# fpthink/3D-WSIS

Hardware: AMD Instinct MI355X
Metric: scenes/sec fwd+bwd ScanNet 2cm (~150k voxels) @1/8 GPU; HBM GB/s vs roofline (higher is better)
Workload: dtype f32

## Files before the change

3d-wsis_amd/csrc/bn.hip:

```cpp
#include <cstdlib>

#include "common.h"

using namespace wsis;

namespace {

constexpr int BN_ROWS_PER_THREAD = 8;
__host__ __device__ inline int bn_rows_per_wg(int Cp) {
  const int G = Cp >> 2;
  const int R = 256 / G > 1 ? 256 / G : 1;
  return R * BN_ROWS_PER_THREAD;
}
constexpr int BN_THREADS = 256;

struct f4 {
  float v[4];
};
__device__ __forceinline__ f4 ld4(const float* p, bool vec) {
  f4 r;
  if (vec) {
    const float4 t = *reinterpret_cast<const float4*>(p);
    r.v[0] = t.x; r.v[1] = t.y; r.v[2] = t.z; r.v[3] = t.w;
  } else {
    r.v[0] = p[0]; r.v[1] = p[1]; r.v[2] = p[2]; r.v[3] = p[3];
  }
  return r;
}

__device__ __forceinline__ float bn_pivot(const float* __restrict__ x, int64_t M, int C, int c) {
  const int n = M < 8 ? (int)M : 8;
  float s = 0.0f;
  for (int r = 0; r < n; ++r) s += x[(int64_t)r * C + c];
  return s / (float)n;
}

__global__ __launch_bounds__(BN_THREADS) void bn_stats_partial_kernel(const float* __restrict__ x, int64_t M, int C,
                                                                      int Cp, float* __restrict__ partial) {
  __shared__ float s_a[BN_THREADS * 4];
  __shared__ float s_b[BN_THREADS * 4];
  const int G = Cp >> 2;
  const int R = max(BN_THREADS / G, 1);
  const bool vec = (C & 3) == 0;
  const int64_t r0 = (int64_t)blockIdx.x * bn_rows_per_wg(Cp);
  const int64_t r1 = min(M, r0 + bn_rows_per_wg(Cp));
  for (int g0 = 0; g0 < G; g0 += BN_THREADS) {
    const int g = g0 + (threadIdx.x % min(G, BN_THREADS));
    const int rl = threadIdx.x / min(G, BN_THREADS);
    float sa[4] = {0.f, 0.f, 0.f, 0.f}, sb[4] = {0.f, 0.f, 0.f, 0.f};
    if (g < G && rl < R) {
      const int c = g * 4;
      float K[4];
#pragma unroll
      for (int e = 0; e < 4; ++e) K[e] = (c + e < C) ? bn_pivot(x, M, C, c + e) : 0.0f;
#pragma unroll 8
      for (int64_t r = r0 + rl; r < r1; r += R) {
        float v[4];
        if (vec) {
          const f4 t = ld4(x + r * C + c, true);
#pragma unroll
          for (int e = 0; e < 4; ++e) v[e] = t.v[e] - K[e];
        } else {
#pragma unroll
          for (int e = 0; e < 4; ++e) v[e] = (c + e < C) ? x[r * C + c + e] - K[e] : 0.0f;
        }
#pragma unroll
        for (int e = 0; e < 4; ++e) {
          sa[e] += v[e];
          sb[e] += v[e] * v[e];
        }
      }
    }
#pragma unroll
    for (int e = 0; e < 4; ++e) {
      s_a[threadIdx.x * 4 + e] = sa[e];
      s_b[threadIdx.x * 4 + e] = sb[e];
    }
    __syncthreads();
    if (g < G && rl == 0) {
      const int gw = min(G, BN_THREADS);
      float ta[4] = {0.f, 0.f, 0.f, 0.f}, tb[4] = {0.f, 0.f, 0.f, 0.f};
      for (int j = 0; j < R; ++j)
#pragma unroll
        for (int e = 0; e < 4; ++e) {
          ta[e] += s_a[(j * gw + (threadIdx.x % gw)) * 4 + e];
          tb[e] += s_b[(j * gw + (threadIdx.x % gw)) * 4 + e];
        }
      float* p = partial + (int64_t)blockIdx.x * 2 * Cp;
#pragma unroll
      for (int e = 0; e < 4; ++e) {
        p[g * 4 + e] = ta[e];
        p[Cp + g * 4 + e] = tb[e];
      }
    }
    __syncthreads();
  }
}

__device__ __forceinline__ double wave_sum_f64(double v) {
#pragma unroll
  for (int off = 32; off >= 1; off >>= 1) v += __shfl_xor(v, off, 64);
  return v;
}

__global__ __launch_bounds__(64) void bn_stats_final_kernel(const float* __restrict__ partial, int nblk, int C,
                                                            int Cp, int64_t M, const float* __restrict__ x0,
                                                            float* __restrict__ mean,
                                                            float* __restrict__ var,
                                                            float* __restrict__ running_mean,
                                                            float* __restrict__ running_var, float momentum) {
  const int c = blockIdx.x;
  double s = 0.0, q = 0.0;
#pragma unroll 8
  for (int b = threadIdx.x; b < nblk; b += 64) {
    s += partial[(int64_t)b * 2 * Cp + c];
    q += partial[(int64_t)b * 2 * Cp + Cp + c];
  }
  const double S = wave_sum_f64(s), Q = wave_sum_f64(q);
  if (threadIdx.x == 0) {
    const double n = (double)M;
    const double ms = S / n;
    const double mu = (double)bn_pivot(x0, M, C, c) + ms;
    double v = Q / n - ms * ms;
    if (v < 0.0) v = 0.0;
    mean[c] = (float)mu;
    var[c] = (float)v;
    if (running_mean) {
      const double unb = n > 1 ? v * n / (n - 1) : v;
      running_mean[c] = (float)((1.0 - momentum) * running_mean[c] + momentum * mu);
      running_var[c] = (float)((1.0 - momentum) * running_var[c] + momentum * unb);
    }
  }
}

constexpr int BN_FIN_CHUNKS = kBnFinChunks;

__device__ __forceinline__ bool bn_chunk_centred_stage(const float* __restrict__ partial, int nblk, int C, int64_t M,
                                                       double* __restrict__ chunk, float* __restrict__ mean,
                                                       float* __restrict__ var, float* __restrict__ running_mean,
                                                       float* __restrict__ running_var, float momentum,
                                                       unsigned* __restrict__ ticket, int g0, int G, int cgi,
                                                       double (&red)[3][8][33], int& s_last) {
  const int cl = threadIdx.x & 31, pl = threadIdx.x >> 5;
  const int c = cgi * 32 + cl;
  const int per = (nblk + G - 1) / G;
  const int lo = g0 * per;
  const int hi = lo + per < nblk ? lo + per : nblk;
  double s = 0.0, q = 0.0, w = 0.0;
  if (c < C) {
#pragma unroll 4
    for (int b = lo + pl; b < hi; b += 8) {
      const float sf = partial[(int64_t)b * 2 * C + c];
      const float qf = partial[(int64_t)b * 2 * C + C + c];
      const int64_t left = M - (int64_t)b * 32;
      const double si = sf;
      s += si;
      q += qf;
      w += si * si * (left < 32 ? 1.0 / (double)left : 0.03125);
    }
  }
  red[0][pl][cl] = s;
  red[1][pl][cl] = q;
  red[2][pl][cl] = w;
  __syncthreads();
  if (pl == 0 && c < C) {
    double S = 0.0, Q = 0.0, W = 0.0;
#pragma unroll
    for (int j = 0; j < 8; ++j) {
      S += red[0][j][cl];
      Q += red[1][j][cl];
      W += red[2][j][cl];
    }
    if (G == 1) {
      bn_finish_centred(S, Q, W, M, c, mean, var, running_mean, running_var, momentum);
    } else {
      double* o = chunk + (int64_t)g0 * 3 * C;
      st_sc1(o + c, S);
      st_sc1(o + C + c, Q);
      st_sc1(o + 2 * C + c, W);
    }
  }
  if (G == 1) return true;
  if (!ticket) return false;
  wait_stores_left();
  __syncthreads();
  if (threadIdx.x == 0) {
    const unsigned t = atomicAdd(ticket + cgi, 1u);
    s_last = t == (unsigned)G - 1;
    if (s_last) ticket[cgi] = 0u;
  }
  __syncthreads();
  if (!s_last) return false;
  double s2 = 0.0, q2 = 0.0, w2 = 0.0;
  if (c < C)
    for (int g = pl; g < G; g += 8) {
      const double* o = chunk + (int64_t)g * 3 * C;
      s2 += ld_sc1(o + c);
      q2 += ld_sc1(o + C + c);
      w2 += ld_sc1(o + 2 * C + c);
    }
  __syncthreads();
  red[0][pl][cl] = s2;
  red[1][pl][cl] = q2;
  red[2][pl][cl] = w2;
  __syncthreads();
  if (pl == 0 && c < C) {
    double S = 0.0, Q = 0.0, W = 0.0;
#pragma unroll
    for (int j = 0; j < 8; ++j) {
      S += red[0][j][cl];
      Q += red[1][j][cl];
      W += red[2][j][cl];
    }
    bn_finish_centred(S, Q, W, M, c, mean, var, running_mean, running_var, momentum);
  }
  return true;
}

__global__ __launch_bounds__(256) void bn_stats_chunk_centred_kernel(const float* __restrict__ partial, int nblk, int C,
                                                                     int64_t M, double* __restrict__ chunk,
                                                                     float* __restrict__ mean, float* __restrict__ var,
                                                                     float* __restrict__ running_mean,
                                                                     float* __restrict__ running_var, float momentum,
                                                                     unsigned* __restrict__ ticket) {
  __shared__ double red[3][8][33];
  __shared__ int s_last;
  bn_chunk_centred_stage(partial, nblk, C, M, chunk, mean, var, running_mean, running_var, momentum, ticket,
                         (int)blockIdx.x, (int)gridDim.x, (int)blockIdx.y, red, s_last);
}

__global__ __launch_bounds__(256) void bn_stats_final_centred_kernel(const double* __restrict__ chunk, int G, int C,
                                                                     int64_t M, float* __restrict__ mean,
                                                                     float* __restrict__ var,
                                                                     float* __restrict__ running_mean,
                                                                     float* __restrict__ running_var, float momentum) {
  const int lane = threadIdx.x & 63;
  const int c = blockIdx.x * 4 + (threadIdx.x >> 6);
  if (c >= C) return;
  const bool in = lane < G;
  const double S = wave_sum_f64(in ? chunk[(int64_t)lane * 3 * C + c] : 0.0);
  const double Q = wave_sum_f64(in ? chunk[(int64_t)lane * 3 * C + C + c] : 0.0);
  const double W = wave_sum_f64(in ? chunk[(int64_t)lane * 3 * C + 2 * C + c] : 0.0);
  if (lane == 0) bn_finish_centred(S, Q, W, M, c, mean, var, running_mean, running_var, momentum);
}

template <bool COHERENT>
__device__ __forceinline__ float bn_ld_stat(const float* p) {
  if (COHERENT) return __hip_atomic_load(p, __ATOMIC_RELAXED, __HIP_MEMORY_SCOPE_AGENT);
  return *p;
}

template <bool COHERENT>
__device__ __forceinline__ void bn_apply_body(const float* __restrict__ x, const float* mean,
                                              const float* var, const float* __restrict__ gamma,
                                              const float* __restrict__ beta, float eps, int relu,
                                              float* __restrict__ y, int64_t M, int C) {
  const int64_t total = M * C;
  if ((C & 3) == 0) {
    const int64_t total4 = total >> 2;
    const unsigned C4 = (unsigned)(C >> 2);
    const int64_t stride = (int64_t)gridDim.x * blockDim.x;
    int64_t t = blockIdx.x * (int64_t)blockDim.x + threadIdx.x;
    const bool fixed_c = (stride % C4) == 0;
    unsigned cg = (unsigned)(t % C4);
    float sc[4], mu[4], bt[4];
    auto coef = [&](unsigned g) {
#pragma unroll
      for (int e = 0; e < 4; ++e) {
        const int c = (int)g * 4 + e;
        sc[e] = (gamma ? gamma[c] : 1.0f) * rsqrtf(bn_ld_stat<COHERENT>(var + c) + eps);
        mu[e] = bn_ld_stat<COHERENT>(mean + c);
        bt[e] = beta ? beta[c] : 0.0f;
      }
    };
    coef(cg);
    auto body = [&](const float4 v) {
      float o[4] = {v.x, v.y, v.z, v.w};
#pragma unroll
      for (int e = 0; e < 4; ++e) {
        float z = __builtin_fmaf(o[e] - mu[e], sc[e], bt[e]);
        if (relu) z = fmaxf(z, 0.0f);
        o[e] = z;
      }
      return make_float4(o[0], o[1], o[2], o[3]);
    };
    if (fixed_c) {
      for (; t + stride < total4; t += 2 * stride) {
        const float4 v0 = reinterpret_cast<const float4*>(x)[t];
        const float4 v1 = reinterpret_cast<const float4*>(x)[t + stride];
        reinterpret_cast<float4*>(y)[t] = body(v0);
        reinterpret_cast<float4*>(y)[t + stride] = body(v1);
      }
      if (t < total4) reinterpret_cast<float4*>(y)[t] = body(reinterpret_cast<const float4*>(x)[t]);
    } else {
      for (; t < total4; t += stride) {
        cg = (unsigned)(t % C4);
        coef(cg);
        reinterpret_cast<float4*>(y)[t] = body(reinterpret_cast<const float4*>(x)[t]);
      }
    }
  } else {
    for (int64_t t = blockIdx.x * (int64_t)blockDim.x + threadIdx.x; t < total;
         t += (int64_t)gridDim.x * blockDim.x) {
      const int c = (int)(t % C);
      const float sc = (gamma ? gamma[c] : 1.0f) * rsqrtf(bn_ld_stat<COHERENT>(var + c) + eps);
      float z = __builtin_fmaf(x[t] - bn_ld_stat<COHERENT>(mean + c), sc, beta ? beta[c] : 0.0f);
      if (relu) z = fmaxf(z, 0.0f);
      y[t] = z;
    }
  }
}

__global__ void bn_apply_kernel(const float* __restrict__ x, const float* __restrict__ mean,
                                const float* __restrict__ var, const float* __restrict__ gamma,
                                const float* __restrict__ beta, float eps, int relu, float* __restrict__ y,
                                int64_t M, int C) {
  bn_apply_body<false>(x, mean, var, gamma, beta, eps, relu, y, M, C);
}

constexpr int BN_POLL_SLEEP = 12;
constexpr unsigned long long BN_SPIN_LIMIT = 200000000ull;

__device__ __forceinline__ void bn_wait_published(SyncSlot* s) {
  if (threadIdx.x == 0) {
    const unsigned long long t0 = __builtin_amdgcn_s_memrealtime();
    while (__hip_atomic_load(&s->flag, __ATOMIC_RELAXED, __HIP_MEMORY_SCOPE_AGENT) == 0u) {
      __builtin_amdgcn_s_sleep(BN_POLL_SLEEP);
      if (__builtin_amdgcn_s_memrealtime() - t0 > BN_SPIN_LIMIT) {
        __hip_atomic_store(&s->err, 1u, __ATOMIC_RELAXED, __HIP_MEMORY_SCOPE_AGENT);
        break;
      }
    }
    const unsigned l = atomicAdd(&s->left, 1u);
    if (l == gridDim.x - 1) {
      __hip_atomic_store(&s->left, 0u, __ATOMIC_RELAXED, __HIP_MEMORY_SCOPE_AGENT);
      __hip_atomic_store(&s->flag, 0u, __ATOMIC_RELAXED, __HIP_MEMORY_SCOPE_AGENT);
    }
  }
  __syncthreads();
}
__device__ __forceinline__ void bn_publish(SyncSlot* s, int CG) {
  const unsigned d = atomicAdd(&s->done, 1u);
  if (d == (unsigned)CG - 1) {
    __hip_atomic_store(&s->done, 0u, __ATOMIC_RELAXED, __HIP_MEMORY_SCOPE_AGENT);
    __threadfence();
    __hip_atomic_store(&s->flag, 1u, __ATOMIC_RELEASE, __HIP_MEMORY_SCOPE_AGENT);
  }
}

__global__ __launch_bounds__(256) void bn_finalize_apply_kernel(
    const float* __restrict__ partial, int nblk, int C, int64_t M, double* __restrict__ chunk, int G,
    float* mean, float* var, float* __restrict__ running_mean,
    float* __restrict__ running_var, float momentum, SyncSlot* __restrict__ sync, const float* __restrict__ x,
    const float* __restrict__ gamma, const float* __restrict__ beta, float eps, int relu, float* __restrict__ y) {
  __shared__ double red[3][8][33];
  __shared__ int s_last;
  const int CG = (C + 31) / 32;
  if ((int)blockIdx.x < G * CG) {
    const bool fin = bn_chunk_centred_stage(partial, nblk, C, M, chunk, mean, var, running_mean, running_var, momentum,
                                            sync->ticket, (int)blockIdx.x % G, G, (int)blockIdx.x / G, red, s_last);
    if (fin) {
      __threadfence();
      __syncthreads();
      if (threadIdx.x == 0) bn_publish(sync, CG);
    }
  }
  bn_wait_published(sync);
  bn_apply_body<true>(x, mean, var, gamma, beta, eps, relu, y, M, C);
}

__global__ __launch_bounds__(BN_THREADS) void bn_bwd_partial_kernel(
    const float* __restrict__ x, const float* __restrict__ dy, const float* __restrict__ mean,
    const float* __restrict__ var, const float* __restrict__ gamma, const float* __restrict__ beta, float eps,
    int relu, int64_t M, int C, int Cp, float* __restrict__ partial) {
  __shared__ float s_a[BN_THREADS * 4];
  __shared__ float s_b[BN_THREADS * 4];
  const int G = Cp >> 2;
  const int gw = min(G, BN_THREADS);
  const int R = max(BN_THREADS / G, 1);
  const bool vec = (C & 3) == 0;
  const int64_t r0 = (int64_t)blockIdx.x * bn_rows_per_wg(Cp);
  const int64_t r1 = min(M, r0 + bn_rows_per_wg(Cp));
  for (int g0 = 0; g0 < G; g0 += BN_THREADS) {
    const int g = g0 + (threadIdx.x % gw);
    const int rl = threadIdx.x / gw;
    float sa[4] = {0.f, 0.f, 0.f, 0.f}, sb[4] = {0.f, 0.f, 0.f, 0.f};
    if (g < G && rl < R) {
      const int c = g * 4;
      float mu[4], rstd[4], gm[4], bt[4];
#pragma unroll
      for (int e = 0; e < 4; ++e) {
        const int cc = min(c + e, C - 1);
        mu[e] = mean[cc];
        rstd[e] = rsqrtf(var[cc] + eps);
        gm[e] = gamma ? gamma[cc] : 1.0f;
        bt[e] = beta ? beta[cc] : 0.0f;
      }
#pragma unroll 8
      for (int64_t r = r0 + rl; r < r1; r += R) {
        float xv[4], dv[4];
        if (vec) {
          const f4 tx = ld4(x + r * C + c, true), td = ld4(dy + r * C + c, true);
#pragma unroll
          for (int e = 0; e < 4; ++e) {
            xv[e] = tx.v[e];
            dv[e] = td.v[e];
          }
        } else {
#pragma unroll
          for (int e = 0; e < 4; ++e) {
            const bool ok = c + e < C;
            xv[e] = ok ? x[r * C + c + e] : 0.0f;
            dv[e] = ok ? dy[r * C + c + e] : 0.0f;
          }
        }
#pragma unroll
        for (int e = 0; e < 4; ++e) {
          const float xh = (xv[e] - mu[e]) * rstd[e];
          float dz = dv[e];
          if (relu && xh * gm[e] + bt[e] <= 0.0f) dz = 0.0f;
          sa[e] += dz;
          sb[e] += dz * xh;
        }
      }
    }
#pragma unroll
    for (int e = 0; e < 4; ++e) {
      s_a[threadIdx.x * 4 + e] = sa[e];
      s_b[threadIdx.x * 4 + e] = sb[e];
    }
    __syncthreads();
    if (g < G && rl == 0) {
      float ta[4] = {0.f, 0.f, 0.f, 0.f}, tb[4] = {0.f, 0.f, 0.f, 0.f};
      for (int j = 0; j < R; ++j)
#pragma unroll
        for (int e = 0; e < 4; ++e) {
          ta[e] += s_a[(j * gw + (threadIdx.x % gw)) * 4 + e];
          tb[e] += s_b[(j * gw + (threadIdx.x % gw)) * 4 + e];
        }
      float* p = partial + (int64_t)blockIdx.x * 2 * Cp;
#pragma unroll
      for (int e = 0; e < 4; ++e) {
        p[g * 4 + e] = ta[e];
        p[Cp + g * 4 + e] = tb[e];
      }
    }
    __syncthreads();
  }
}

__global__ __launch_bounds__(64) void bn_bwd_final_kernel(const float* __restrict__ partial, int nblk, int C, int Cp,
                                                          float* __restrict__ dgamma, float* __restrict__ dbeta) {
  const int c = blockIdx.x;
  double a = 0.0, b = 0.0;
#pragma unroll 8
  for (int k = threadIdx.x; k < nblk; k += 64) {
    a += partial[(int64_t)k * 2 * Cp + c];
    b += partial[(int64_t)k * 2 * Cp + Cp + c];
  }
  const double A = wave_sum_f64(a), B = wave_sum_f64(b);
  if (threadIdx.x == 0) {
    dbeta[c] = (float)A;
    dgamma[c] = (float)B;
  }
}

__device__ __forceinline__ bool bn_sum_chunk_stage(const float* __restrict__ partial, int nblk, int C,
                                                   double* __restrict__ chunk, float* dbeta, float* dgamma,
                                                   unsigned* __restrict__ ticket, int g0, int G, int cgi,
                                                   double (&red)[2][8][33], int& s_last) {
  const int cl = threadIdx.x & 31, pl = threadIdx.x >> 5;
  const int c = cgi * 32 + cl;
  const int per = (nblk + G - 1) / G;
  const int lo = g0 * per;
  const int hi = lo + per < nblk ? lo + per : nblk;
  double a = 0.0, b = 0.0;
  if (c < C) {
#pragma unroll 4
    for (int k = lo + pl; k < hi; k += 8) {
      a += partial[(int64_t)k * 2 * C + c];
      b += partial[(int64_t)k * 2 * C + C + c];
    }
  }
  red[0][pl][cl] = a;
  red[1][pl][cl] = b;
  __syncthreads();
  if (pl == 0 && c < C) {
    double A = 0.0, B = 0.0;
#pragma unroll
    for (int j = 0; j < 8; ++j) {
      A += red[0][j][cl];
      B += red[1][j][cl];
    }
    if (G == 1) {
      dbeta[c] = (float)A;
      dgamma[c] = (float)B;
    } else {
      st_sc1(chunk + (int64_t)g0 * 2 * C + c, A);
      st_sc1(chunk + (int64_t)g0 * 2 * C + C + c, B);
    }
  }
  if (G == 1) return true;
  if (!ticket) return false;
  wait_stores_left();
  __syncthreads();
  if (threadIdx.x == 0) {
    const unsigned t = atomicAdd(ticket + cgi, 1u);
    s_last = t == (unsigned)G - 1;
    if (s_last) ticket[cgi] = 0u;
  }
  __syncthreads();
  if (!s_last) return false;
  double a2 = 0.0, b2 = 0.0;
  if (c < C)
    for (int g = pl; g < G; g += 8) {
      const double* o = chunk + (int64_t)g * 2 * C;
      a2 += ld_sc1(o + c);
      b2 += ld_sc1(o + C + c);
    }
  __syncthreads();
  red[0][pl][cl] = a2;
  red[1][pl][cl] = b2;
  __syncthreads();
  if (pl == 0 && c < C) {
    double A = 0.0, B = 0.0;
#pragma unroll
    for (int j = 0; j < 8; ++j) {
      A += red[0][j][cl];
      B += red[1][j][cl];
    }
    dbeta[c] = (float)A;
    dgamma[c] = (float)B;
  }
  return true;
}

__global__ __launch_bounds__(256) void bn_sum_chunk_kernel(const float* __restrict__ partial, int nblk, int C,
                                                           double* __restrict__ chunk, float* __restrict__ dbeta,
                                                           float* __restrict__ dgamma, unsigned* __restrict__ ticket) {
  __shared__ double red[2][8][33];
  __shared__ int s_last;
  bn_sum_chunk_stage(partial, nblk, C, chunk, dbeta, dgamma, ticket, (int)blockIdx.x, (int)gridDim.x, (int)blockIdx.y, red,
                     s_last);
}

__global__ __launch_bounds__(256) void bn_sum_final_kernel(const double* __restrict__ chunk, int G, int C,
                                                           float* __restrict__ dbeta, float* __restrict__ dgamma) {
  const int lane = threadIdx.x & 63;
  const int c = blockIdx.x * 4 + (threadIdx.x >> 6);
  if (c >= C) return;
  const bool in = lane < G;
  const double A = wave_sum_f64(in ? chunk[(int64_t)lane * 2 * C + c] : 0.0);
  const double B = wave_sum_f64(in ? chunk[(int64_t)lane * 2 * C + C + c] : 0.0);
  if (lane == 0) {
    dbeta[c] = (float)A;
    dgamma[c] = (float)B;
  }
}

template <bool COHERENT>
__device__ __forceinline__ void bn_bwd_apply_body(const float* __restrict__ x, const float* __restrict__ dy,
                                                  const float* __restrict__ mean, const float* __restrict__ var,
                                                  const float* __restrict__ gamma, const float* __restrict__ beta,
                                                  const float* dgamma, const float* dbeta,
                                                  const float* __restrict__ addend, float eps, int relu, int training,
                                                  float* __restrict__ dx, int64_t M, int C) {
  const int64_t total = M * C;
  const float inv_m = 1.0f / (float)M;
  const bool vec = (C & 3) == 0;
  const int W = vec ? 4 : 1;
  const int64_t totalw = total / W;
  const unsigned Cw = (unsigned)(C / W);
  const int64_t stride = (int64_t)gridDim.x * blockDim.x;
  int64_t t = blockIdx.x * (int64_t)blockDim.x + threadIdx.x;
  const bool fixed_c = (stride % Cw) == 0;
  float mu[4], rstd[4], gm[4], bt[4], k1[4], k2[4];
  auto coef = [&](int c0) {
#pragma unroll
    for (int e = 0; e < 4; ++e) {
      if (e < W) {
        const int c = c0 + e;
        mu[e] = mean[c];
        rstd[e] = rsqrtf(var[c] + eps);
        gm[e] = gamma ? gamma[c] : 1.0f;
        bt[e] = beta ? beta[c] : 0.0f;
        k1[e] = training ? bn_ld_stat<COHERENT>(dbeta + c) * inv_m : 0.0f;
        k2[e] = training ? bn_ld_stat<COHERENT>(dgamma + c) * inv_m : 0.0f;
      }
    }
  };
  if (t < totalw) coef((int)(t % Cw) * W);
  auto one = [&](const float (&xv)[4], const float (&dv)[4], const float (&av)[4], float (&ov)[4]) {
#pragma unroll
    for (int e = 0; e < 4; ++e) {
      if (e < W) {
        const float xh = (xv[e] - mu[e]) * rstd[e];
        float dz = dv[e];
        if (relu && xh * gm[e] + bt[e] <= 0.0f) dz = 0.0f;
        float r = dz;
        if (training) r = dz - k1[e] - xh * k2[e];
        ov[e] = gm[e] * rstd[e] * r;
        if (addend) ov[e] += av[e];
      }
    }
  };
  if (vec && fixed_c) {
    for (; t + stride < totalw; t += 2 * stride) {
      const int64_t u = t + stride;
      const f4 tx0 = ld4(x + t * 4, true), td0 = ld4(dy + t * 4, true);
      const f4 tx1 = ld4(x + u * 4, true), td1 = ld4(dy + u * 4, true);
      f4 ta0, ta1;
#pragma unroll
      for (int e = 0; e < 4; ++e) ta0.v[e] = ta1.v[e] = 0.f;
      if (addend) {
        ta0 = ld4(addend + t * 4, true);
        ta1 = ld4(addend + u * 4, true);
      }
      float o0[4], o1[4];
      one(tx0.v, td0.v, ta0.v, o0);
      one(tx1.v, td1.v, ta1.v, o1);
      reinterpret_cast<float4*>(dx)[t] = make_float4(o0[0], o0[1], o0[2], o0[3]);
      reinterpret_cast<float4*>(dx)[u] = make_float4(o1[0], o1[1], o1[2], o1[3]);
    }
  }
  for (; t < totalw; t += stride) {
    if (!fixed_c) coef((int)(t % Cw) * W);
    float xv[4], dv[4], av[4] = {0.f, 0.f, 0.f, 0.f}, ov[4];
    if (vec) {
      const f4 tx = ld4(x + t * 4, true), td = ld4(dy + t * 4, true);
#pragma unroll
      for (int e = 0; e < 4; ++e) {
        xv[e] = tx.v[e];
        dv[e] = td.v[e];
      }
      if (addend) {
        const f4 ta = ld4(addend + t * 4, true);
#pragma unroll
        for (int e = 0; e < 4; ++e) av[e] = ta.v[e];
      }
    } else {
      xv[0] = x[t];
      dv[0] = dy[t];
      if (addend) av[0] = addend[t];
    }
    one(xv, dv, av, ov);
    if (vec)
      reinterpret_cast<float4*>(dx)[t] = make_float4(ov[0], ov[1], ov[2], ov[3]);
    else
      dx[t] = ov[0];
  }
}

__global__ void bn_bwd_apply_kernel(const float* __restrict__ x, const float* __restrict__ dy,
                                    const float* __restrict__ mean, const float* __restrict__ var,
                                    const float* __restrict__ gamma, const float* __restrict__ beta,
                                    const float* __restrict__ dgamma, const float* __restrict__ dbeta,
                                    const float* __restrict__ addend, float eps, int relu, int training,
                                    float* __restrict__ dx, int64_t M, int C) {
  bn_bwd_apply_body<false>(x, dy, mean, var, gamma, beta, dgamma, dbeta, addend, eps, relu, training, dx, M, C);
}

__global__ __launch_bounds__(256) void bn_bwd_finish_apply_kernel(
    const float* __restrict__ partial, int nblk, int C, double* __restrict__ chunk, int G, float* dbeta, float* dgamma,
    SyncSlot* __restrict__ sync, const float* __restrict__ x, const float* __restrict__ dy, const float* __restrict__ mean,
    const float* __restrict__ var, const float* __restrict__ gamma, const float* __restrict__ beta,
    const float* __restrict__ addend, float eps, int relu, float* __restrict__ dx, int64_t M) {
  __shared__ double red[2][8][33];
  __shared__ int s_last;
  const int CG = (C + 31) / 32;
  if ((int)blockIdx.x < G * CG) {
    const bool fin = bn_sum_chunk_stage(partial, nblk, C, chunk, dbeta, dgamma, sync->ticket, (int)blockIdx.x % G, G,
                                        (int)blockIdx.x / G, red, s_last);
    if (fin) {
      __threadfence();
      __syncthreads();
      if (threadIdx.x == 0) bn_publish(sync, CG);
    }
  }
  bn_wait_published(sync);
  bn_bwd_apply_body<true>(x, dy, mean, var, gamma, beta, dgamma, dbeta, addend, eps, relu, 1, dx, M, C);
}

constexpr int BN_SF_ROWS = 256;

__global__ __launch_bounds__(256) void bn_small_finish_apply_kernel(
    const float* __restrict__ partial, int nblk, int C, int64_t M, float* __restrict__ mean, float* __restrict__ var,
    float* __restrict__ running_mean, float* __restrict__ running_var, float momentum, const float* __restrict__ x,
    const float* __restrict__ gamma, const float* __restrict__ beta, float eps, int relu, float* __restrict__ y, int G) {
  __shared__ double red[3][8][33];
  __shared__ float s_mu[32], s_sc[32], s_bt[32];
  const int cgi = blockIdx.y;
  const int cl = threadIdx.x & 31, pl = threadIdx.x >> 5;
  const int c = cgi * 32 + cl;
  const int per = (nblk + G - 1) / G;
  double S = 0.0, Q = 0.0, W = 0.0;
  for (int g = 0; g < G; ++g) {
    const int lo = g * per;
    const int hi = lo + per < nblk ? lo + per : nblk;
    double s = 0.0, q = 0.0, w = 0.0;
    if (c < C) {
#pragma unroll 4
      for (int b = lo + pl; b < hi; b += 8) {
        const float sf = partial[(int64_t)b * 2 * C + c];
        const float qf = partial[(int64_t)b * 2 * C + C + c];
        const int64_t left = M - (int64_t)b * 32;
        const double si = sf;
        s += si;
        q += qf;
        w += si * si * (left < 32 ? 1.0 / (double)left : 0.03125);
      }
    }
    if (g) __syncthreads();
    red[0][pl][cl] = s;
    red[1][pl][cl] = q;
    red[2][pl][cl] = w;
    __syncthreads();
    if (pl == 0 && c < C) {
      double Sg = 0.0, Qg = 0.0, Wg = 0.0;
#pragma unroll
      for (int j = 0; j < 8; ++j) {
        Sg += red[0][j][cl];
        Qg += red[1][j][cl];
        Wg += red[2][j][cl];
      }
      if (G == 1) {
        S = Sg; Q = Qg; W = Wg;
      } else {
        S += Sg; Q += Qg; W += Wg;
      }
    }
  }
  if (pl == 0 && c < C) {
    const double n = (double)M;
    const double mu = S / n;
    double v = (Q + (W - n * mu * mu)) / n;
    if (v < 0.0) v = 0.0;
    const float muf = (float)mu, vf = (float)v;
    if (blockIdx.x == 0) {
      mean[c] = muf;
      var[c] = vf;
      if (running_mean) {
        const double unb = n > 1 ? v * n / (n - 1) : v;
        running_mean[c] = (float)((1.0 - momentum) * running_mean[c] + momentum * mu);
        running_var[c] = (float)((1.0 - momentum) * running_var[c] + momentum * unb);
      }
    }
    s_mu[cl] = muf;
    s_sc[cl] = (gamma ? gamma[c] : 1.0f) * rsqrtf(vf + eps);
    s_bt[cl] = beta ? beta[c] : 0.0f;
  }
  __syncthreads();
  const int q4 = threadIdx.x & 7, rl = threadIdx.x >> 3;
  const int c4 = cgi * 32 + q4 * 4;
  if (c4 >= C) return;
  float mu4[4], sc4[4], bt4[4];
#pragma unroll
  for (int e = 0; e < 4; ++e) {
    mu4[e] = s_mu[q4 * 4 + e];
    sc4[e] = s_sc[q4 * 4 + e];
    bt4[e] = s_bt[q4 * 4 + e];
  }
  const int64_t r0 = (int64_t)blockIdx.x * BN_SF_ROWS;
#pragma unroll 4
  for (int it = 0; it < BN_SF_ROWS / 32; ++it) {
    const int64_t r = r0 + it * 32 + rl;
    if (r < M) {
      const float4 vx = *reinterpret_cast<const float4*>(x + r * C + c4);
      float o[4] = {vx.x, vx.y, vx.z, vx.w};
#pragma unroll
      for (int e = 0; e < 4; ++e) {
        float z = __builtin_fmaf(o[e] - mu4[e], sc4[e], bt4[e]);
        if (relu) z = fmaxf(z, 0.0f);
        o[e] = z;
      }
      *reinterpret_cast<float4*>(y + r * C + c4) = make_float4(o[0], o[1], o[2], o[3]);
    }
  }
}

__global__ __launch_bounds__(256) void bn_small_bwd_finish_apply_kernel(
    const float* __restrict__ partial, int nblk, int C, int64_t M, const float* __restrict__ x,
    const float* __restrict__ dy, const float* __restrict__ mean, const float* __restrict__ var,
    const float* __restrict__ gamma, const float* __restrict__ beta, const float* __restrict__ addend, float eps, int relu,
    float* __restrict__ dx, float* __restrict__ dgamma, float* __restrict__ dbeta, int G) {
  __shared__ double red[2][8][33];
  __shared__ float s_k1[32], s_k2[32];
  const int cgi = blockIdx.y;
  const int cl = threadIdx.x & 31, pl = threadIdx.x >> 5;
  const int c = cgi * 32 + cl;
  const int per = (nblk + G - 1) / G;
  double A = 0.0, B = 0.0;
  for (int g = 0; g < G; ++g) {
    const int lo = g * per;
    const int hi = lo + per < nblk ? lo + per : nblk;
    double a = 0.0, b = 0.0;
    if (c < C) {
#pragma unroll 4
      for (int k = lo + pl; k < hi; k += 8) {
        a += partial[(int64_t)k * 2 * C + c];
        b += partial[(int64_t)k * 2 * C + C + c];
      }
    }
    if (g) __syncthreads();
    red[0][pl][cl] = a;
    red[1][pl][cl] = b;
    __syncthreads();
    if (pl == 0 && c < C) {
      double Ag = 0.0, Bg = 0.0;
#pragma unroll
      for (int j = 0; j < 8; ++j) {
        Ag += red[0][j][cl];
        Bg += red[1][j][cl];
      }
      if (G == 1) {
        A = Ag; B = Bg;
      } else {
        A += Ag; B += Bg;
      }
    }
  }
  if (pl == 0 && c < C) {
    const float db = (float)A, dg = (float)B;
    if (blockIdx.x == 0) {
      dbeta[c] = db;
      dgamma[c] = dg;
    }
    const float inv_m = 1.0f / (float)M;
    s_k1[cl] = db * inv_m;
    s_k2[cl] = dg * inv_m;
  }
  __syncthreads();
  const int q4 = threadIdx.x & 7, rl = threadIdx.x >> 3;
  const int c4 = cgi * 32 + q4 * 4;
  if (c4 >= C) return;
  float mu[4], rstd[4], gm[4], bt[4], k1[4], k2[4];
#pragma unroll
  for (int e = 0; e < 4; ++e) {
    const int cc = c4 + e;
    mu[e] = mean[cc];
    rstd[e] = rsqrtf(var[cc] + eps);
    gm[e] = gamma ? gamma[cc] : 1.0f;
    bt[e] = beta ? beta[cc] : 0.0f;
    k1[e] = s_k1[q4 * 4 + e];
    k2[e] = s_k2[q4 * 4 + e];
  }
  const int64_t r0 = (int64_t)blockIdx.x * BN_SF_ROWS;
#pragma unroll 2
  for (int it = 0; it < BN_SF_ROWS / 32; ++it) {
    const int64_t r = r0 + it * 32 + rl;
    if (r < M) {
      const float4 vx = *reinterpret_cast<const float4*>(x + r * C + c4);
      const float4 vd = *reinterpret_cast<const float4*>(dy + r * C + c4);
      float4 va = make_float4(0.f, 0.f, 0.f, 0.f);
      if (addend) va = *reinterpret_cast<const float4*>(addend + r * C + c4);
      const float xv[4] = {vx.x, vx.y, vx.z, vx.w}, dv[4] = {vd.x, vd.y, vd.z, vd.w}, av[4] = {va.x, va.y, va.z, va.w};
      float ov[4];
#pragma unroll
      for (int e = 0; e < 4; ++e) {
        const float xh = (xv[e] - mu[e]) * rstd[e];
        float dz = dv[e];
        if (relu && xh * gm[e] + bt[e] <= 0.0f) dz = 0.0f;
        const float rr = dz - k1[e] - xh * k2[e];
        ov[e] = gm[e] * rstd[e] * rr;
        if (addend) ov[e] += av[e];
      }
      *reinterpret_cast<float4*>(dx + r * C + c4) = make_float4(ov[0], ov[1], ov[2], ov[3]);
    }
  }
}

static int bn_small_gmax() {
  const char* e = getenv("WSIS_BN_SMALL_G");
  const int g = e ? atoi(e) : 4;
  return g < 1 ? 1 : g > 8 ? 8 : g;
}
static bool bn_small_fused_on() {
  const char* e = getenv("WSIS_BN_SMALL_FUSED");
  return !e || atoi(e) != 0;
}

int64_t bn_small_rows() {
  static const int64_t v = [] {
    const char* e = getenv("WSIS_BN_SMALL_ROWS");
    return e ? (int64_t)atoll(e) : (int64_t)4096;
  }();
  return v;
}
constexpr int BN_SMALL_THREADS = 1024;

__device__ __forceinline__ void block_sum2_f64(double (&a)[4], double (&b)[4], double* sh) {
  const int lane = threadIdx.x & 63, wave = threadIdx.x >> 6;
#pragma unroll
  for (int off = 32; off >= 1; off >>= 1) {
#pragma unroll
    for (int e = 0; e < 4; ++e) {
      a[e] += __shfl_xor(a[e], off, 64);
      b[e] += __shfl_xor(b[e], off, 64);
    }
  }
  if (lane == 0) {
#pragma unroll
    for (int e = 0; e < 4; ++e) {
      sh[wave * 8 + e] = a[e];
      sh[wave * 8 + 4 + e] = b[e];
    }
  }
  __syncthreads();
#pragma unroll
  for (int e = 0; e < 4; ++e) {
    double sa = 0.0, sb = 0.0;
    for (int w = 0; w < BN_SMALL_THREADS / 64; ++w) {
      sa += sh[w * 8 + e];
      sb += sh[w * 8 + 4 + e];
    }
    a[e] = sa;
    b[e] = sb;
  }
}

__global__ __launch_bounds__(BN_SMALL_THREADS) void bn_stats_small_kernel(const float* __restrict__ x, int64_t M, int C,
                                                                    float* __restrict__ mean, float* __restrict__ var,
                                                                    float* __restrict__ running_mean,
                                                                    float* __restrict__ running_var, float momentum) {
  __shared__ double sh[BN_SMALL_THREADS / 64 * 8];
  const int c0 = blockIdx.x * 4;
  const bool vec = (C & 3) == 0;
  float sa[4] = {0.f, 0.f, 0.f, 0.f}, sb[4] = {0.f, 0.f, 0.f, 0.f};
  float K[4];
#pragma unroll
  for (int e = 0; e < 4; ++e) K[e] = (c0 + e < C) ? bn_pivot(x, M, C, c0 + e) : 0.0f;
#pragma unroll 8
  for (int64_t r = threadIdx.x; r < M; r += BN_SMALL_THREADS) {
    float v[4];
    if (vec) {
      const f4 t = ld4(x + r * C + c0, true);
#pragma unroll
      for (int e = 0; e < 4; ++e) v[e] = t.v[e] - K[e];
    } else {
#pragma unroll
      for (int e = 0; e < 4; ++e) v[e] = (c0 + e < C) ? x[r * C + c0 + e] - K[e] : 0.0f;
    }
#pragma unroll
    for (int e = 0; e < 4; ++e) {
      sa[e] += v[e];
      sb[e] += v[e] * v[e];
    }
  }
  double a[4], b[4];
#pragma unroll
  for (int e = 0; e < 4; ++e) {
    a[e] = sa[e];
    b[e] = sb[e];
  }
  block_sum2_f64(a, b, sh);
  if (threadIdx.x < 4 && c0 + (int)threadIdx.x < C) {
    const int e = threadIdx.x, c = c0 + e;
    const double n = (double)M;
    const double ms = a[e] / n;
    const double mu = (double)K[e] + ms;
    double v = b[e] / n - ms * ms;
    if (v < 0.0) v = 0.0;
    mean[c] = (float)mu;
    var[c] = (float)v;
    if (running_mean) {
      const double unb = n > 1 ? v * n / (n - 1) : v;
      running_mean[c] = (float)((1.0 - momentum) * running_mean[c] + momentum * mu);
      running_var[c] = (float)((1.0 - momentum) * running_var[c] + momentum * unb);
    }
  }
}

__global__ __launch_bounds__(BN_SMALL_THREADS) void bn_bwd_small_kernel(
    const float* __restrict__ x, const float* __restrict__ dy, const float* __restrict__ mean,
    const float* __restrict__ var, const float* __restrict__ gamma, const float* __restrict__ beta, float eps,
    int relu, int64_t M, int C, float* __restrict__ dgamma, float* __restrict__ dbeta) {
  __shared__ double sh[BN_SMALL_THREADS / 64 * 8];
  const int c0 = blockIdx.x * 4;
  const bool vec = (C & 3) == 0;
  float mu[4], rstd[4], gm[4], bt[4];
#pragma unroll
  for (int e = 0; e < 4; ++e) {
    const int cc = min(c0 + e, C - 1);
    mu[e] = mean[cc];
    rstd[e] = rsqrtf(var[cc] + eps);
    gm[e] = gamma ? gamma[cc] : 1.0f;
    bt[e] = beta ? beta[cc] : 0.0f;
  }
  float sa[4] = {0.f, 0.f, 0.f, 0.f}, sb[4] = {0.f, 0.f, 0.f, 0.f};
#pragma unroll 8
  for (int64_t r = threadIdx.x; r < M; r += BN_SMALL_THREADS) {
    float xv[4], dv[4];
    if (vec) {
      const f4 tx = ld4(x + r * C + c0, true), td = ld4(dy + r * C + c0, true);
#pragma unroll
      for (int e = 0; e < 4; ++e) {
        xv[e] = tx.v[e];
        dv[e] = td.v[e];
      }
    } else {
#pragma unroll
      for (int e = 0; e < 4; ++e) {
        const bool ok = c0 + e < C;
        xv[e] = ok ? x[r * C + c0 + e] : 0.0f;
        dv[e] = ok ? dy[r * C + c0 + e] : 0.0f;
      }
    }
#pragma unroll
    for (int e = 0; e < 4; ++e) {
      const float xh = (xv[e] - mu[e]) * rstd[e];
      float dz = dv[e];
      if (relu && xh * gm[e] + bt[e] <= 0.0f) dz = 0.0f;
      sa[e] += dz;
      sb[e] += dz * xh;
    }
  }
  double a[4], b[4];
#pragma unroll
  for (int e = 0; e < 4; ++e) {
    a[e] = sa[e];
    b[e] = sb[e];
  }
  block_sum2_f64(a, b, sh);
  if (threadIdx.x < 4 && c0 + (int)threadIdx.x < C) {
    dbeta[c0 + threadIdx.x] = (float)a[threadIdx.x];
    dgamma[c0 + threadIdx.x] = (float)b[threadIdx.x];
  }
}

int bn_nblk(int64_t M, int Cp) { return (int)ceil_div(M > 0 ? M : 1, (int64_t)bn_rows_per_wg(Cp)); }

}

extern "C" {

int64_t wsis_bn_workspace_bytes(int64_t M, int32_t C) {
  if (M < 0 || C < 1) return -1;
  const int64_t Cp = (C + 3) / 4 * 4;
  return (int64_t)bn_nblk(M, (int)Cp) * 2 * Cp * (int64_t)sizeof(float) + 256;
}

int wsis_bn_stats(const float* d_x, int64_t M, int32_t C, float* d_mean, float* d_var, float* d_running_mean,
                  float* d_running_var, float momentum, void* d_ws, int64_t ws_bytes, void* stream) {
  WSIS_REQUIRE(M >= 1 && C >= 1 && d_x && d_mean && d_var && d_ws, "bad args");
  WSIS_REQUIRE(ws_bytes >= wsis_bn_workspace_bytes(M, C), "workspace too small");
  WSIS_REQUIRE((d_running_mean == nullptr) == (d_running_var == nullptr), "running stats come in pairs");
  const int Cp = (C + 3) / 4 * 4;
  const int nblk = bn_nblk(M, Cp);
  float* partial = static_cast<float*>(d_ws);
  hipStream_t st = as_stream(stream);
  WSIS_REQUIRE(Cp / 4 <= BN_THREADS, "C > 1024 is not supported");
  if (M <= bn_small_rows()) {
    hipLaunchKernelGGL(bn_stats_small_kernel, dim3(Cp / 4), dim3(BN_SMALL_THREADS), 0, st, d_x, M, C, d_mean, d_var,
                       d_running_mean, d_running_var, momentum);
    WSIS_LAUNCH_CHECK();
    return WSIS_OK;
  }
  hipLaunchKernelGGL(bn_stats_partial_kernel, dim3(nblk), dim3(BN_THREADS), 0, st, d_x, M, C, Cp, partial);
  WSIS_LAUNCH_CHECK();
  hipLaunchKernelGGL(bn_stats_final_kernel, dim3(C), dim3(64), 0, st, partial, nblk, C, Cp, M, d_x, d_mean,
                     d_var, d_running_mean, d_running_var, momentum);
  WSIS_LAUNCH_CHECK();
  return WSIS_OK;
}


__device__ __forceinline__ void colsum_block(const bool IN, const bool OUT, const float* __restrict__ x, int64_t lo,
                                             int64_t hi, int C4, float4* red, float* __restrict__ out) {
  const int RL = 256 / C4;
  const int cl = threadIdx.x % C4, rl = threadIdx.x / C4;
  float4 a = {0.f, 0.f, 0.f, 0.f};
  if (rl < RL) {
    const float4* x4 = reinterpret_cast<const float4*>(x);
#pragma unroll 8
    for (int64_t r = lo + rl; r < hi; r += RL) {
      float4 v;
      if (IN) {
        const float* p = x + (r * C4 + cl) * 4;
        v = make_float4(ld_sc1(p), ld_sc1(p + 1), ld_sc1(p + 2), ld_sc1(p + 3));
      } else {
        v = x4[r * C4 + cl];
      }
      a.x += v.x;
      a.y += v.y;
      a.z += v.z;
      a.w += v.w;
    }
    red[rl * C4 + cl] = a;
  }
  __syncthreads();
  if (threadIdx.x < C4) {
    float4 s = red[threadIdx.x];
    for (int j = 1; j < RL; ++j) {
      const float4 v = red[j * C4 + threadIdx.x];
      s.x += v.x;
      s.y += v.y;
      s.z += v.z;
      s.w += v.w;
    }
    if (OUT) {
      float* p = out + threadIdx.x * 4;
      st_sc1(p, s.x);
      st_sc1(p + 1, s.y);
      st_sc1(p + 2, s.z);
      st_sc1(p + 3, s.w);
    } else {
      reinterpret_cast<float4*>(out)[threadIdx.x] = s;
    }
  }
}

__global__ __launch_bounds__(256) void colsum_kernel(const float* __restrict__ x, int64_t M, int C, int64_t per,
                                                     float* __restrict__ chunk, float* __restrict__ out,
                                                     unsigned* __restrict__ ticket) {
  __shared__ float4 red[256];
  __shared__ int s_last;
  const int C4 = C >> 2;
  const int64_t lo = (int64_t)blockIdx.x * per;
  const int64_t hi = lo + per < M ? lo + per : M;
  if (gridDim.x == 1) {
    colsum_block(false, false, x, lo, hi, C4, red, out);
    return;
  }
  colsum_block(false, true, x, lo, hi, C4, red, chunk + (int64_t)blockIdx.x * C);
  wait_stores_left();
  __syncthreads();
  if (threadIdx.x == 0) {
    const unsigned t = atomicAdd(ticket, 1u);
    s_last = t == gridDim.x - 1;
    if (s_last) *ticket = 0u;
  }
  __syncthreads();
  if (!s_last) return;
  __syncthreads();
  colsum_block(true, false, chunk, 0, gridDim.x, C4, red, out);
}

static unsigned* bn_tickets(void* d_sync) {
  static int on = -1;
  if (on < 0) {
    const char* e = tune_env("WSIS_BN_TICKET");
    on = e ? atoi(e) : 1;
  }
  if (!on || !d_sync) return nullptr;
  return static_cast<SyncSlot*>(d_sync)->ticket;
}


int64_t wsis_bn_stats_finalize_workspace_bytes(int64_t n_part, int32_t C) {
  return (int64_t)bn_fin_chunks(n_part) * 3 * C * (int64_t)sizeof(double) + 256;
}

int wsis_bn_stats_finalize(const float* d_partials, int64_t n_part, int64_t M, int32_t C, float* d_mean, float* d_var,
                           float* d_running_mean, float* d_running_var, float momentum, void* d_ws, int64_t ws_bytes,
                           void* d_sync, void* stream) {
  WSIS_REQUIRE(n_part >= 1 && M >= 1 && C >= 1 && d_partials && d_mean && d_var, "bad args");
  WSIS_REQUIRE(n_part < ((int64_t)1 << 31), "too many partials");
  WSIS_REQUIRE((d_running_mean == nullptr) == (d_running_var == nullptr), "running stats come in pairs");
  WSIS_REQUIRE(n_part == (M + 31) / 32, "one partial per 32-row slice");
  const int G = bn_fin_chunks(n_part);
  WSIS_REQUIRE(G == 1 || (d_ws && ws_bytes >= wsis_bn_stats_finalize_workspace_bytes(n_part, C)), "workspace too small");
  double* chunk = reinterpret_cast<double*>((reinterpret_cast<uintptr_t>(d_ws) + 255) & ~(uintptr_t)255);
  WSIS_REQUIRE(C <= 512, "more than 512 channels");
  unsigned* tickets = bn_tickets(d_sync);
  hipLaunchKernelGGL(bn_stats_chunk_centred_kernel, dim3(G, (C + 31) / 32), dim3(256), 0, as_stream(stream), d_partials,
                     (int)n_part, C, M, chunk, d_mean, d_var, d_running_mean, d_running_var, momentum, tickets);
  WSIS_LAUNCH_CHECK();
  if (G > 1 && !tickets) {
    hipLaunchKernelGGL(bn_stats_final_centred_kernel, dim3((C + 3) / 4), dim3(256), 0, as_stream(stream), chunk, G, C, M,
                       d_mean, d_var, d_running_mean, d_running_var, momentum);
    WSIS_LAUNCH_CHECK();
  }
  return WSIS_OK;
}

static int bn_fused_grid(int64_t M, int C, int need_chunk_wgs, int which = 0) {
#if !WSIS_EXPERIMENTAL
  return 0;
#endif
  const char* e = getenv("WSIS_BN_FUSED_APPLY");
  const int on = e ? atoi(e) : 0;
  const char* ed = getenv(which ? "WSIS_BN_FUSED_BWD" : "WSIS_BN_FUSED_FWD");
  const int on_dir = ed ? atoi(ed) : on;
  const char* g = tune_env("WSIS_BN_FUSED_GRID");
  int gmax = g ? atoi(g) : 256;
  if (gmax < 64 || gmax > 512) gmax = 256;
  int n_cu = 0;
  {
    int dev = 0, v = 0;
    n_cu = (hipGetDevice(&dev) == hipSuccess &&
            hipDeviceGetAttribute(&v, hipDeviceAttributeMultiprocessorCount, dev) == hipSuccess) ? v : 0;
  }
  if (!on_dir || (C & 3) != 0) return 0;
  const int cw = C >> 2;
  const int64_t work = (M * C) >> 2;
  int gcap = (work > 600000 && gmax == 256) ? 512 : gmax;
  if (gcap > 2 * n_cu) gcap = 2 * n_cu;
  if (gcap < 1) return 0;
  int grid = gcap - (gcap % cw);
  const int need = grid_for(work, 256);
  if (need < grid) {
    grid = need;
    if (grid > cw) grid -= grid % cw;
  }
  return (grid >= need_chunk_wgs && grid >= 1) ? grid : 0;
}

int wsis_bn_stats_finalize_apply(const float* d_partials, int64_t n_part, int64_t M, int32_t C, float* d_mean,
                                 float* d_var, float* d_running_mean, float* d_running_var, float momentum,
                                 const float* d_x, const float* d_gamma, const float* d_beta, float eps, int32_t relu,
                                 float* d_y, void* d_ws, int64_t ws_bytes, void* d_sync, void* stream) {
  WSIS_REQUIRE(n_part >= 1 && M >= 1 && C >= 1 && d_partials && d_mean && d_var && d_x && d_y, "bad args");
  WSIS_REQUIRE(n_part == (M + 31) / 32 && n_part < ((int64_t)1 << 31), "one partial per 32-row slice");
  WSIS_REQUIRE(C <= 512, "more than 512 channels");
  hipStream_t st = as_stream(stream);
  const int G = bn_fin_chunks(n_part);
  const int CG = (C + 31) / 32;
  WSIS_REQUIRE(G == 1 || (d_ws && ws_bytes >= wsis_bn_stats_finalize_workspace_bytes(n_part, C)), "workspace too small");
  double* chunk = reinterpret_cast<double*>((reinterpret_cast<uintptr_t>(d_ws) + 255) & ~(uintptr_t)255);
  unsigned* tickets = bn_tickets(d_sync);
  const int grid = tickets ? bn_fused_grid(M, C, G * CG) : 0;
  const bool fused = grid > 0;
  if (G <= bn_small_gmax() && (G == 1 || tickets) && (C & 3) == 0 && bn_small_fused_on() &&
      (reinterpret_cast<uintptr_t>(d_x) & 15) == 0 &&
      (reinterpret_cast<uintptr_t>(d_y) & 15) == 0) {
    hipLaunchKernelGGL(bn_small_finish_apply_kernel, dim3((unsigned)ceil_div(M, BN_SF_ROWS), (unsigned)CG), dim3(256), 0,
                       st, d_partials, (int)n_part, (int)C, M, d_mean, d_var, d_running_mean, d_running_var, momentum, d_x,
                       d_gamma, d_beta, eps, (int)relu, d_y, G);
    WSIS_LAUNCH_CHECK();
    return WSIS_OK;
  }
  if (!fused) {
    const int rc = wsis_bn_stats_finalize(d_partials, n_part, M, C, d_mean, d_var, d_running_mean, d_running_var, momentum,
                                          d_ws, ws_bytes, d_sync, stream);
    if (rc != WSIS_OK) return rc;
    return wsis_bn_apply(d_x, d_mean, d_var, d_gamma, d_beta, eps, relu, d_y, M, C, stream);
  }
  hipLaunchKernelGGL(bn_finalize_apply_kernel, dim3(grid), dim3(256), 0, st, d_partials, (int)n_part, (int)C, M, chunk, G,
                     d_mean, d_var, d_running_mean, d_running_var, momentum, static_cast<SyncSlot*>(d_sync), d_x, d_gamma,
                     d_beta, eps, (int)relu, d_y);
  WSIS_LAUNCH_CHECK();
  return WSIS_OK;
}

static int bn_apply_grid(int64_t work, int cw, int pt_unused) {
  (void)pt_unused;
  const int pt = tune_int("WSIS_BN_APPLY_PT", 8);
  int64_t g;
  if (pt < 0) {
    g = grid_for(work, 256);
  } else {
    g = ceil_div(work, (int64_t)256 * pt);
    if (g < 512) {
      g = ceil_div(work, 256);
      if (g > 512) g = 512;
    }
    if (g > 16384) g = 16384;
  }
  if (g < 1) g = 1;
  if (g > cw) g -= g % cw;
  return (int)g;
}

int wsis_bn_apply(const float* d_x, const float* d_mean, const float* d_var, const float* d_gamma,
                  const float* d_beta, float eps, int32_t relu, float* d_y, int64_t M, int32_t C, void* stream) {
  WSIS_REQUIRE(M >= 0 && C >= 1, "bad sizes");
  if (M == 0) return WSIS_OK;
  WSIS_REQUIRE(d_x && d_mean && d_var && d_y, "null pointer");
  const int64_t work = (C & 3) == 0 ? (M * C) >> 2 : M * C;
  const int cw = (C & 3) == 0 ? C >> 2 : C;
  const int grid = bn_apply_grid(work, cw, 2);
  hipLaunchKernelGGL(bn_apply_kernel, dim3(grid), dim3(256), 0, as_stream(stream), d_x, d_mean, d_var,
                     d_gamma, d_beta, eps, relu, d_y, M, C);
  WSIS_LAUNCH_CHECK();
  return WSIS_OK;
}

int wsis_bn_bwd_from_partials(const float* d_partials, int64_t n_part, const float* d_x, const float* d_dy,
                              const float* d_mean, const float* d_var, const float* d_gamma, const float* d_beta,
                              float eps, int32_t relu, float* d_dx, float* d_dgamma, float* d_dbeta,
                              const float* d_addend, int64_t M, int32_t C, void* d_ws, int64_t ws_bytes, void* d_sync,
                              void* stream) {
  WSIS_REQUIRE(M >= 1 && C >= 1 && d_partials && d_x && d_dy && d_mean && d_var && d_dgamma && d_dbeta, "bad args");
  WSIS_REQUIRE(n_part == (M + 31) / 32 && n_part < ((int64_t)1 << 31), "one partial per 32-row slice");
  const int G = bn_fin_chunks(n_part);
  WSIS_REQUIRE(G == 1 || (d_ws && ws_bytes >= wsis_bn_stats_finalize_workspace_bytes(n_part, C)), "workspace too small");
  double* chunk = reinterpret_cast<double*>((reinterpret_cast<uintptr_t>(d_ws) + 255) & ~(uintptr_t)255);
  hipStream_t st = as_stream(stream);
  WSIS_REQUIRE(C <= 512, "more than 512 channels");
  unsigned* tickets = bn_tickets(d_sync);
  if (d_dx && G <= bn_small_gmax() && (G == 1 || tickets) && (C & 3) == 0 && bn_small_fused_on() &&
      (reinterpret_cast<uintptr_t>(d_x) & 15) == 0 &&
      (reinterpret_cast<uintptr_t>(d_dy) & 15) == 0 && (reinterpret_cast<uintptr_t>(d_dx) & 15) == 0 &&
      (reinterpret_cast<uintptr_t>(d_addend) & 15) == 0) {
    hipLaunchKernelGGL(bn_small_bwd_finish_apply_kernel, dim3((unsigned)ceil_div(M, BN_SF_ROWS), (unsigned)((C + 31) / 32)),
                       dim3(256), 0, st, d_partials, (int)n_part, (int)C, M, d_x, d_dy, d_mean, d_var, d_gamma, d_beta,
                       d_addend, eps, (int)relu, d_dx, d_dgamma, d_dbeta, G);
    WSIS_LAUNCH_CHECK();
    return WSIS_OK;
  }
  if (d_dx) {
    const int CG = (C + 31) / 32;
    const int fgrid = tickets ? bn_fused_grid(M, C, G * CG, 1) : 0;
    if (fgrid > 0) {
      hipLaunchKernelGGL(bn_bwd_finish_apply_kernel, dim3(fgrid), dim3(256), 0, st, d_partials, (int)n_part, (int)C, chunk, G,
                         d_dbeta, d_dgamma, static_cast<SyncSlot*>(d_sync), d_x, d_dy, d_mean,
                         d_var, d_gamma, d_beta, d_addend, eps, (int)relu, d_dx, M);
      WSIS_LAUNCH_CHECK();
      return WSIS_OK;
    }
  }
  hipLaunchKernelGGL(bn_sum_chunk_kernel, dim3(G, (C + 31) / 32), dim3(256), 0, st, d_partials, (int)n_part, C, chunk,
                     d_dbeta, d_dgamma, tickets);
  WSIS_LAUNCH_CHECK();
  if (G > 1 && !tickets) {
    hipLaunchKernelGGL(bn_sum_final_kernel, dim3((C + 3) / 4), dim3(256), 0, st, chunk, G, C, d_dbeta, d_dgamma);
    WSIS_LAUNCH_CHECK();
  }
  if (d_dx) {
    const int64_t work = (C & 3) == 0 ? (M * C) >> 2 : M * C;
    const int cw = (C & 3) == 0 ? C >> 2 : C;
    const int grid = bn_apply_grid(work, cw, 2);
    hipLaunchKernelGGL(bn_bwd_apply_kernel, dim3(grid), dim3(256), 0, st, d_x, d_dy, d_mean, d_var, d_gamma, d_beta,
                       d_dgamma, d_dbeta, d_addend, eps, relu, 1, d_dx, M, C);
    WSIS_LAUNCH_CHECK();
  }
  return WSIS_OK;
}

int wsis_bn_bwd_apply(const float* d_x, const float* d_dy, const float* d_mean, const float* d_var,
                      const float* d_gamma, const float* d_beta, const float* d_sum_dz_xhat, const float* d_sum_dz,
                      float eps, int32_t relu, float* d_dx, const float* d_addend, int64_t M, int32_t C, void* stream) {
  WSIS_REQUIRE(M >= 1 && C >= 1 && d_x && d_dy && d_mean && d_var && d_sum_dz_xhat && d_sum_dz && d_dx, "bad args");
  const int64_t work = (C & 3) == 0 ? (M * C) >> 2 : M * C;
  const int cw = (C & 3) == 0 ? C >> 2 : C;
  const int grid = bn_apply_grid(work, cw, 2);
  hipLaunchKernelGGL(bn_bwd_apply_kernel, dim3(grid), dim3(256), 0, as_stream(stream), d_x, d_dy, d_mean, d_var, d_gamma,
                     d_beta, d_sum_dz_xhat, d_sum_dz, d_addend, eps, relu, 1, d_dx, M, C);
  WSIS_LAUNCH_CHECK();
  return WSIS_OK;
}

int wsis_bn_bwd(const float* d_x, const float* d_dy, const float* d_mean, const float* d_var,
                const float* d_gamma, const float* d_beta, float eps, int32_t relu, int32_t training,
                float* d_dx, float* d_dgamma, float* d_dbeta, const float* d_addend, int64_t M, int32_t C, void* d_ws,
                int64_t ws_bytes, void* stream) {
  WSIS_REQUIRE(M >= 1 && C >= 1 && d_x && d_dy && d_mean && d_var && d_dgamma && d_dbeta && d_ws, "bad args");
  WSIS_REQUIRE(ws_bytes >= wsis_bn_workspace_bytes(M, C), "workspace too small");
  const int Cp = (C + 3) / 4 * 4;
  const int nblk = bn_nblk(M, Cp);
  float* partial = static_cast<float*>(d_ws);
  hipStream_t st = as_stream(stream);
  WSIS_REQUIRE(Cp / 4 <= BN_THREADS, "C > 1024 is not supported");
  if (M <= bn_small_rows()) {
    hipLaunchKernelGGL(bn_bwd_small_kernel, dim3(Cp / 4), dim3(BN_SMALL_THREADS), 0, st, d_x, d_dy, d_mean, d_var, d_gamma,
                       d_beta, eps, relu, M, C, d_dgamma, d_dbeta);
    WSIS_LAUNCH_CHECK();
  } else {
    hipLaunchKernelGGL(bn_bwd_partial_kernel, dim3(nblk), dim3(BN_THREADS), 0, st, d_x, d_dy, d_mean, d_var, d_gamma,
                       d_beta, eps, relu, M, C, Cp, partial);
    WSIS_LAUNCH_CHECK();
    hipLaunchKernelGGL(bn_bwd_final_kernel, dim3(C), dim3(64), 0, st, partial, nblk, C, Cp, d_dgamma, d_dbeta);
    WSIS_LAUNCH_CHECK();
  }
  if (d_dx) {
    const int64_t work = (C & 3) == 0 ? (M * C) >> 2 : M * C;
    const int cw = (C & 3) == 0 ? C >> 2 : C;
    const int grid = bn_apply_grid(work, cw, 2);
    hipLaunchKernelGGL(bn_bwd_apply_kernel, dim3(grid), dim3(256), 0, st, d_x, d_dy, d_mean, d_var, d_gamma, d_beta,
                       d_dgamma, d_dbeta, d_addend, eps, relu, training, d_dx, M, C);
    WSIS_LAUNCH_CHECK();
  }
  return WSIS_OK;
}

int64_t wsis_sync_bytes(void) { return (int64_t)kSyncSlotsTotal * (int64_t)sizeof(SyncSlot); }

int64_t wsis_colsum_workspace_bytes(int64_t M, int32_t C) {
  if (M < 0 || C < 4) return -1;
  int64_t per = (M + 127) / 128;
  if (per < 256) per = 256;
  const int64_t G = (M + per - 1) / per;
  return (G > 1 ? G : 1) * (int64_t)C * (int64_t)sizeof(float) + 256;
}

int wsis_colsum(const float* d_x, int64_t M, int32_t C, float* d_out, void* d_ws, int64_t ws_bytes, void* d_sync,
                void* stream) {
  WSIS_REQUIRE(M >= 0 && C >= 4 && C % 4 == 0 && C <= 1024 && d_out, "colsum: C must be a multiple of 4, <= 1024");
  hipStream_t st = as_stream(stream);
  if (M == 0) {
    WSIS_HIP_CHECK(hipMemsetAsync(d_out, 0, sizeof(float) * (size_t)C, st));
    return WSIS_OK;
  }
  WSIS_REQUIRE(d_x && (reinterpret_cast<uintptr_t>(d_x) & 15) == 0 && (reinterpret_cast<uintptr_t>(d_out) & 15) == 0,
               "colsum: 16-byte alignment");
  int64_t per = (M + 127) / 128;
  if (per < 256) per = 256;
  const int64_t G = (M + per - 1) / per;
  float* chunk = nullptr;
  unsigned* ticket = nullptr;
  if (G > 1) {
    WSIS_REQUIRE(d_ws && ws_bytes >= wsis_colsum_workspace_bytes(M, C), "workspace too small");
    chunk = reinterpret_cast<float*>((reinterpret_cast<uintptr_t>(d_ws) + 255) & ~(uintptr_t)255);
    WSIS_REQUIRE(d_sync, "colsum over more than one chunk needs a sync slot");
    ticket = static_cast<SyncSlot*>(d_sync)->ticket;
  }
  hipLaunchKernelGGL(colsum_kernel, dim3((unsigned)G), dim3(256), 0, st, d_x, M, (int)C, per, chunk, d_out, ticket);
  WSIS_LAUNCH_CHECK();
  return WSIS_OK;
}

}
```

3d-wsis_amd/csrc/common.h:

```cpp
#pragma once
#include <hip/hip_runtime.h>
#include <hip/hip_ext.h>
#include <cstdlib>

#include <cstdint>
#include <cstdio>
#include <string>
#include <vector>

#include "../../include/wsis_hip.h"

namespace wsis {
inline const char* tune_env(const char* name) {
#if WSIS_EXPERIMENTAL
  return getenv(name);
#else
  (void)name;
  return nullptr;
#endif
}
inline int tune_int(const char* name, int dflt) {
  const char* e = tune_env(name);
  return e ? atoi(e) : dflt;
}

std::string& err_slot();
int fail(int code, const char* fmt, ...);

#define WSIS_HIP_CHECK(expr)                                                          \
  do {                                                                                \
    hipError_t e_ = (expr);                                                           \
    if (e_ != hipSuccess)                                                             \
      return ::wsis::fail(WSIS_ERR_HIP, "%s failed: %s (%s:%d)", #expr, hipGetErrorString(e_), \
                          __FILE__, __LINE__);                                        \
  } while (0)

#define WSIS_LAUNCH_CHECK() WSIS_HIP_CHECK(hipGetLastError())

#define WSIS_REQUIRE(cond, msg)                                     \
  do {                                                              \
    if (!(cond)) return ::wsis::fail(WSIS_ERR_ARG, "%s: %s", __func__, msg); \
  } while (0)

inline hipStream_t as_stream(void* s) { return reinterpret_cast<hipStream_t>(s); }

inline int64_t ceil_div(int64_t a, int64_t b) { return (a + b - 1) / b; }

inline int grid_for(int64_t work_items, int block) {
  int64_t g = ceil_div(work_items, block);
  if (g < 1) g = 1;
  if (g > 256 * 8) g = 256 * 8;
  return (int)g;
}

struct ProfRec {
  hipEvent_t a, b, c;
  const unsigned long long* d_stamps = nullptr;
  int s0 = 0, sm = 0, s1 = 0;
};
inline bool g_prof_on = false;
inline std::vector<ProfRec> g_prof[3];
inline std::vector<void*> g_prof_bufs;

struct ProfScope {
  int which;
  hipStream_t st;
  ProfRec r{};
  int stage = 0;
  bool exact = false;
  ProfScope(int w, hipStream_t s, bool exact_events = false) : which(w), st(s) {
    if (g_prof_on && hipEventCreate(&r.a) == hipSuccess && hipEventCreate(&r.b) == hipSuccess) {
      exact = exact_events && prof_exact();
      stage = exact ? 1 : (hipEventRecord(r.a, st) == hipSuccess ? 1 : 0);
    }
  }
  static bool prof_exact() {
    static int on = -1;
    if (on < 0) {
      const char* e = getenv("WSIS_PROF_EXACT");
      on = e ? atoi(e) : 1;
    }
    return on != 0;
  }
  void bracket() {
    if (exact && stage == 1) {
      exact = false;
      stage = hipEventRecord(r.a, st) == hipSuccess ? 1 : 0;
    }
  }
  hipEvent_t ka() const { return (exact && stage == 1) ? r.a : nullptr; }
  hipEvent_t kb() const { return (exact && stage == 1) ? r.b : nullptr; }
  void stop() {
    if (stage == 1) {
      if (!exact) (void)hipEventRecord(r.b, st);
      stage = 2;
    }
  }
  void tail() {
    if (stage == 2 && hipEventCreate(&r.c) == hipSuccess) (void)hipEventRecord(r.c, st);
  }
  ~ProfScope() {
    if (stage == 2) g_prof[which].push_back(r);
  }
};


#ifdef __HIPCC__
__device__ __forceinline__ void st_sc1(float* p, float v) { __hip_atomic_store(p, v, __ATOMIC_RELAXED, __HIP_MEMORY_SCOPE_AGENT); }
__device__ __forceinline__ void st_sc1(double* p, double v) { __hip_atomic_store(p, v, __ATOMIC_RELAXED, __HIP_MEMORY_SCOPE_AGENT); }
__device__ __forceinline__ float ld_sc1(const float* p) {
  return __hip_atomic_load(const_cast<float*>(p), __ATOMIC_RELAXED, __HIP_MEMORY_SCOPE_AGENT);
}
__device__ __forceinline__ double ld_sc1(const double* p) {
  return __hip_atomic_load(const_cast<double*>(p), __ATOMIC_RELAXED, __HIP_MEMORY_SCOPE_AGENT);
}
__device__ __forceinline__ void wait_stores_left() { asm volatile("s_waitcnt vmcnt(0)" ::: "memory"); }
#endif

struct SyncSlot {
  unsigned ticket[16];
  unsigned done, flag, left, err;
  unsigned ctr[44];
  unsigned fin[960];
};
static_assert(sizeof(SyncSlot) == 4096, "sync slot layout");
constexpr int kSyncSlots = 64;
constexpr int kSyncSlotsTotal = kSyncSlots + 1;
inline SyncSlot* sync_slot(void* d_sync, int i) {
  return d_sync ? static_cast<SyncSlot*>(d_sync) + (i % kSyncSlots) : nullptr;
}
inline void* deep_sync_slot(void* d_sync) { return d_sync ? static_cast<SyncSlot*>(d_sync) + kSyncSlots : nullptr; }

__device__ __forceinline__ void bn_finish_centred(double S, double Q, double W, int64_t M, int c, float* mean, float* var,
                                                  float* running_mean, float* running_var, float momentum) {
  const double n = (double)M;
  const double mu = S / n;
  double v = (Q + (W - n * mu * mu)) / n;
  if (v < 0.0) v = 0.0;
  mean[c] = (float)mu;
  var[c] = (float)v;
  if (running_mean) {
    const double unb = n > 1 ? v * n / (n - 1) : v;
    running_mean[c] = (float)((1.0 - momentum) * running_mean[c] + momentum * mu);
    running_var[c] = (float)((1.0 - momentum) * running_var[c] + momentum * unb);
  }
}

constexpr int kBnFinChunks = 64;
inline int bn_fin_chunks(int64_t n_part) {
  int64_t g = n_part / 64;
  if (g < 1) g = 1;
  if (g > kBnFinChunks) g = kBnFinChunks;
  return (int)g;
}

bool spconv_in_supported(int K, int Cin, int Cout);
int spconv_in_launch(const float* d_X, const int32_t* d_nbr, const int32_t* d_order, const float* d_W, const float* d_bias,
                     const float* d_residual, float* d_out, int64_t M_out, hipEvent_t ka, hipEvent_t kb, hipStream_t st);

int64_t spconv_in_dw_workspace_bytes(int64_t M_out);
int spconv_in_dw_launch(const float* d_X, const int32_t* d_nbr, const int32_t* d_order, const float* d_dY, float* d_dW,
                        int64_t M_out, void* d_ws, hipEvent_t ka, hipEvent_t kb, hipStream_t st);

int spconv_ring_plan(int64_t M_out, int K, int Cin, int Cout);
int spconv_ring_launch(int nt, const float* d_X, const int32_t* d_nbr, const int32_t* d_order, const float* d_WT, int flip,
                       const float* d_bias, const float* d_residual, float* d_out, float* d_stats, const void* epi,
                       unsigned* d_err, int64_t M_in, int64_t M_out, int K, int Cin, int Cout, hipEvent_t ka, hipEvent_t kb, hipStream_t st,
                       unsigned long long* d_dbg = nullptr);

bool dw2_supported(int K, int Cin, int Cout);
bool dw2_fits(int64_t M_in, int64_t M_out, int K, int Cin, int Cout);
int64_t dw2_workspace_bytes(int64_t M_out, int K, int Cin, int Cout);
void dw2_set_batch_rows(int64_t rows);
int64_t dw2_batch_rows();
struct DwRedRec {
  const float* partial = nullptr;
  float* dW = nullptr;
  int64_t total4 = 0;
  int32_t P = 0;
};
void dw2_set_defer(DwRedRec* slot);
int dw2_reduce_batch(const DwRedRec* recs, int n, hipStream_t st);
int dw2_launch(const float* d_X, const int32_t* d_nbr, const int32_t* d_order, const float* d_dY, float* d_dW,
               int64_t M_in, int64_t M_out, int K, int Cin, int Cout, void* d_ws, hipStream_t st);
int dw2_launch_swapped(const float* d_X, const float* d_mean, const float* d_var, const float* d_gamma, const float* d_beta,
                       float eps, int relu, const int32_t* d_nbr_b, const int32_t* d_order_b, int flip, const float* d_dY,
                       float* d_dW, int64_t M_in, int64_t M_out, int K, int Cin, int Cout, void* d_ws, hipStream_t st);

#ifdef __HIPCC__
struct RowCol {
  int64_t row;
  int col;
};
__device__ __forceinline__ RowCol row_col(int64_t t, int C, int64_t total) {
  RowCol rc;
  if ((C & (C - 1)) == 0) {
    const int sh = __ffs(C) - 1;
    rc.row = t >> sh;
    rc.col = (int)(t & (C - 1));
  } else if (total < ((int64_t)1 << 32)) {
    const uint32_t q = (uint32_t)t / (uint32_t)C;
    rc.row = q;
    rc.col = (int)((uint32_t)t - q * (uint32_t)C);
  } else {
    rc.row = t / C;
    rc.col = (int)(t - rc.row * C);
  }
  return rc;
}
#endif

constexpr int64_t kEmptyKey = -1;

__device__ __forceinline__ uint64_t mix64(uint64_t x) {
  x ^= x >> 33;
  x *= 0xff51afd7ed558ccdULL;
  x ^= x >> 33;
  x *= 0xc4ceb9fe1a85ec53ULL;
  x ^= x >> 33;
  return x;
}

__device__ __forceinline__ int32_t hash_lookup(const int64_t* __restrict__ keys,
                                               const int32_t* __restrict__ vals, uint64_t mask,
                                               int64_t key) {
  uint64_t h = mix64((uint64_t)key) & mask;
  for (;;) {
    int64_t k = keys[h];
    if (k == key) return vals[h];
    if (k == kEmptyKey) return -1;
    h = (h + 1) & mask;
  }
}

}
```

3d-wsis_amd/csrc/executor.hip:

```cpp
#include <optional>
#include <condition_variable>
#include <cstdlib>
#include <deque>
#include <map>
#include <mutex>
#include <string>
#include <thread>
#include <utility>
#include <vector>

#include <unistd.h>

#include <algorithm>

#include "common.h"
#if WSIS_EXPERIMENTAL
#include "deep.h"
#endif

using namespace wsis;

namespace {

constexpr int64_t ALIGN = 256;
inline int64_t up(int64_t v) { return (v + ALIGN - 1) / ALIGN * ALIGN; }

template <int W>
__global__ void cat_rows_kernel(const float* __restrict__ a, const float* __restrict__ b, float* __restrict__ out,
                                int64_t M, int Ca, int Cb) {
  const int Ca_w = Ca / W, C_w = (Ca + Cb) / W;
  const int64_t total = M * C_w;
  for (int64_t t = blockIdx.x * (int64_t)blockDim.x + threadIdx.x; t < total; t += (int64_t)gridDim.x * blockDim.x) {
    const RowCol rc = row_col(t, C_w, total);
    const int64_t r = rc.row;
    const int c = rc.col;
    const float* src = c < Ca_w ? a + (r * Ca_w + c) * W : b + (r * (C_w - Ca_w) + (c - Ca_w)) * W;
    if (W == 4)
      reinterpret_cast<float4*>(out)[t] = *reinterpret_cast<const float4*>(src);
    else
      out[t] = *src;
  }
}

template <int W>
__global__ void split_rows_kernel(const float* __restrict__ in, float* __restrict__ a, float* __restrict__ b, int64_t M,
                                  int Ca, int Cb) {
  const int Ca_w = Ca / W, C_w = (Ca + Cb) / W;
  const int64_t total = M * C_w;
  for (int64_t t = blockIdx.x * (int64_t)blockDim.x + threadIdx.x; t < total; t += (int64_t)gridDim.x * blockDim.x) {
    const RowCol rc = row_col(t, C_w, total);
    const int64_t r = rc.row;
    const int c = rc.col;
    float* dst = c < Ca_w ? a + (r * Ca_w + c) * W : b + (r * (C_w - Ca_w) + (c - Ca_w)) * W;
    if (W == 4)
      *reinterpret_cast<float4*>(dst) = reinterpret_cast<const float4*>(in)[t];
    else
      *dst = in[t];
  }
}

__global__ void add_inplace_kernel(float* __restrict__ dst, const float* __restrict__ src, int64_t n) {
  for (int64_t t = blockIdx.x * (int64_t)blockDim.x + threadIdx.x; t < n; t += (int64_t)gridDim.x * blockDim.x)
    dst[t] += src[t];
}

inline bool vec4_ok(const wsis_op& op, const void* p0, const void* p1, const void* p2) {
  return (op.Cin % 4 == 0) && (op.Cout % 4 == 0) &&
         ((reinterpret_cast<uintptr_t>(p0) | reinterpret_cast<uintptr_t>(p1) | reinterpret_cast<uintptr_t>(p2)) & 15) == 0;
}

constexpr int WT_MAX = 64;
constexpr int WT_TILE = 32;
struct WtBatch {
  const float* src[WT_MAX];
  float* dst[WT_MAX];
  int K[WT_MAX], Cin[WT_MAX], Cout[WT_MAX], flip[WT_MAX];
  int start[WT_MAX + 1];
  int n;
};

__global__ __launch_bounds__(256) void weight_transpose_batch_kernel(WtBatch b) {
  __shared__ float tile[WT_TILE][WT_TILE + 1];
  const int t = blockIdx.x;
  int lo = 0, hi = b.n - 1;
  while (lo < hi) {
    const int mid = (lo + hi + 1) >> 1;
    if (b.start[mid] <= t)
      lo = mid;
    else
      hi = mid - 1;
  }
  const int Cin = b.Cin[lo], Cout = b.Cout[lo], K = b.K[lo];
  const int ti = (Cin + WT_TILE - 1) / WT_TILE, to = (Cout + WT_TILE - 1) / WT_TILE;
  int u = t - b.start[lo];
  const int bo = u % to;
  u /= to;
  const int bi = u % ti;
  const int kt = u / ti;
  const int ks = b.flip[lo] ? (K - 1 - kt) : kt;
  const float* __restrict__ src = b.src[lo] + (int64_t)ks * Cin * Cout;
  float* __restrict__ dst = b.dst[lo] + (int64_t)kt * Cin * Cout;
  const int x = threadIdx.x & 31, y0 = threadIdx.x >> 5;
#pragma unroll
  for (int y = y0; y < WT_TILE; y += 8) {
    const int ci = bi * WT_TILE + y, co = bo * WT_TILE + x;
    if (ci < Cin && co < Cout) tile[y][x] = src[(int64_t)ci * Cout + co];
  }
  __syncthreads();
#pragma unroll
  for (int y = y0; y < WT_TILE; y += 8) {
    const int co = bo * WT_TILE + y, ci = bi * WT_TILE + x;
    if (ci < Cin && co < Cout) dst[(int64_t)co * Cin + ci] = tile[x][y];
  }
}

struct SideStream {
  bool pending_join = false;
  hipStream_t stream = nullptr;
  hipEvent_t join = nullptr;
  hipEvent_t mark_main = nullptr, mark_side = nullptr;
  hipEvent_t wt_fork = nullptr, wt_done = nullptr;
  std::vector<hipEvent_t> fork;
  size_t next = 0;
};

SideStream* side_stream_for(hipStream_t main) {
  static std::mutex mu;
  static std::map<std::pair<int, hipStream_t>, SideStream> pool;
  int dev = 0;
  if (hipGetDevice(&dev) != hipSuccess) return nullptr;
  std::lock_guard<std::mutex> lock(mu);
  SideStream& s = pool[std::make_pair(dev, main)];
  if (!s.stream) {
    if (hipStreamCreateWithFlags(&s.stream, hipStreamNonBlocking) != hipSuccess) return nullptr;
    if (hipEventCreateWithFlags(&s.join, hipEventDisableTiming) != hipSuccess) return nullptr;
    if (hipEventCreateWithFlags(&s.mark_main, hipEventDisableTiming) != hipSuccess) return nullptr;
    if (hipEventCreateWithFlags(&s.mark_side, hipEventDisableTiming) != hipSuccess) return nullptr;
    if (hipEventCreateWithFlags(&s.wt_fork, hipEventDisableTiming) != hipSuccess) return nullptr;
    if (hipEventCreateWithFlags(&s.wt_done, hipEventDisableTiming) != hipSuccess) return nullptr;
  }
  return &s;
}

hipEvent_t next_fork_event(SideStream* s) {
  if (s->next == s->fork.size()) {
    hipEvent_t e = nullptr;
    if (hipEventCreateWithFlags(&e, hipEventDisableTiming) != hipSuccess) return nullptr;
    s->fork.push_back(e);
  }
  return s->fork[s->next++];
}

struct DwTask {
  std::thread::id owner;
  wsis_op op;
  hipEvent_t ev;
  int dev;
  hipStream_t side;
  char* ws;
  int64_t ws_bytes;
  DwRedRec* rec = nullptr;
  const DwRedRec* flush = nullptr;
  int flush_n = 0;
};
static int issue_dw_raw(const wsis_op& op, char* dw_ws, int64_t dw_bytes, void* dw_stream) {
  if (op.flags & WSIS_OPF_BN_IN)
    return wsis_spconv_dw_bn((const float*)op.in[0], (const float*)op.in[7], (const float*)op.in[8], (const float*)op.in[9],
                             (const float*)op.in[10], op.eps, (op.flags & WSIS_OPF_RELU) ? 1 : 0, (const int32_t*)op.in[5],
                             (const int32_t*)op.in[6], (op.flags & WSIS_OPF_FLIP) ? 1 : 0, (const float*)op.in[2],
                             (float*)op.out[1], op.M_in, op.M_out, op.K, op.Cin, op.Cout, dw_ws, dw_bytes, dw_stream);
  return wsis_spconv_dw((const float*)op.in[0], (const int32_t*)op.in[3], (const int32_t*)op.in[4], (const float*)op.in[2],
                        (float*)op.out[1], op.M_in, op.M_out, op.K, op.Cin, op.Cout, dw_ws, dw_bytes, dw_stream);
}
int issue_dw(const wsis_op& op, char* dw_ws, int64_t dw_bytes, void* dw_stream, DwRedRec* rec = nullptr) {
  if (rec) *rec = DwRedRec{};
  dw2_set_defer(rec);
  const int rc = issue_dw_raw(op, dw_ws, dw_bytes, dw_stream);
  dw2_set_defer(nullptr);
  return rc;
}
class DwWorker {
 public:
  void push(DwTask t) {
    std::lock_guard<std::mutex> lock(mu_);
    const long pid = (long)getpid();
    if (started_ && pid_ != pid) {
      started_ = false;
      q_.clear();
      st_.clear();
    }
    if (!started_) {
      started_ = true;
      pid_ = pid;
      std::thread(&DwWorker::run, this).detach();
    }
    t.owner = std::this_thread::get_id();
    q_.push_back(t);
    ++st_[t.owner].pending;
    cv_.notify_one();
  }
  int drain(std::string* msg) {
    const std::thread::id me = std::this_thread::get_id();
    std::unique_lock<std::mutex> lock(mu_);
    done_.wait(lock, [&] { return st_[me].pending == 0; });
    State& s = st_[me];
    const int rc = s.err;
    if (rc != WSIS_OK && msg) *msg = s.msg;
    s.err = WSIS_OK;
    s.msg.clear();
    return rc;
  }

 private:
  struct State {
    int pending = 0, err = WSIS_OK;
    std::string msg;
  };
  void run() {
    for (;;) {
      DwTask t;
      {
        std::unique_lock<std::mutex> lock(mu_);
        cv_.wait(lock, [this] { return !q_.empty(); });
        t = q_.front();
        q_.pop_front();
      }
      int rc = WSIS_OK;
      std::string msg;
      hipError_t he = hipSetDevice(t.dev);
      if (he == hipSuccess && t.ev) he = hipStreamWaitEvent(t.side, t.ev, 0);
      if (he != hipSuccess) {
        rc = WSIS_ERR_HIP;
        msg = std::string("dW worker: ") + hipGetErrorString(he);
      } else {
        rc = t.flush ? dw2_reduce_batch(t.flush, t.flush_n, t.side) : issue_dw(t.op, t.ws, t.ws_bytes, t.side, t.rec);
        if (rc != WSIS_OK) msg = wsis_last_error();
      }
      std::lock_guard<std::mutex> lock(mu_);
      State& s = st_[t.owner];
      if (rc != WSIS_OK && s.err == WSIS_OK) {
        s.err = rc;
        s.msg = msg;
      }
      if (--s.pending == 0) done_.notify_all();
    }
  }
  std::mutex mu_;
  std::condition_variable cv_, done_;
  std::deque<DwTask> q_;
  std::map<std::thread::id, State> st_;
  bool started_ = false;
  long pid_ = 0;
};
DwWorker& dw_worker() {
  static DwWorker* w = new DwWorker();
  return *w;
}
bool dw_thread_enabled() {
  const char* e = tune_env("WSIS_DW_THREAD");
  return e ? atoi(e) != 0 : true;
}

bool dw_batch_reduce_enabled() {
  const char* e = getenv("WSIS_DW_BATCH_REDUCE");
  return (e ? atoi(e) != 0 : false) && !g_prof_on;
}

bool dw_tail_main_enabled() {
  const char* e = getenv("WSIS_DW_TAIL_MAIN");
  return e ? atoi(e) != 0 : true;
}
inline bool dw_tail_on_main(const wsis_op* ops, int n, int i) {
  return i == n - 1 && ops[i].kind == WSIS_OP_CONV_BWD && ops[i].out[1] && !ops[i].out[0];
}

bool dw_stream_enabled() {
  const char* e = getenv("WSIS_DW_STREAM");
  return e ? atoi(e) != 0 : true;
}

inline int64_t wt_bytes_of(const wsis_op& op) {
  return up((int64_t)op.K * op.Cin * op.Cout * (int64_t)sizeof(float));
}

bool fwd2_enabled() {
  const char* e = getenv("WSIS_FWD2");
  return e ? atoi(e) != 0 : true;
}
inline bool use_fwd2(const wsis_op& op, bool on) {
  const int64_t gathered = op.kind == WSIS_OP_CONV ? op.M_in * op.Cin : op.M_out * op.Cout;
  return on && wsis_spconv_fwd_t_supported(op.K, op.Cin, op.Cout) != 0 && gathered * 4 < ((int64_t)1 << 31);
}
inline bool needs_wt(const wsis_op& op, bool on) {
  if (op.kind == WSIS_OP_CONV) return use_fwd2(op, on);
  if (op.kind == WSIS_OP_CONV_BWD) return op.out[0] != nullptr && !use_fwd2(op, on);
  return false;
}

inline int64_t dw_ws_of(const wsis_op& op) {
  if (op.flags & WSIS_OPF_BN_IN) return up(wsis_spconv_dw_bn_workspace_bytes(op.M_in, op.K, op.Cin, op.Cout));
  return up(wsis_spconv_dw_workspace_bytes(op.M_out, op.K, op.Cin, op.Cout));
}

int64_t op_ws_bytes(const wsis_op& op, bool on) {
  switch (op.kind) {
    case WSIS_OP_CONV:
#if WSIS_EXPERIMENTAL
      if (op.flags & (WSIS_OPF_BN_IN | WSIS_OPF_STAT_FIN))
        return up(std::max(wsis_spconv_fwd_f_workspace_bytes(op.M_out, op.K, op.Cin, op.Cout),
                           wsis_spconv_fwd_t_workspace_bytes(op.M_out, op.K, op.Cin, op.Cout)));
#else
      if (op.flags & (WSIS_OPF_BN_IN | WSIS_OPF_STAT_FIN)) return -1;
#endif
      if (use_fwd2(op, on)) return up(wsis_spconv_fwd_t_workspace_bytes(op.M_out, op.K, op.Cin, op.Cout));
      return up(wsis_spconv_fwd_workspace_bytes(op.M_out, op.K, op.Cin, op.Cout));
    case WSIS_OP_BN_RELU:
      if (!(op.flags & WSIS_OPF_TRAINING)) return 0;
      return up(std::max(wsis_bn_workspace_bytes(op.M_in, op.Cin),
                         wsis_bn_stats_finalize_workspace_bytes((op.M_in + 31) / 32, op.Cin)));
    case WSIS_OP_BN_RELU_BWD:
      return up(std::max(wsis_bn_workspace_bytes(op.M_in, op.Cin),
                         wsis_bn_stats_finalize_workspace_bytes((op.M_in + 31) / 32, op.Cin)));
    case WSIS_OP_CONV_BWD:
      if (!op.out[0]) return 0;
      if (use_fwd2(op, on)) return up(wsis_spconv_fwd_t_workspace_bytes(op.M_in, op.K, op.Cout, op.Cin));
      return up(wsis_spconv_fwd_workspace_bytes(op.M_in, op.K, op.Cout, op.Cin));
    default:
      return 0;
  }
}


#if WSIS_EXPERIMENTAL
inline int64_t deep_rows(const wsis_op& op) {
  switch (op.kind) {
    case WSIS_OP_CONV: return op.M_out;
    case WSIS_OP_CONV_BWD: return op.out[0] ? op.M_in : 0;
    default: return op.M_in;
  }
}
inline bool aligned16(const void* p) { return (reinterpret_cast<uintptr_t>(p) & 15) == 0; }

inline int paired_bn(const wsis_op* ops, int n, int i) {
  const wsis_op& op = ops[i];
  for (int j = i + 1; j < n && j <= i + 4; ++j)
    if (ops[j].kind == WSIS_OP_BN_RELU_BWD && ops[j].in[1] == op.out[0] && (ops[j].flags & WSIS_OPF_STATS)) return j;
  return -1;
}

bool deep_op_ok(const wsis_op* ops, int n, int i, bool fwd2_on) {
  const wsis_op& op = ops[i];
  const int64_t R = deep_max_rows();
  int nw = 0, zs = 0;
  switch (op.kind) {
    case WSIS_OP_CONV:
      if (op.flags & (WSIS_OPF_BN_IN | WSIS_OPF_STAT_FIN)) return false;
      if (!use_fwd2(op, fwd2_on) || op.M_out < 1 || op.M_out > R) return false;
      if ((int64_t)op.K * op.M_out * 4 >= ((int64_t)1 << 31)) return false;
      return deep_conv_plan(op.M_out, op.K, op.Cin, op.Cout, &nw, &zs) && aligned16(op.in[0]) && aligned16(op.out[0]);
    case WSIS_OP_CONV_BWD: {
      if (op.flags & WSIS_OPF_BN_IN) return false;
      if (!op.out[0]) return op.M_in <= R;
      if (!use_fwd2(op, fwd2_on) || op.M_in < 1 || op.M_in > R) return false;
      if (!deep_conv_plan(op.M_in, op.K, op.Cout, op.Cin, &nw, &zs)) return false;
      if (op.flags & WSIS_OPF_STATS) {
        const int j = paired_bn(ops, n, i);
        if (j < 0 || !ops[j].in[7] || ops[j].M_in != op.M_in || ops[j].Cin != op.Cin) return false;
      }
      return aligned16(op.in[2]) && aligned16(op.out[0]);
    }
    case WSIS_OP_BN_RELU:
      if (op.M_in < 1 || op.M_in > R || op.Cin % 32 || !deep_bn_rows_ok(op.M_in)) return false;
      if (op.flags & WSIS_OPF_TRAINING) {
        if (!(op.flags & WSIS_OPF_STATS) || !op.in[5]) return false;
        if (op.in[6] && (op.K % 32 || op.K <= 0 || op.K >= op.Cin)) return false;
      } else if (!op.out[0]) {
        return false;
      }
      return aligned16(op.in[0]) && (!op.out[0] || aligned16(op.out[0]));
    case WSIS_OP_BN_RELU_BWD:
      if (op.M_in < 1 || op.M_in > R || op.Cin % 32 || !deep_bn_rows_ok(op.M_in)) return false;
      if (!(op.flags & WSIS_OPF_TRAINING) || !(op.flags & WSIS_OPF_STATS) || !op.in[7]) return false;
      return aligned16(op.in[0]) && aligned16(op.in[1]) && aligned16(op.out[0]) && (!op.in[6] || aligned16(op.in[6]));
    case WSIS_OP_CAT:
      return op.M_in >= 1 && op.M_in <= R && vec4_ok(op, op.in[0], op.in[1], op.out[0]);
    case WSIS_OP_SPLIT:
      return op.M_in >= 1 && op.M_in <= R && vec4_ok(op, op.in[0], op.out[0], op.out[1]);
    default:
      return false;
  }
}

int deep_run_end(const wsis_op* ops, int n, int i0, int stop, bool fwd2_on) {
  int i1 = i0;
  while (i1 < n && (stop < 0 || i1 <= stop) && deep_op_ok(ops, n, i1, fwd2_on)) ++i1;
  for (int i = i0; i < i1; ++i)
    if (ops[i].kind == WSIS_OP_CONV_BWD && ops[i].out[0] && (ops[i].flags & WSIS_OPF_STATS)) {
      const int j = paired_bn(ops, n, i);
      if (j >= i1) {
        i1 = i;
        break;
      }
    }
  for (int j = i0; j < i1; ++j)
    if (ops[j].kind == WSIS_OP_BN_RELU_BWD) {
      bool found = false;
      for (int i = j - 1; i >= i0 && i >= j - 4 && !found; --i)
        found = ops[i].kind == WSIS_OP_CONV_BWD && ops[i].out[0] == ops[j].in[1] && (ops[i].flags & WSIS_OPF_STATS);
      if (!found) {
        i1 = j;
        break;
      }
    }
  return i1;
}

constexpr int kDeepMinOps = 4;
std::vector<std::pair<std::vector<DeepOp>, const unsigned long long*>> g_deep_log;
inline int64_t deep_table_bytes(int n_ops) { return up((int64_t)(2 * n_ops + 2) * (int64_t)sizeof(DeepOp)); }

int64_t deep_slab_bytes(const wsis_op* ops, int i0, int i1) {
  int64_t b = 0;
  for (int i = i0; i < i1; ++i) {
    const wsis_op& op = ops[i];
    int nw = 0, zs = 1;
    if (op.kind == WSIS_OP_CONV && deep_conv_plan(op.M_out, op.K, op.Cin, op.Cout, &nw, &zs) && zs > 1)
      b += up((int64_t)zs * op.M_out * op.Cout * 4);
    if (op.kind == WSIS_OP_CONV_BWD && op.out[0] && deep_conv_plan(op.M_in, op.K, op.Cout, op.Cin, &nw, &zs) && zs > 1)
      b += up((int64_t)zs * op.M_in * op.Cin * 4);
  }
  return b;
}

int64_t deep_ws_bytes(const wsis_op* ops, int n, bool fwd2_on) {
  if (!deep_enabled()) return 0;
  int64_t best = 0;
  for (int i = 0; i < n;) {
    if (!deep_op_ok(ops, n, i, fwd2_on)) {
      ++i;
      continue;
    }
    const int i1 = deep_run_end(ops, n, i, -1, fwd2_on);
    if (i1 - i >= kDeepMinOps) best = std::max(best, deep_table_bytes(i1 - i) + deep_slab_bytes(ops, i, i1));
    i = i1 > i ? i1 : i + 1;
  }
  return best;
}

int deep_build(const wsis_op* ops, int n, int i0, int i1, const char* wt_base, const std::vector<int64_t>& wt_off, char* slab,
               bool stamps, std::vector<DeepOp>& tab, std::vector<std::pair<int, std::pair<int, int>>>& conv_stamps) {
  tab.clear();
  conv_stamps.clear();
  auto push = [&](DeepOp& d) {
    d.stamp = stamps ? (int)tab.size() + 1 : -1;
    tab.push_back(d);
  };
  for (int i = i0; i < i1; ++i) {
    const wsis_op& op = ops[i];
    DeepOp d{};
    d.NW = 1;
    d.ZS = 1;
    switch (op.kind) {
      case WSIS_OP_CONV:
      case WSIS_OP_CONV_BWD: {
        const bool fwd = op.kind == WSIS_OP_CONV;
        if (!fwd && !op.out[0]) break;
        const int64_t Mo = fwd ? op.M_out : op.M_in, Mg = fwd ? op.M_in : op.M_out;
        const int Ci = fwd ? op.Cin : op.Cout, Co = fwd ? op.Cout : op.Cin;
        int nw = 1, zs = 1;
        if (!deep_conv_plan(Mo, op.K, Ci, Co, &nw, &zs)) return fail(WSIS_ERR_ARG, "deep: op %d has no plan", i);
        d.kind = DK_CONV;
        d.NW = nw;
        d.ZS = zs;
        d.K = op.K;
        d.Cin = Ci;
        d.Cout = Co;
        d.M_in = Mg;
        d.M_out = Mo;
        d.x_bytes = (uint32_t)(Mg * Ci * 4);
        const void* stats = nullptr;
        DeepOp epi{};
        if (fwd) {
          d.p[0] = op.in[0];
          d.p[1] = op.in[1];
          d.p[2] = op.in[2];
          d.p[3] = wt_base + wt_off[i];
          d.p[4] = op.in[4];
          d.p[5] = op.in[5];
          d.p[6] = op.out[0];
          d.flip = 0;
          if (op.flags & WSIS_OPF_STATS) stats = op.out[1];
        } else {
          d.p[0] = op.in[2];
          d.p[1] = op.in[5];
          d.p[2] = op.in[6];
          d.p[3] = op.in[1];
          d.p[6] = op.out[0];
          d.flip = (op.flags & WSIS_OPF_FLIP) ? 1 : 0;
          if (op.flags & WSIS_OPF_STATS) {
            const wsis_op& bn = ops[paired_bn(ops, n, i)];
            stats = bn.in[7];
            epi.p[9] = bn.in[0];
            epi.p[10] = bn.in[2];
            epi.p[11] = bn.in[3];
            epi.p[12] = bn.in[4];
            epi.p[13] = bn.in[5];
            epi.eps = bn.eps;
            epi.relu = (bn.flags & WSIS_OPF_RELU) ? 1 : 0;
          }
        }
        WSIS_REQUIRE(d.p[1] || (op.K == 1 && Mg == Mo), "nbr may be null only for the dense 1x1 case");
        const int s0 = (int)tab.size();
        if (zs > 1) {
          DeepOp r = d;
          d.p[7] = slab;
          d.p[4] = d.p[5] = nullptr;
          push(d);
          r.kind = DK_REDUCE;
          r.p[7] = slab;
          r.p[8] = stats;
          for (int k = 9; k <= 13; ++k) r.p[k] = epi.p[k];
          r.eps = epi.eps;
          r.relu = epi.relu;
          push(r);
          slab += up((int64_t)zs * Mo * Co * 4);
        } else {
          d.p[8] = stats;
          for (int k = 9; k <= 13; ++k) d.p[k] = epi.p[k];
          d.eps = epi.eps;
          d.relu = epi.relu;
          push(d);
        }
        conv_stamps.push_back({i, {s0, (int)tab.size()}});
        break;
      }
      case WSIS_OP_BN_RELU: {
        const bool training = (op.flags & WSIS_OPF_TRAINING) != 0;
        const bool upd = (op.flags & WSIS_OPF_UPDATE_RUNNING) != 0;
        d.kind = DK_BN_FWD;
        d.training = training ? 1 : 0;
        d.relu = (op.flags & WSIS_OPF_RELU) ? 1 : 0;
        d.Cin = op.Cin;
        d.M_in = op.M_in;
        d.eps = op.eps;
        d.momentum = op.momentum;
        d.C0 = op.in[6] ? op.K : op.Cin;
        d.p[0] = op.in[0];
        d.p[1] = op.in[1];
        d.p[2] = op.in[2];
        d.p[3] = (training && !upd) ? nullptr : op.in[3];
        d.p[4] = (training && !upd) ? nullptr : op.in[4];
        d.p[5] = op.in[5];
        d.p[6] = op.in[6];
        d.p[7] = op.out[0];
        d.p[8] = op.out[1];
        d.p[9] = op.out[2];
        push(d);
        break;
      }
      case WSIS_OP_BN_RELU_BWD:
        d.kind = DK_BN_BWD;
        d.relu = (op.flags & WSIS_OPF_RELU) ? 1 : 0;
        d.Cin = op.Cin;
        d.M_in = op.M_in;
        d.eps = op.eps;
        d.p[0] = op.in[0];
        d.p[1] = op.in[1];
        d.p[2] = op.in[2];
        d.p[3] = op.in[3];
        d.p[4] = op.in[4];
        d.p[5] = op.in[5];
        d.p[6] = op.in[6];
        d.p[7] = op.in[7];
        d.p[8] = op.out[0];
        d.p[9] = op.out[1];
        d.p[10] = op.out[2];
        push(d);
        break;
      case WSIS_OP_CAT:
        d.kind = DK_CAT;
        d.Cin = op.Cin;
        d.Cout = op.Cout;
        d.M_in = op.M_in;
        d.p[0] = op.in[0];
        d.p[1] = op.in[1];
        d.p[2] = op.out[0];
        push(d);
        break;
      case WSIS_OP_SPLIT:
        d.kind = DK_SPLIT;
        d.Cin = op.Cin;
        d.Cout = op.Cout;
        d.M_in = op.M_in;
        d.p[0] = op.in[0];
        d.p[1] = op.out[0];
        d.p[2] = op.out[1];
        push(d);
        break;
      default:
        return fail(WSIS_ERR_ARG, "deep: op %d of kind %d is not a phase", i, op.kind);
    }
  }
  return WSIS_OK;
}

#else
inline int64_t deep_ws_bytes(const wsis_op*, int, bool) { return 0; }
#endif

}

__global__ void warm_stream_kernel(int* p) {
  if (p && threadIdx.x == 0xffff) p[0] = 0;
}

extern "C" {

int wsis_warm_streams(void* stream) {
  hipStream_t st = as_stream(stream);
  SideStream* side = side_stream_for(st);
  WSIS_REQUIRE(side != nullptr, "side stream creation failed");
  hipLaunchKernelGGL(warm_stream_kernel, dim3(1), dim3(64), 0, st, (int*)nullptr);
  hipLaunchKernelGGL(warm_stream_kernel, dim3(1), dim3(64), 0, side->stream, (int*)nullptr);
  WSIS_LAUNCH_CHECK();
  WSIS_HIP_CHECK(hipStreamSynchronize(side->stream));
  return WSIS_OK;
}

int64_t wsis_run_ops_workspace_bytes(const wsis_op* ops, int32_t n) {
  if (!ops || n < 0) return -1;
  int64_t need = ALIGN, wt = 0, dw = 0, dw_sum = 0;
  const bool on = fwd2_enabled();
  for (int i = 0; i < n; ++i) {
    int64_t b = op_ws_bytes(ops[i], on);
    if (b < 0) return -1;
    if (dw_tail_on_main(ops, n, i)) b = std::max(b, dw_ws_of(ops[i]));
    if (b > need) need = b;
    if (needs_wt(ops[i], on)) wt += wt_bytes_of(ops[i]);
    if (ops[i].kind == WSIS_OP_CONV_BWD && ops[i].out[1]) {
      const int64_t d = dw_ws_of(ops[i]);
      if (d < 0) return -1;
      if (d > dw) dw = d;
      dw_sum += d;
    }
  }
  const char* be = getenv("WSIS_DW_BATCH_REDUCE");
  const bool batch = be && atoi(be) != 0;
  return wt + (batch ? std::max(dw, dw_sum) : dw) + need + deep_ws_bytes(ops, n, on) + ALIGN;
}

int wsis_run_ops(const wsis_op* ops, int32_t n, void* d_ws, int64_t ws_bytes, void* d_sync, void* stream) {
  return wsis_run_ops_marked(ops, n, d_ws, ws_bytes, d_sync, stream, -1, nullptr);
}

static int run_ops_impl(const wsis_op* ops, int32_t n, void* d_ws, int64_t ws_bytes, void* d_sync, void* stream,
                        int32_t mark_op, void* waiter_stream, bool defer_join = false);

int wsis_run_ops_part(const wsis_op* ops, int32_t n, void* d_ws, int64_t ws_bytes, void* d_sync, void* stream, int32_t last) {
  return run_ops_impl(ops, n, d_ws, ws_bytes, d_sync, stream, -1, nullptr, last == 0);
}

int wsis_run_ops_marked(const wsis_op* ops, int32_t n, void* d_ws, int64_t ws_bytes, void* d_sync, void* stream,
                        int32_t mark_op, void* waiter_stream) {
#if !WSIS_EXPERIMENTAL
  return run_ops_impl(ops, n, d_ws, ws_bytes, d_sync, stream, mark_op, waiter_stream);
#else
  const char* ge = getenv("WSIS_GRAPH");
  const int graph_mode = ge ? atoi(ge) : 0;
  if (!graph_mode || mark_op >= 0 || g_prof_on || n == 0)
    return run_ops_impl(ops, n, d_ws, ws_bytes, d_sync, stream, mark_op, waiter_stream);
  hipStream_t st = as_stream(stream);
  static std::map<std::pair<hipStream_t, int64_t>, hipGraphExec_t> cache;
  static hipStream_t cap = nullptr;
  if (!cap) WSIS_HIP_CHECK(hipStreamCreateWithFlags(&cap, hipStreamNonBlocking));
  const int target = graph_mode >= 4 ? graph_mode : 1 << 30;
  int chunk_no = 0;
  for (int i0 = 0; i0 < n; ++chunk_no) {
    int i1 = i0, pending = 0;
    while (i1 < n) {
      const wsis_op& op = ops[i1];
      if (op.kind == WSIS_OP_CONV_BWD && (op.flags & WSIS_OPF_STATS) && op.out[0]) ++pending;
      if (op.kind == WSIS_OP_BN_RELU_BWD && (op.flags & WSIS_OPF_STATS) && pending > 0) --pending;
      ++i1;
      if (i1 - i0 >= target && pending == 0) break;
    }
    WSIS_HIP_CHECK(hipStreamBeginCapture(cap, hipStreamCaptureModeRelaxed));
    const int rc = run_ops_impl(ops + i0, i1 - i0, d_ws, ws_bytes, d_sync, cap, -1, nullptr);
    hipGraph_t g = nullptr;
    const hipError_t ec = hipStreamEndCapture(cap, &g);
    if (ec != hipSuccess || !g) return fail(WSIS_ERR_HIP, "graph capture failed: %s", hipGetErrorString(ec));
    if (rc != WSIS_OK) {
      (void)hipGraphDestroy(g);
      return rc;
    }
    const auto key = std::make_pair(st, ((int64_t)ops[0].kind * 4096 + n) * 64 + chunk_no);
    hipGraphExec_t& ex = cache[key];
    bool ready = false;
    if (ex) {
      hipGraphNode_t bad = nullptr;
      hipGraphExecUpdateResult res;
      if (hipGraphExecUpdate(ex, g, &bad, &res) == hipSuccess && res == hipGraphExecUpdateSuccess) {
        ready = true;
      } else {
        (void)hipGetLastError();
        (void)hipGraphExecDestroy(ex);
        ex = nullptr;
      }
    }
    if (!ready) {
      const hipError_t ei = hipGraphInstantiate(&ex, g, nullptr, nullptr, 0);
      if (ei != hipSuccess) {
        (void)hipGraphDestroy(g);
        ex = nullptr;
        return fail(WSIS_ERR_HIP, "graph instantiate failed: %s", hipGetErrorString(ei));
      }
    }
    const hipError_t el = hipGraphLaunch(ex, st);
    (void)hipGraphDestroy(g);
    if (el != hipSuccess) return fail(WSIS_ERR_HIP, "graph launch failed: %s", hipGetErrorString(el));
    i0 = i1;
  }
  return WSIS_OK;
#endif
}

static int run_ops_impl(const wsis_op* ops, int32_t n, void* d_ws, int64_t ws_bytes, void* d_sync, void* stream,
                        int32_t mark_op, void* waiter_stream, bool defer_join) {
  WSIS_REQUIRE((ops || n == 0) && n >= 0, "bad op list");
  WSIS_REQUIRE(mark_op < n && (mark_op < 0 || waiter_stream), "bad milestone");
  WSIS_REQUIRE((n == 0 || ws_bytes >= wsis_run_ops_workspace_bytes(ops, n)) && (d_ws || n == 0), "workspace too small");
  hipStream_t st = as_stream(stream);
  char* ws = static_cast<char*>(d_ws);
  const bool on = fwd2_enabled();
  std::vector<int64_t> wt_off(n, -1);
  int64_t wt_total = 0;
  SideStream* wt_side = nullptr;
  bool wt_pending = false;
  {
    const char* we = getenv("WSIS_WT_SIDE");
    hipStreamCaptureStatus cs = hipStreamCaptureStatusNone;
    const bool cap = hipStreamIsCapturing(st, &cs) != hipSuccess || cs != hipStreamCaptureStatusNone;
    bool any_wt = false, first_needs = n > 0 && needs_wt(ops[0], on);
    for (int i = 0; i < n && !any_wt; ++i) any_wt = needs_wt(ops[i], on);
    if ((we ? atoi(we) != 0 : true) && dw_stream_enabled() && !cap && any_wt && !first_needs && !g_prof_on &&
        deep_ws_bytes(ops, n, on) == 0)
      wt_side = side_stream_for(st);
    if (wt_side) {
      hipError_t e = hipEventRecord(wt_side->wt_fork, st);
      if (e == hipSuccess) e = hipStreamWaitEvent(wt_side->stream, wt_side->wt_fork, 0);
      if (e != hipSuccess) return fail(WSIS_ERR_HIP, "weight-transpose fork failed: %s", hipGetErrorString(e));
    }
  }
  hipStream_t wt_st = wt_side ? wt_side->stream : st;
  {
    WtBatch b;
    b.n = 0;
    b.start[0] = 0;
    auto flush = [&]() -> int {
      if (b.n == 0) return WSIS_OK;
      hipLaunchKernelGGL(weight_transpose_batch_kernel, dim3(b.start[b.n]), dim3(256), 0, wt_st, b);
      WSIS_LAUNCH_CHECK();
      b.n = 0;
      return WSIS_OK;
    };
    for (int i = 0; i < n; ++i) {
      const wsis_op& op = ops[i];
      if (!needs_wt(op, on)) continue;
      const bool fwd = op.kind == WSIS_OP_CONV;
      const void* wsrc = fwd ? op.in[3] : op.in[1];
      WSIS_REQUIRE(wsrc, "convolution without weights");
      wt_off[i] = wt_total;
      b.src[b.n] = (const float*)wsrc;
      b.dst[b.n] = reinterpret_cast<float*>(ws + wt_total);
      b.K[b.n] = op.K;
      b.Cin[b.n] = op.Cin;
      b.Cout[b.n] = op.Cout;
      b.flip[b.n] = (!fwd && (op.flags & WSIS_OPF_FLIP)) ? 1 : 0;
      b.start[b.n + 1] = b.start[b.n] + op.K * ((op.Cin + WT_TILE - 1) / WT_TILE) * ((op.Cout + WT_TILE - 1) / WT_TILE);
      ++b.n;
      wt_total += wt_bytes_of(op);
      if (b.n == WT_MAX) {
        const int rc = flush();
        if (rc != WSIS_OK) return rc;
      }
    }
    const int rc = flush();
    if (rc != WSIS_OK) return rc;
    if (wt_side) {
      const hipError_t e = hipEventRecord(wt_side->wt_done, wt_side->stream);
      if (e != hipSuccess) return fail(WSIS_ERR_HIP, "weight-transpose event failed: %s", hipGetErrorString(e));
      wt_pending = true;
    }
  }
  ws += wt_total;
  ws_bytes -= wt_total;
  char* const wt_base = static_cast<char*>(d_ws);
  const bool dw_defer = dw_batch_reduce_enabled();
  const bool tail_main = dw_tail_main_enabled();
  const char* early_env = getenv("WSIS_DW_EARLY");
  const char* early_rows_env = getenv("WSIS_DW_EARLY_ROWS");
  const int64_t early_rows = early_rows_env ? atoll(early_rows_env) : 500000;
  const bool dw_early = early_env ? atoi(early_env) != 0 : dw2_batch_rows() < early_rows;
  int64_t dw_bytes = 0, dw_sum = 0;
  int n_dw = 0;
  for (int i = 0; i < n; ++i)
    if (ops[i].kind == WSIS_OP_CONV_BWD && ops[i].out[1]) {
      const int64_t d = dw_ws_of(ops[i]);
      if (d > dw_bytes) dw_bytes = d;
      dw_sum += d;
      ++n_dw;
    }
  char* const dw_ws = ws;
  ws += dw_defer ? dw_sum : dw_bytes;
  ws_bytes -= dw_defer ? dw_sum : dw_bytes;
  if (ws_bytes < 0) return fail(WSIS_ERR_ARG, "wsis_run_ops: workspace too small for the weight-gradient slabs");
  std::vector<DwRedRec> dw_recs((size_t)(dw_defer ? n_dw : 0));
  int dw_next = 0, dw_flushed = 0;
  int64_t dw_off = 0;
  const int64_t deep_bytes = deep_ws_bytes(ops, n, on);
  char* const deep_ws = ws;
  (void)deep_ws;
  ws += deep_bytes;
  ws_bytes -= deep_bytes;
  SideStream* side = (dw_bytes > 0 && dw_stream_enabled()) ? side_stream_for(st) : nullptr;
  if (side) side->next = 0;
  hipStreamCaptureStatus cap_state = hipStreamCaptureStatusNone;
  const bool capturing = hipStreamIsCapturing(st, &cap_state) != hipSuccess || cap_state != hipStreamCaptureStatusNone;
  const bool use_worker = side != nullptr && dw_thread_enabled() && !g_prof_on && !capturing;
  int cur_dev = 0;
  if (use_worker && hipGetDevice(&cur_dev) != hipSuccess) return fail(WSIS_ERR_HIP, "hipGetDevice failed");
  bool worker_busy = false;
  auto drain_worker = [&]() -> int {
    if (!worker_busy) return WSIS_OK;
    worker_busy = false;
    std::string msg;
    const int wrc = dw_worker().drain(&msg);
    return wrc == WSIS_OK ? WSIS_OK : fail(wrc, "%s", msg.c_str());
  };
#define RUN_LAUNCH_CHECK()                                                                              \
  do {                                                                                                  \
    const hipError_t le_ = hipGetLastError();                                                           \
    if (le_ != hipSuccess) rc = fail(WSIS_ERR_HIP, "wsis_run_ops: launch failed: %s", hipGetErrorString(le_)); \
  } while (0)
  bool forked = false;
  int first_err = WSIS_OK;
  auto dw_issue = [&](const wsis_op& op) -> int {
    void* dw_stream = stream;
    char* my_ws = dw_ws;
    int64_t my_bytes = dw_bytes;
    DwRedRec* rec = nullptr;
    if (dw_defer && dw_next < n_dw) {
      my_bytes = dw_ws_of(op);
      my_ws = dw_ws + dw_off;
      dw_off += my_bytes;
      rec = &dw_recs[(size_t)dw_next++];
    }
    if (side) {
      hipEvent_t e = next_fork_event(side);
      hipError_t he = e ? hipEventRecord(e, st) : hipErrorOutOfMemory;
      if (he == hipSuccess && !use_worker) he = hipStreamWaitEvent(side->stream, e, 0);
      if (he != hipSuccess) return fail(WSIS_ERR_HIP, "dW side-stream fork failed: %s", hipGetErrorString(he));
      dw_stream = side->stream;
      forked = true;
      if (use_worker) {
        DwTask t;
        t.op = op;
        t.ev = e;
        t.dev = cur_dev;
        t.side = side->stream;
        t.ws = my_ws;
        t.ws_bytes = my_bytes;
        t.rec = rec;
        dw_worker().push(t);
        worker_busy = true;
        return WSIS_OK;
      }
    }
    return issue_dw(op, my_ws, my_bytes, dw_stream, rec);
  };
  auto dw_flush = [&]() -> int {
    if (!dw_defer || dw_flushed == dw_next) return WSIS_OK;
    const DwRedRec* recs = dw_recs.data() + dw_flushed;
    const int cnt = dw_next - dw_flushed;
    dw_flushed = dw_next;
    if (side && use_worker) {
      DwTask t;
      t.ev = nullptr;
      t.dev = cur_dev;
      t.side = side->stream;
      t.ws = nullptr;
      t.ws_bytes = 0;
      t.flush = recs;
      t.flush_n = cnt;
      dw_worker().push(t);
      worker_busy = true;
      return WSIS_OK;
    }
    return dw2_reduce_batch(recs, cnt, side ? side->stream : st);
  };
#if WSIS_EXPERIMENTAL
  const bool deep_on = deep_bytes > 0 && d_sync != nullptr && !capturing;
  std::vector<DeepOp> deep_tab;
  std::vector<std::pair<int, std::pair<int, int>>> deep_convs;
#endif
  const char* slab_bn_env = getenv("WSIS_SLAB_BN_PARTIALS");
  const bool slab_bn_partials = slab_bn_env && atoi(slab_bn_env) != 0;
  std::vector<char> bn_unfused(n, 0);
  for (int i = 0; i < n; ++i) {
    int rc = WSIS_OK;
    if (wt_pending && wt_off[i] >= 0) {
      wt_pending = false;
      const hipError_t e = hipStreamWaitEvent(st, wt_side->wt_done, 0);
      if (e != hipSuccess) {
        first_err = fail(WSIS_ERR_HIP, "weight-transpose join failed: %s", hipGetErrorString(e));
        break;
      }
    }
#if WSIS_EXPERIMENTAL
    if (deep_on && deep_op_ok(ops, n, i, on)) {
      const int i1 = deep_run_end(ops, n, i, mark_op >= i ? mark_op : -1, on);
      if (i1 - i >= kDeepMinOps) {
        char* slab = deep_ws + deep_table_bytes(i1 - i);
        rc = deep_build(ops, n, i, i1, wt_base, wt_off, slab, g_prof_on, deep_tab, deep_convs);
        unsigned long long* d_stamps = nullptr;
        if (rc == WSIS_OK && g_prof_on && !deep_tab.empty()) {
          if (hipMalloc((void**)&d_stamps, (deep_tab.size() + 1) * sizeof(unsigned long long)) != hipSuccess)
            rc = fail(WSIS_ERR_HIP, "deep: stamp buffer allocation failed");
          else
            g_prof_bufs.push_back(d_stamps);
        }
        if (rc == WSIS_OK)
          rc = deep_launch(deep_tab.data(), (int)deep_tab.size(), deep_ws, deep_sync_slot(d_sync), d_stamps, st);
        if (rc == WSIS_OK && d_stamps) {
          if (g_deep_log.size() > 64) g_deep_log.clear();
          g_deep_log.push_back({deep_tab, d_stamps});
        }
        if (rc == WSIS_OK && d_stamps)
          for (const auto& cs : deep_convs) {
            ProfRec r{};
            r.d_stamps = d_stamps;
            r.s0 = cs.second.first;
            r.sm = cs.second.first + 1;
            r.s1 = cs.second.second;
            g_prof[0].push_back(r);
          }
        for (int k = i; k < i1 && rc == WSIS_OK; ++k)
          if (ops[k].kind == WSIS_OP_CONV_BWD && ops[k].out[1]) rc = dw_issue(ops[k]);
        if (rc != WSIS_OK) {
          first_err = rc;
          break;
        }
        i = i1 - 1;
        goto op_done;
      }
    }
#endif
    {
    const wsis_op& op = ops[i];
    const bool is_bn = op.kind == WSIS_OP_BN_RELU || op.kind == WSIS_OP_BN_RELU_BWD;
    std::optional<ProfScope> bn_prof;
    if (is_bn && g_prof_on) bn_prof.emplace(2, st);
    switch (op.kind) {
      case WSIS_OP_CONV:
        if (op.flags & (WSIS_OPF_BN_IN | WSIS_OPF_STAT_FIN)) {
#if !WSIS_EXPERIMENTAL
          rc = fail(WSIS_ERR_ARG, "op %d: the fused BatchNorm forms of the convolution are in the EXPERIMENTAL build only", i);
          break;
#else
          if (wt_off[i] < 0) {
            rc = fail(WSIS_ERR_ARG, "op %d: fused BatchNorm requested from a convolution that is not on wsis_spconv_fwd_t", i);
            break;
          }
          wsis_bn_in bi;
          bi.mean = (const float*)op.in[6];
          bi.var = (const float*)op.in[7];
          bi.gamma = (const float*)op.in[8];
          bi.beta = (const float*)op.in[9];
          bi.eps = op.eps;
          bi.relu = (op.flags & WSIS_OPF_RELU) ? 1 : 0;
          wsis_stat_target tg[2];
          int nt = 0;
          if (op.flags & WSIS_OPF_STAT_FIN) {
            tg[0].mean = (float*)op.out[2];
            tg[0].var = (float*)op.out[3];
            tg[0].running_mean = (float*)const_cast<void*>(op.in[10]);
            tg[0].running_var = (float*)const_cast<void*>(op.in[11]);
            tg[0].momentum = op.momentum;
            tg[0].reserved = 0;
            nt = 1;
            if (op.out[4]) {
              tg[1].mean = (float*)op.out[4];
              tg[1].var = (float*)op.out[5];
              tg[1].running_mean = (float*)op.out[6];
              tg[1].running_var = (float*)op.out[7];
              tg[1].momentum = op.momentum2;
              tg[1].reserved = 0;
              nt = 2;
            }
          }
          rc = wsis_spconv_fwd_f((const float*)op.in[0], (op.flags & WSIS_OPF_BN_IN) ? &bi : nullptr, (const int32_t*)op.in[1],
                                 (const int32_t*)op.in[2], reinterpret_cast<const float*>(wt_base + wt_off[i]), 0,
                                 (const float*)op.in[4], (const float*)op.in[5], (float*)op.out[0],
                                 (op.flags & WSIS_OPF_STATS) ? (float*)op.out[1] : nullptr, tg, nt, op.M_in, op.M_out, op.K,
                                 op.Cin, op.Cout, ws, ws_bytes, sync_slot(d_sync, i), stream);
          break;
#endif
        }
        if (wt_off[i] >= 0)
          rc = wsis_spconv_fwd_t((const float*)op.in[0], (const int32_t*)op.in[1], (const int32_t*)op.in[2],
                                 reinterpret_cast<const float*>(wt_base + wt_off[i]), 0, (const float*)op.in[4],
                                 (const float*)op.in[5], (float*)op.out[0],
                                 (op.flags & WSIS_OPF_STATS) ? (float*)op.out[1] : nullptr, op.M_in, op.M_out, op.K,
                                 op.Cin, op.Cout, ws, ws_bytes, sync_slot(d_sync, i), stream);
        else if (op.flags & WSIS_OPF_STATS)
          rc = fail(WSIS_ERR_ARG, "op %d: statistics requested from a convolution that is not on wsis_spconv_fwd_t", i);
        else
          rc = wsis_spconv_fwd((const float*)op.in[0], (const int32_t*)op.in[1], (const int32_t*)op.in[2],
                               (const float*)op.in[3], (const float*)op.in[4], (const float*)op.in[5],
                               (float*)op.out[0], op.M_in, op.M_out, op.K, op.Cin, op.Cout, ws, ws_bytes, stream);
        break;
      case WSIS_OP_BN_RELU: {
        const float* mean = (const float*)op.out[1];
        const float* var = (const float*)op.out[2];
        if (op.flags & WSIS_OPF_TRAINING) {
          const bool upd = (op.flags & WSIS_OPF_UPDATE_RUNNING) != 0;
          float* rm = upd ? (float*)op.in[3] : nullptr;
          float* rv = upd ? (float*)op.in[4] : nullptr;
          if ((op.flags & WSIS_OPF_STATS) && op.M_in > 0) {
            const int64_t n_part = (op.M_in + 31) / 32;
            const int C0 = op.in[6] ? op.K : op.Cin;
            if (!op.in[6] && op.out[0]) {
              rc = wsis_bn_stats_finalize_apply((const float*)op.in[5], n_part, op.M_in, op.Cin, (float*)op.out[1],
                                                (float*)op.out[2], rm, rv, op.momentum, (const float*)op.in[0],
                                                (const float*)op.in[1], (const float*)op.in[2], op.eps,
                                                (op.flags & WSIS_OPF_RELU) ? 1 : 0, (float*)op.out[0], ws, ws_bytes,
                                                sync_slot(d_sync, i), stream);
              break;
            }
            rc = wsis_bn_stats_finalize((const float*)op.in[5], n_part, op.M_in, C0, (float*)op.out[1],
                                        (float*)op.out[2], rm, rv, op.momentum, ws, ws_bytes, sync_slot(d_sync, i), stream);
            if (rc == WSIS_OK && op.in[6])
              rc = wsis_bn_stats_finalize((const float*)op.in[6], n_part, op.M_in, op.Cin - C0, (float*)op.out[1] + C0,
                                          (float*)op.out[2] + C0, rm ? rm + C0 : nullptr, rv ? rv + C0 : nullptr,
                                          op.momentum, ws, ws_bytes, sync_slot(d_sync, i), stream);
          } else {
            rc = wsis_bn_stats((const float*)op.in[0], op.M_in, op.Cin, (float*)op.out[1], (float*)op.out[2], rm, rv,
                               op.momentum, ws, ws_bytes, stream);
          }
          if (rc != WSIS_OK) break;
        } else {
          mean = (const float*)op.in[3];
          var = (const float*)op.in[4];
        }
        if (!op.out[0]) break;
        rc = wsis_bn_apply((const float*)op.in[0], mean, var, (const float*)op.in[1], (const float*)op.in[2], op.eps,
                           (op.flags & WSIS_OPF_RELU) ? 1 : 0, (float*)op.out[0], op.M_in, op.Cin, stream);
        break;
      }
      case WSIS_OP_CAT:
        if (op.M_in > 0) {
          if (vec4_ok(op, op.in[0], op.in[1], op.out[0]))
            hipLaunchKernelGGL(cat_rows_kernel<4>, dim3(grid_for(op.M_in * (op.Cin + op.Cout) / 4, 256)), dim3(256), 0,
                               st, (const float*)op.in[0], (const float*)op.in[1], (float*)op.out[0], op.M_in, op.Cin,
                               op.Cout);
          else
            hipLaunchKernelGGL(cat_rows_kernel<1>, dim3(grid_for(op.M_in * (op.Cin + op.Cout), 256)), dim3(256), 0, st,
                               (const float*)op.in[0], (const float*)op.in[1], (float*)op.out[0], op.M_in, op.Cin,
                               op.Cout);
          RUN_LAUNCH_CHECK();
        }
        break;
      case WSIS_OP_SPLIT:
        if (op.M_in > 0) {
          if (vec4_ok(op, op.in[0], op.out[0], op.out[1]))
            hipLaunchKernelGGL(split_rows_kernel<4>, dim3(grid_for(op.M_in * (op.Cin + op.Cout) / 4, 256)), dim3(256),
                               0, st, (const float*)op.in[0], (float*)op.out[0], (float*)op.out[1], op.M_in, op.Cin,
                               op.Cout);
          else
            hipLaunchKernelGGL(split_rows_kernel<1>, dim3(grid_for(op.M_in * (op.Cin + op.Cout), 256)), dim3(256), 0, st,
                               (const float*)op.in[0], (float*)op.out[0], (float*)op.out[1], op.M_in, op.Cin, op.Cout);
          RUN_LAUNCH_CHECK();
        }
        break;
      case WSIS_OP_ADD:
        if (op.M_in * op.Cin > 0) {
          hipLaunchKernelGGL(add_inplace_kernel, dim3(grid_for(op.M_in * op.Cin, 256)), dim3(256), 0, st,
                             (float*)op.out[0], (const float*)op.in[0], op.M_in * op.Cin);
          RUN_LAUNCH_CHECK();
        }
        break;
      case WSIS_OP_CONV_BWD: {
        char* rest = ws;
        const int64_t rest_bytes = ws_bytes;
        bool dw_forked = false;
        if (dw_early && op.out[1] && op.out[0] && side) {
          rc = dw_issue(op);
          dw_forked = true;
          if (rc != WSIS_OK) break;
        }
        if (op.out[0]) {
          if (wt_off[i] >= 0 && (op.flags & WSIS_OPF_STATS)) {
            rc = fail(WSIS_ERR_ARG, "op %d: BatchNorm partials requested from a dIn pass that is not on wsis_spconv_fwd_t", i);
            break;
          }
          if (wt_off[i] >= 0) {
            const float* WT = reinterpret_cast<const float*>(wt_base + wt_off[i]);
            rc = wsis_spconv_fwd((const float*)op.in[2], (const int32_t*)op.in[5], (const int32_t*)op.in[6], WT, nullptr,
                                 nullptr, (float*)op.out[0], op.M_out, op.M_in, op.K, op.Cout, op.Cin, rest, rest_bytes,
                                 stream);
          } else if (op.flags & WSIS_OPF_STATS) {
            const wsis_op* bn = nullptr;
            for (int j = i + 1; j < n && j <= i + 4 && !bn; ++j)
              if (ops[j].kind == WSIS_OP_BN_RELU_BWD && ops[j].in[1] == op.out[0] && (ops[j].flags & WSIS_OPF_STATS))
                bn = &ops[j];
            if (!bn || !bn->in[7] || bn->M_in != op.M_in || bn->Cin != op.Cin) {
              rc = fail(WSIS_ERR_ARG, "op %d: no BatchNorm backward takes the partials of this dIn pass", i);
              break;
            }
            if (!slab_bn_partials && wsis_spconv_fwd_t_slabs(op.M_in, op.K, op.Cout, op.Cin) > 1) {
              bn_unfused[bn - ops] = 1;
              rc = wsis_spconv_fwd_t((const float*)op.in[2], (const int32_t*)op.in[5], (const int32_t*)op.in[6],
                                     (const float*)op.in[1], (op.flags & WSIS_OPF_FLIP) ? 1 : 0, nullptr, nullptr,
                                     (float*)op.out[0], nullptr, op.M_out, op.M_in, op.K, op.Cout, op.Cin, rest,
                                     rest_bytes, sync_slot(d_sync, i), stream);
              if (rc != WSIS_OK) break;
              goto din_done;
            }
            rc = wsis_spconv_fwd_t_bn((const float*)op.in[2], (const int32_t*)op.in[5], (const int32_t*)op.in[6],
                                      (const float*)op.in[1], (op.flags & WSIS_OPF_FLIP) ? 1 : 0, (float*)op.out[0],
                                      (float*)const_cast<void*>(bn->in[7]), (const float*)bn->in[0],
                                      (const float*)bn->in[2], (const float*)bn->in[3], (const float*)bn->in[4],
                                      (const float*)bn->in[5], bn->eps, (bn->flags & WSIS_OPF_RELU) ? 1 : 0, op.M_out,
                                      op.M_in, op.K, op.Cout, op.Cin, rest, rest_bytes, sync_slot(d_sync, i), stream);
          } else {
            rc = wsis_spconv_fwd_t((const float*)op.in[2], (const int32_t*)op.in[5], (const int32_t*)op.in[6],
                                   (const float*)op.in[1], (op.flags & WSIS_OPF_FLIP) ? 1 : 0, nullptr, nullptr,
                                   (float*)op.out[0], nullptr, op.M_out, op.M_in, op.K, op.Cout, op.Cin, rest, rest_bytes,
                                   sync_slot(d_sync, i), stream);
          }
          if (rc != WSIS_OK) break;
        }
      din_done:
        if (op.out[1] && !dw_forked) {
          if (tail_main && side && dw_tail_on_main(ops, n, i)) {
            rc = issue_dw(op, ws, ws_bytes, stream, nullptr);
          } else {
            rc = dw_issue(op);
          }
        }
        break;
      }
      case WSIS_OP_BN_RELU_BWD:
        if ((op.flags & WSIS_OPF_STATS) && !bn_unfused[i]) {
          if (!op.in[7] || !(op.flags & WSIS_OPF_TRAINING)) {
            rc = fail(WSIS_ERR_ARG, "op %d: BatchNorm backward from partials needs in[7] and training mode", i);
            break;
          }
          rc = wsis_bn_bwd_from_partials((const float*)op.in[7], (op.M_in + 31) / 32, (const float*)op.in[0],
                                         (const float*)op.in[1], (const float*)op.in[2], (const float*)op.in[3],
                                         (const float*)op.in[4], (const float*)op.in[5], op.eps,
                                         (op.flags & WSIS_OPF_RELU) ? 1 : 0, (float*)op.out[0], (float*)op.out[1],
                                         (float*)op.out[2], (const float*)op.in[6], op.M_in, op.Cin, ws, ws_bytes,
                                         sync_slot(d_sync, i), stream);
          break;
        }
        rc = wsis_bn_bwd((const float*)op.in[0], (const float*)op.in[1], (const float*)op.in[2], (const float*)op.in[3],
                         (const float*)op.in[4], (const float*)op.in[5], op.eps, (op.flags & WSIS_OPF_RELU) ? 1 : 0,
                         (op.flags & WSIS_OPF_TRAINING) ? 1 : 0, (float*)op.out[0], (float*)op.out[1], (float*)op.out[2],
                         (const float*)op.in[6], op.M_in, op.Cin, ws, ws_bytes, stream);
        break;
      default:
        rc = fail(WSIS_ERR_ARG, "wsis_run_ops: unknown op kind");
    }
    if (bn_prof) bn_prof->stop();
    }
    if (rc != WSIS_OK) {
      first_err = rc;
      break;
    }
#if WSIS_EXPERIMENTAL
  op_done:
#endif
    if (i == mark_op) {
      SideStream* ms = side ? side : side_stream_for(st);
      {
        int wrc = dw_flush();
        if (wrc == WSIS_OK) wrc = drain_worker();
        if (wrc != WSIS_OK) {
          first_err = wrc;
          break;
        }
      }
      hipError_t e = ms ? hipEventRecord(ms->mark_main, st) : hipErrorOutOfMemory;
      if (e == hipSuccess) e = hipStreamWaitEvent(as_stream(waiter_stream), ms->mark_main, 0);
      if (e == hipSuccess && forked) {
        e = hipEventRecord(ms->mark_side, side->stream);
        if (e == hipSuccess) e = hipStreamWaitEvent(as_stream(waiter_stream), ms->mark_side, 0);
      }
      if (e != hipSuccess) {
        first_err = fail(WSIS_ERR_HIP, "wsis_run_ops: milestone failed: %s", hipGetErrorString(e));
        break;
      }
    }
  }
#undef RUN_LAUNCH_CHECK
  {
    int wrc = first_err == WSIS_OK ? dw_flush() : WSIS_OK;
    if (wrc != WSIS_OK && first_err == WSIS_OK) first_err = wrc;
    wrc = drain_worker();
    if (wrc != WSIS_OK && first_err == WSIS_OK) first_err = wrc;
  }
  if (defer_join && first_err == WSIS_OK) {
    if (forked) side->pending_join = true;
    return WSIS_OK;
  }
  if (!forked && !side && dw_stream_enabled()) {
    SideStream* s2 = side_stream_for(st);
    if (s2 && s2->pending_join) {
      side = s2;
      forked = true;
    }
  } else if (side && side->pending_join) {
    forked = true;
  }
  if (forked) {
    side->pending_join = false;
    const hipError_t e1 = hipEventRecord(side->join, side->stream);
    const hipError_t e2 = e1 == hipSuccess ? hipStreamWaitEvent(st, side->join, 0) : e1;
    if (e2 != hipSuccess && first_err == WSIS_OK)
      return fail(WSIS_ERR_HIP, "side-stream join failed: %s", hipGetErrorString(e2));
  }
  return first_err;
}

#if WSIS_EXPERIMENTAL
int wsis_debug_deep_phases(int32_t which, int32_t* info, double* us, int32_t cap) {
  if (which < 0 || which >= (int)g_deep_log.size()) return -1;
  const auto& rec = g_deep_log[which];
  const int n = (int)rec.first.size();
  if (n > cap) return -1;
  std::vector<unsigned long long> t(n + 1);
  if (hipDeviceSynchronize() != hipSuccess) return -1;
  if (hipMemcpy(t.data(), rec.second, (n + 1) * sizeof(unsigned long long), hipMemcpyDeviceToHost) != hipSuccess) return -1;
  for (int i = 0; i < n; ++i) {
    const DeepOp& d = rec.first[i];
    info[i * 8 + 0] = d.kind;
    info[i * 8 + 1] = d.NW;
    info[i * 8 + 2] = d.ZS;
    info[i * 8 + 3] = (int32_t)(d.kind == DK_CONV || d.kind == DK_REDUCE ? d.M_out : d.M_in);
    info[i * 8 + 4] = d.Cin;
    info[i * 8 + 5] = d.Cout;
    info[i * 8 + 6] = d.K;
    info[i * 8 + 7] = (int32_t)d.M_in;
    us[i] = (double)(t[i + 1] - t[i]) * 0.01;
  }
  return n;
}

#endif

}
```

3d-wsis_amd/model/unet_native.py:

```python
import os

import numpy as np
import torch
from torch import nn
from torch.autograd import Function

import wsis_native as _n
import wsis_ops
from spconv import ops as sp_ops

OP_CONV, OP_BN_RELU, OP_CAT, OP_SPLIT, OP_ADD, OP_CONV_BWD, OP_BN_RELU_BWD = 1, 2, 3, 4, 5, 6, 7
F_RELU, F_TRAINING, F_UPDATE, F_FLIP, F_STATS, F_BN_IN, F_STAT_FIN = 1, 2, 4, 8, 16, 32, 64
N_IN, N_OUT = 12, 8

OP_DTYPE = np.dtype([("kind", "<i4"), ("flags", "<i4"), ("M_in", "<i8"), ("M_out", "<i8"), ("K", "<i4"),
                     ("Cin", "<i4"), ("Cout", "<i4"), ("reserved", "<i4"), ("eps", "<f4"), ("momentum", "<f4"),
                     ("momentum2", "<f4"), ("reserved2", "<f4"), ("inp", "<u8", (N_IN,)), ("out", "<u8", (N_OUT,))])
assert OP_DTYPE.itemsize == 216

_FWD = 1 << 62
_BWD = 1 << 61
_PAR = 1 << 60
_TBL = 1 << 59
_EXT = 1 << 58
_TAGS = (_FWD, _BWD, _PAR, _TBL, _EXT)
_ID_MASK = (1 << 32) - 1
_OFF_SHIFT = 32
_OFF_MASK = (1 << 26) - 1


def _at(handle, floats):
    if floats == 0 or handle == 0:
        return handle
    if any(handle & t for t in _TAGS):
        return handle + (int(floats) << _OFF_SHIFT)
    return handle + 4 * int(floats)


def _fuse_fin_enabled():
    on = os.environ.get("WSIS_FUSE_BN_FIN", "0") != "0"
    if on:
        _n.require_experimental("WSIS_FUSE_BN_FIN (statistics finished inside the convolution)")
    return on


def _fuse_apply_level():
    v = os.environ.get("WSIS_FUSE_BN_APPLY", "")
    lvl = int(v) if v.lstrip("-").isdigit() else 99
    if lvl < 99:
        _n.require_experimental("WSIS_FUSE_BN_APPLY (BatchNorm applied by the consuming convolution)")
    return lvl


def _fuse_stats_enabled():
    return os.environ.get("WSIS_FUSE_BN_STATS", "1") != "0"


def _lvl(level):
    return -(level + 1)


class _Recorder(object):

    def __init__(self, tag, align=256):
        self.tag, self.align = tag, align
        self.rows = []
        self.alloc_level, self.alloc_mult, self.alloc_slices = [], [], []

    def alloc(self, level, mult, per_slice=False):
        self.alloc_level.append(level)
        self.alloc_mult.append(int(mult))
        self.alloc_slices.append(bool(per_slice))
        return self.tag | (len(self.alloc_level) - 1)

    def op(self, kind, flags=0, M_in=0, M_out=0, K=0, Cin=0, Cout=0, eps=0.0, momentum=0.0, inp=(), out=()):
        inp = list(inp) + [0] * (N_IN - len(inp))
        out = list(out) + [0] * (N_OUT - len(out))
        self.rows.append([kind, flags, M_in, M_out, K, Cin, Cout, eps, momentum, inp, out, 0.0])
        return len(self.rows) - 1


class _Arena(object):

    def __init__(self, rec):
        self.level = np.asarray(rec.alloc_level, dtype=np.int64)
        self.mult = np.asarray(rec.alloc_mult, dtype=np.int64)
        self.slices = np.asarray(rec.alloc_slices, dtype=bool)
        self.align = rec.align

    def layout(self, Mvec):
        if len(self.level) == 0:
            return np.zeros(0, dtype=np.int64), 0
        rows = np.where(self.level >= 0, Mvec[np.maximum(self.level, 0)], 1)
        rows = np.where(self.slices, (rows + 31) // 32, rows)
        size = (rows * self.mult * 4 + self.align - 1) // self.align * self.align
        end = np.cumsum(size)
        return end - size, int(end[-1])


class _Template(object):

    def __init__(self, rec):
        n = len(rec.rows)
        self.arr = np.zeros(n, dtype=OP_DTYPE)
        ptr = np.zeros((n, N_IN + N_OUT), dtype=np.uint64)
        m_in = np.zeros(n, dtype=np.int64)
        m_out = np.zeros(n, dtype=np.int64)
        for i, r in enumerate(rec.rows):
            self.arr[i] = (r[0], r[1], 0, 0, r[4], r[5], r[6], 0, r[7], r[8], r[11], 0, 0, 0)
            m_in[i], m_out[i] = r[2], r[3]
            ptr[i, :N_IN] = r[9]
            ptr[i, N_IN:] = r[10]
        self.m_in_lit, self.m_out_lit = np.maximum(m_in, 0), np.maximum(m_out, 0)
        self.m_in_lvl, self.m_out_lvl = np.maximum(-m_in - 1, 0), np.maximum(-m_out - 1, 0)
        self.m_in_sym, self.m_out_sym = m_in < 0, m_out < 0
        flat = ptr.reshape(-1)
        self.static = flat.copy()
        self.patch = {}
        for tag in _TAGS:
            pos = np.nonzero((flat & np.uint64(tag)) != 0)[0]
            off = ((flat[pos] >> np.uint64(_OFF_SHIFT)) & np.uint64(_OFF_MASK)) * np.uint64(4)
            self.patch[tag] = (pos, (flat[pos] & np.uint64(_ID_MASK)).astype(np.int64), off)
            self.static[pos] = 0

    def instantiate(self, Mvec, luts):
        arr = self.arr.copy()
        arr["M_in"] = np.where(self.m_in_sym, Mvec[self.m_in_lvl], self.m_in_lit)
        arr["M_out"] = np.where(self.m_out_sym, Mvec[self.m_out_lvl], self.m_out_lit)
        flat = self.static.copy()
        for tag, (pos, idx, off) in self.patch.items():
            if len(pos):
                flat[pos] = luts[tag][idx] + off
        ptr = flat.reshape(-1, N_IN + N_OUT)
        arr["inp"] = ptr[:, :N_IN]
        arr["out"] = ptr[:, N_IN:]
        return arr


def _ptr(t):
    return 0 if t is None else t.data_ptr()


class _Table(object):

    def __init__(self, nbr_f=0, order_f=0, nbr_b=0, order_b=0, flip=0):
        self.nbr_f, self.order_f, self.nbr_b, self.order_b, self.flip = nbr_f, order_f, nbr_b, order_b, flip


def _subm(l):
    return _Table(_TBL | (l * 6), _TBL | (l * 6 + 1), _TBL | (l * 6), _TBL | (l * 6 + 1), 1)


def _down(l):
    return _Table(_TBL | (l * 6 + 2), _TBL | (l * 6 + 3), _TBL | (l * 6 + 4), _TBL | (l * 6 + 5), 0)


def _up(l):
    return _Table(_TBL | (l * 6 + 4), _TBL | (l * 6 + 5), _TBL | (l * 6 + 2), _TBL | (l * 6 + 3), 0)


class _Compiled(object):
    pass


class UNetProgram(object):

    def __init__(self, net):
        self.net = net
        self.params = [p for m in (net.input_conv, net.unet, net.output_layer) for p in m.parameters()]
        self.bns = [m for mod in (net.unet, net.output_layer) for m in mod.modules() if isinstance(m, nn.BatchNorm1d)]
        self.flat_grad, self.flat_params = None, []
        self.flat_tail = None
        self.tail_floats = 0
        self.overlap = None
        self._garena = None
        self.persistent_grads = os.environ.get("WSIS_PERSISTENT_GRADS", "1") != "0"
        self.bn_sync = None
        self._cache = {}

    def _conv(self, rec, x, conv, table, lvl_in, lvl_out, residual=0, stats=True):
        K = int(np.prod(conv.kernel_size))
        Cin, Cout = conv.in_channels, conv.out_channels
        W = conv.weight
        assert conv.bias is None, "the UNet convolutions carry no bias (sparse_unet3d.py)"
        y = rec.alloc(lvl_out, Cout)
        t = table if table is not None else _Table()
        part = 0
        if stats and self._fuse_stats and sp_ops._use_fwd2(K, Cin, Cout):
            part = rec.alloc(lvl_out, 2 * Cout, per_slice=True)
        v = self._virt.get(x)
        flags, eps, bn_in = (F_STATS if part else 0), 0.0, (0, 0, 0, 0)
        if v is not None:
            assert sp_ops._use_fwd2(K, Cin, Cout) and v["C"] == Cin
            x = v["x"]
            flags |= F_BN_IN | (F_RELU if v["relu"] else 0)
            eps, bn_in = v["eps"], (v["mean"], v["var"], v["gamma"], v["beta"])
        row = rec.op(OP_CONV, flags, _lvl(lvl_in), _lvl(lvl_out), K, Cin, Cout, eps=eps,
                     inp=(x, t.nbr_f, t.order_f, W.data_ptr(), 0, residual) + bn_in, out=(y, part))
        if part:
            self._stats_src[y] = [(part, Cout, row)]
        self._acc_f.append(("spconv_fwd_kernel", t.nbr_f, lvl_out, Cin, Cout))

        def bwd(recb, dy, need_dx=True):
            dx = recb.alloc(lvl_in, Cin) if need_dx else 0
            dW = self._grad_handle(W)
            bflags = (F_FLIP if t.flip else 0) | ((F_BN_IN | (F_RELU if v["relu"] else 0)) if v is not None else 0)
            recb.op(OP_CONV_BWD, bflags, _lvl(lvl_in), _lvl(lvl_out), K, Cin, Cout, eps=eps,
                    inp=(x, W.data_ptr(), dy, t.nbr_f, t.order_f, t.nbr_b, t.order_b) + bn_in, out=(dx, dW))
            if need_dx:
                self._acc_b.append(("spconv_fwd_kernel", t.nbr_b, lvl_in, Cout, Cin))
            self._acc_b.append(("spconv_dw_kernel", t.nbr_f, lvl_out, Cin, Cout))
            return dx
        return y, bwd

    def _bn_relu(self, rec, x, bn, lvl, relu=True, fuse=False):
        C = bn.num_features
        training = bn.training or not bn.track_running_stats
        update = bn.training and bn.track_running_stats
        flags = (F_RELU if relu else 0) | (F_TRAINING if training else 0) | (F_UPDATE if update else 0)
        if update and bn.num_batches_tracked is not None:
            assert bn.momentum is not None, "cumulative-average BatchNorm is not used by 3D-WSIS"
            self._count.append(bn)
        fuse = fuse and lvl >= self._fuse_apply_lvl and self._fuse_stats and C % 32 == 0
        momentum = bn.momentum if bn.momentum is not None else 0.1
        mean = rec.alloc(-1, C) if training else bn.running_mean.data_ptr()
        var = rec.alloc(-1, C) if training else bn.running_var.data_ptr()
        src = self._stats_src.get(x) if training else None
        have_parts = src is not None and sum(c for _, c, _ in src) == C and len(src) <= 2
        stats_done = False
        if have_parts and self._fuse_fin and lvl >= self._fuse_fin_lvl and all(rec.rows[r][10][4] == 0 for _, _, r in src):
            c0 = 0
            rm = _ptr(bn.running_mean) if update else 0
            rv = _ptr(bn.running_var) if update else 0
            for _, c, r in src:
                row = rec.rows[r]
                tgt = (_at(mean, c0), _at(var, c0), _at(rm, c0), _at(rv, c0))
                if not (row[1] & F_STAT_FIN):
                    row[1] |= F_STAT_FIN
                    row[10][2], row[10][3], row[9][10], row[9][11] = tgt
                    row[8] = momentum
                else:
                    row[10][4:8] = tgt
                    row[11] = momentum
                c0 += c
            stats_done = True
        y = rec.alloc(lvl, 0 if fuse else C)
        if fuse:
            self._virt[y] = dict(x=x, C=C, mean=mean, var=var, gamma=_ptr(bn.weight), beta=_ptr(bn.bias), eps=bn.eps,
                                 relu=relu)
        if training and not stats_done:
            K0, parts, sflags = 0, (0, 0), flags
            if have_parts:
                sflags |= F_STATS
                K0 = src[0][1]
                parts = (src[0][0], src[1][0] if len(src) == 2 else 0)
            rec.op(OP_BN_RELU, sflags, _lvl(lvl), _lvl(lvl), K0, C, C, bn.eps, momentum,
                   inp=(x, _ptr(bn.weight), _ptr(bn.bias), _ptr(bn.running_mean), _ptr(bn.running_var), parts[0], parts[1]),
                   out=(0 if fuse else y, mean, var))
            self._acc_f.append(("bn_op", 0, lvl, C, (0 if fuse else 2) + (0 if have_parts else 1)))
        elif not fuse:
            rec.op(OP_BN_RELU, flags & ~(F_TRAINING | F_UPDATE), _lvl(lvl), _lvl(lvl), 0, C, C, bn.eps, momentum,
                   inp=(x, _ptr(bn.weight), _ptr(bn.bias), mean, var), out=(y,))
            self._acc_f.append(("bn_op", 0, lvl, C, 2))

        def bwd(recb, dy, addend=0):
            dx = recb.alloc(lvl, C)
            dg = self._grad_handle(bn.weight) if bn.weight is not None else recb.alloc(-1, C)
            db = self._grad_handle(bn.bias) if bn.bias is not None else recb.alloc(-1, C)
            recb.op(OP_BN_RELU_BWD, flags & ~F_STATS, _lvl(lvl), _lvl(lvl), 0, C, C, bn.eps, 0.0,
                    inp=(x, dy, mean, var, _ptr(bn.weight), _ptr(bn.bias), addend), out=(dx, dg, db))
            self._acc_b.append(("bn_op", 0, lvl, C, 3 + (1 if addend else 0)))
            return dx
        return y, bwd

    def _fuse_bn_bwd(self, recb):
        if os.environ.get("WSIS_FUSE_BN_BWD", "1") == "0" or not self._fuse_stats:
            return
        rows = recb.rows
        for i, r in enumerate(rows):
            if r[0] != OP_CONV_BWD or not r[10][0]:
                continue
            K, Cin, Cout = r[4], r[5], r[6]
            if not sp_ops._use_fwd2(K, Cout, Cin):
                continue
            dx = r[10][0]
            for j in range(i + 1, min(i + 5, len(rows))):
                b = rows[j]
                if b[0] == OP_BN_RELU_BWD and b[9][1] == dx and (b[1] & F_TRAINING) and b[5] == Cin and b[2] == r[2]:
                    lvl = -b[2] - 1
                    b[9][7] = recb.alloc(lvl, 2 * Cin, per_slice=True)
                    b[1] |= F_STATS
                    r[1] |= F_STATS
                    break

    def _residual_block(self, rec, x, blk, lvl):
        seq = blk.conv_branch
        bn1, conv1, bn2, conv2 = seq[0], seq[2], seq[3], seq[5]
        table = _subm(lvl)
        a1, b_bn1 = self._bn_relu(rec, x, bn1, lvl, fuse=True)
        z1, b_c1 = self._conv(rec, a1, conv1, table, lvl, lvl)
        a2, b_bn2 = self._bn_relu(rec, z1, bn2, lvl, fuse=True)
        first = blk.i_branch[0]
        if isinstance(first, nn.Identity):
            res, b_i = x, None
        else:
            res, b_i = self._conv(rec, x, first, None, lvl, lvl, stats=False)
        out, b_c2 = self._conv(rec, a2, conv2, table, lvl, lvl, residual=res)

        def bwd(recb, d_out):
            d_a2 = b_c2(recb, d_out)
            d_z1 = b_bn2(recb, d_a2)
            d_a1 = b_c1(recb, d_z1)
            d_skip = d_out if b_i is None else b_i(recb, d_out)
            return b_bn1(recb, d_a1, addend=d_skip)
        return out, bwd

    def _ublock(self, rec, x, ub, lvl):
        bwds = []
        for blk in ub.blocks:
            x, b = self._residual_block(rec, x, blk, lvl)
            bwds.append(b)
        if len(ub.nPlanes) == 1:
            def bwd_leaf(recb, d):
                for b in reversed(bwds):
                    d = b(recb, d)
                return d
            return x, bwd_leaf
        C0 = ub.nPlanes[0]
        identity = x
        a, b_bn = self._bn_relu(rec, x, ub.conv[0], lvl, fuse=True)
        d, b_down = self._conv(rec, a, ub.conv[2], _down(lvl), lvl, lvl + 1)
        u, b_u = self._ublock(rec, d, ub.u, lvl + 1)
        a2, b_bn2 = self._bn_relu(rec, u, ub.deconv[0], lvl + 1, fuse=True)
        up, b_up = self._conv(rec, a2, ub.deconv[2], _up(lvl), lvl + 1, lvl)
        cat = rec.alloc(lvl, 2 * C0)
        rec.op(OP_CAT, 0, _lvl(lvl), _lvl(lvl), 0, C0, C0, inp=(identity, up), out=(cat,))
        if identity in self._stats_src and up in self._stats_src:
            self._stats_src[cat] = self._stats_src[identity] + self._stats_src[up]
        x = cat
        tails = []
        for blk in ub.blocks_tail:
            x, b = self._residual_block(rec, x, blk, lvl)
            tails.append(b)

        def bwd(recb, dcur):
            for b in reversed(tails):
                dcur = b(recb, dcur)
            d_id = recb.alloc(lvl, C0)
            d_up = recb.alloc(lvl, C0)
            recb.op(OP_SPLIT, 0, _lvl(lvl), _lvl(lvl), 0, C0, C0, inp=(dcur,), out=(d_id, d_up))
            d_a2 = b_up(recb, d_up)
            d_u = b_bn2(recb, d_a2)
            d_d = b_u(recb, d_u)
            d_a = b_down(recb, d_d)
            d_x = b_bn(recb, d_a, addend=d_id)
            for b in reversed(bwds):
                d_x = b(recb, d_x)
            return d_x
        return x, bwd

    def _grad_handle(self, p):
        h = self._grad.get(id(p))
        if h is None:
            h = self._prec.alloc(-1, p.numel())
            self._grad[id(p)] = h
        return h

    def _mode_key(self, need_dx):
        return (need_dx, self.bn_sync is not None, _fuse_stats_enabled(), _fuse_fin_enabled(), _fuse_apply_level(),
                os.environ.get("WSIS_FUSE_BN_FIN_LVL", "0"),
                os.environ.get("WSIS_FWD2", "1"), tuple(bn.training for bn in self.bns), tuple(p.data_ptr() for p in self.params),
                tuple(bn.running_mean.data_ptr() if bn.running_mean is not None else 0 for bn in self.bns))

    def compiled(self, need_dx):
        key = self._mode_key(need_dx)
        c = self._cache.get(key)
        if c is not None:
            return c
        if len(self._cache) > 8:
            self._cache.clear()
        net = self.net
        c = _Compiled()
        rec, recb = _Recorder(_FWD), _Recorder(_BWD)
        self._prec, self._grad = _Recorder(_PAR, align=16), {}
        self._acc_f, self._acc_b, self._count = [], [], []
        self._stats_src, self._fuse_stats = {}, _fuse_stats_enabled()
        self._virt, self._fuse_apply_lvl = {}, _fuse_apply_level()
        self._fuse_fin = _fuse_fin_enabled() and self._fuse_stats
        self._fuse_fin_lvl = int(os.environ.get("WSIS_FUSE_BN_FIN_LVL", "0"))
        if self.bn_sync is not None:
            self._fuse_fin, self._fuse_apply_lvl = False, 99
        y, b_in = self._conv(rec, _EXT | 0, net.input_conv[0], _subm(0), 0, 0)
        y, b_u = self._ublock(rec, y, net.unet, 0)
        out, b_out = self._bn_relu(rec, y, net.output_layer[0], 0)
        d = b_out(recb, _EXT | 1)
        d = b_u(recb, d)
        dx = b_in(recb, d, need_dx)
        self._fuse_bn_bwd(recb)
        c.fwd, c.bwd = _Template(rec), _Template(recb)
        c.fwd_arena, c.bwd_arena, c.par_arena = _Arena(rec), _Arena(recb), _Arena(self._prec)
        c.out_id, c.dx_id = out & _ID_MASK, (dx & _ID_MASK) if need_dx else -1
        c.grad_ids = [(self._grad[id(p)] & _ID_MASK) if id(p) in self._grad else -1 for p in self.params]
        c.acc_f, c.acc_b, c.count = self._acc_f, self._acc_b, self._count
        done = np.zeros(len(recb.rows), dtype=np.int64)
        hw = 0
        for i, r in enumerate(recb.rows):
            for h in r[10]:
                if h & _PAR:
                    hw = max(hw, (h & _ID_MASK) + 1)
            done[i] = hw
        c.bwd_grads_done = done
        c.out_channels = net.output_layer[0].num_features
        self._cache[key] = c
        return c

    def bind(self, tensor):
        net = self.net
        sp_ops.prebuild_unet_rulebooks(tensor, net.blocks)
        L = net.blocks
        self.Mvec = np.zeros(L, dtype=np.int64)
        self.table_lut = np.zeros(L * 6, dtype=np.uint64)
        self.table_tensors = [None] * (L * 6)
        pyr = getattr(tensor.indice_dict, "pyramid", None)
        if pyr is not None and pyr.n_levels == L:
            lay, base = pyr.layout, np.uint64(pyr.base)
            self.Mvec[:] = lay[:, sp_ops.PYR_ROWS]
            fields = (sp_ops.PYR_SUBM_NBR_P, sp_ops.PYR_SUBM_ORDER, sp_ops.PYR_DOWN_NBR_P, sp_ops.PYR_DOWN_ORDER,
                      sp_ops.PYR_UP_NBR_P, sp_ops.PYR_UP_ORDER)
            off = lay[:, fields]
            self.table_lut[:] = np.where(off >= 0, off.astype(np.uint64) + base, np.uint64(0)).reshape(-1)
            self.table_tensors = _LazyTables(tensor.indice_dict, L)
            self.keep = [tensor.indice_dict]
            return
        for lvl in range(L):
            rb = tensor.indice_dict["subm%d" % (lvl + 1)]
            self.Mvec[lvl] = rb.in_indices.shape[0]
            ts = [rb.nbr_p, rb.order, None, None, None, None]
            if lvl + 1 < L:
                rd = tensor.indice_dict["spconv%d" % (lvl + 1)]
                ts[2:] = [rd.nbr_p, rd.order, rd.nbr_up_p, rd.order_up]
            for j, t in enumerate(ts):
                self.table_lut[lvl * 6 + j] = _ptr(t)
                self.table_tensors[lvl * 6 + j] = t
        self.keep = [tensor.indice_dict]

    def account(self, entries, Mvec, tensors):
        prof = sp_ops.PROFILER
        if prof is None:
            return
        for name, nbr, lvl, Cin, Cout in entries:
            if name == "bn_op":
                M = int(Mvec[lvl])
                prof.end(name, None, M * Cin * Cout * 4, 0, (M, Cin, Cout, M))
                continue
            t = tensors[nbr & _ID_MASK] if nbr else None
            P = prof.pairs(t, int(Mvec[lvl]))
            prof.end(name, None, P * (Cin + Cout) * 4 + P * 8, 2 * P * Cin * Cout, (int(Mvec[lvl]), Cin, Cout, P))


class _LazyTables(object):

    def __init__(self, indice_dict, L):
        self.d, self.L = indice_dict, L

    def __getitem__(self, i):
        lvl, slot = divmod(int(i), 6)
        if slot < 2:
            rb = self.d["subm%d" % (lvl + 1)]
            return (rb.nbr_p, rb.order)[slot]
        rd = self.d["spconv%d" % (lvl + 1)]
        return (rd.nbr_p, rd.order, rd.nbr_up_p, rd.order_up)[slot - 2]


def _arena_tensor(nbytes, device, zero=False):
    make = torch.zeros if zero else torch.empty
    t = make(nbytes + 256, dtype=torch.uint8, device=device)
    return t, (t.data_ptr() + 255) // 256 * 256


def _view(arena, base, offset, shape):
    numel = int(np.prod(shape))
    off = base + int(offset) - arena.data_ptr()
    return arena[off:off + numel * 4].view(torch.float32).view(shape)


class _GradArena(object):

    @staticmethod
    def key_of(prog, c, ptotal, tail, dev):
        return (id(c), int(ptotal), int(tail), dev, tuple(p.requires_grad for p in prog.params))

    def __init__(self, prog, c, poffs, ptotal, tail, dev):
        self.key = self.key_of(prog, c, ptotal, tail, dev)
        self.c = c
        self.arena, self.base = _arena_tensor(ptotal + tail, dev, zero=True)
        self.flat = self.arena.view(torch.float32)
        self.first = (self.base - self.arena.data_ptr()) // 4
        self.lut = poffs.astype(np.uint64) + np.uint64(self.base)
        self.params, self.views = [], []
        for i, p in enumerate(prog.params):
            gid = c.grad_ids[i]
            if gid >= 0 and p.requires_grad:
                off = self.first + int(poffs[gid]) // 4
                self.params.append(p)
                self.views.append(self.flat[off:off + p.numel()].view(p.shape))
        t0 = self.first + (ptotal + 3) // 4
        self.tail = self.flat[t0:t0 + prog.tail_floats] if prog.tail_floats else None


class UNetFunction(Function):

    @staticmethod
    def forward(ctx, x, prog, anchor=None):
        _n.require_cuda(x)
        x = x if (x.dtype == torch.float32 and x.is_contiguous()) else x.contiguous().float()
        need_dx = bool(x.requires_grad)
        c = prog.compiled(need_dx)
        for bn in c.count:
            wsis_ops._defer_batch_count(bn)
        Mvec, table_lut, tensors = prog.Mvec, prog.table_lut, prog.table_tensors
        offs, total = c.fwd_arena.layout(Mvec)
        arena, base = _arena_tensor(total, x.device)
        fwd_lut = offs.astype(np.uint64) + np.uint64(base)
        none = fwd_lut[:0]
        luts = {_FWD: fwd_lut, _TBL: table_lut, _EXT: np.array([x.data_ptr(), 0], dtype=np.uint64), _BWD: none,
                _PAR: none}
        sy = prog.bn_sync.new_pass() if prog.bn_sync is not None else None
        if sy is not None:
            sy.arenas = [arena]
            _run_synced(_n.hip(), c.fwd.instantiate(Mvec, luts), x.device, sy)
        else:
            _run(_n.hip(), c.fwd.instantiate(Mvec, luts), x.device)
        ctx.sy = sy
        if not (torch.is_grad_enabled() and (need_dx or anchor is not None)):
            sp_ops.verify_pending_counts()
        prog.account(c.acc_f, Mvec, tensors)
        out = _view(arena, base, offs[c.out_id], (int(Mvec[0]), c.out_channels))
        ctx.prog, ctx.c, ctx.arena, ctx.fwd_lut, ctx.x = prog, c, arena, fwd_lut, x
        ctx.Mvec, ctx.table_lut, ctx.tensors, ctx.keep = Mvec, table_lut, tensors, prog.keep
        return out

    @staticmethod
    def backward(ctx, d_out):
        prog, c, Mvec = ctx.prog, ctx.c, ctx.Mvec
        d_out = d_out if (d_out.dtype == torch.float32 and d_out.is_contiguous()) else d_out.contiguous().float()
        dev = d_out.device
        boffs, btotal = c.bwd_arena.layout(Mvec)
        poffs, ptotal = c.par_arena.layout(Mvec)
        garena, gbase = _arena_tensor(btotal, dev)
        tail = int(prog.tail_floats) * 4
        ga = prog._garena
        if ga is None or ga.key != _GradArena.key_of(prog, c, ptotal, tail, dev):
            ga = prog._garena = _GradArena(prog, c, poffs, ptotal, tail, dev)
        if not prog.persistent_grads or any(p.grad is not None for p in ga.params):
            ga = _GradArena(prog, c, poffs, ptotal, tail, dev)
        parena, pflat, first = ga.arena, ga.flat, ga.first
        luts = {_FWD: ctx.fwd_lut, _BWD: boffs.astype(np.uint64) + np.uint64(gbase), _PAR: ga.lut, _TBL: ctx.table_lut,
                _EXT: np.array([ctx.x.data_ptr(), d_out.data_ptr()], dtype=np.uint64)}
        hook = prog.overlap
        if ctx.sy is not None:
            ctx.sy.arenas = [ctx.arena, garena, parena]
            _run_synced(_n.hip(), c.bwd.instantiate(Mvec, luts), dev, ctx.sy)
        elif hook is not None and hook.ready() and len(poffs) > 1:
            starts = np.append(poffs, ptotal)
            want = ptotal // 2
            op_i = int(np.searchsorted(starts[c.bwd_grads_done], want))
            op_i = min(op_i, len(c.bwd_grads_done) - 2)
            split = int(starts[c.bwd_grads_done[op_i]]) // 4
            _run(_n.hip(), c.bwd.instantiate(Mvec, luts), dev, mark_op=op_i, waiter=hook.comm_stream_ptr())
            hook.early(pflat[first:first + split], first + split)
        else:
            _run(_n.hip(), c.bwd.instantiate(Mvec, luts), dev)
        prog.account(c.acc_b, Mvec, ctx.tensors)
        for p, v in zip(ga.params, ga.views):
            p.grad = v if p.grad is None else p.grad + v
        prog.flat_grad, prog.flat_params, prog.flat_tail = pflat, ga.params, ga.tail
        dx = _view(garena, gbase, boffs[c.dx_id], tuple(ctx.x.shape)) if c.dx_id >= 0 else None
        sp_ops.verify_pending_counts()
        return dx, None, None



class _BnSync(object):

    def __init__(self, prog, group):
        self.group = group
        self.by_ptr = {}
        for bn in prog.bns:
            for t in (bn.running_mean, bn.running_var):
                if t is not None:
                    self.by_ptr[t.data_ptr()] = t
        self.counts = {}
        self.arenas = []

    def new_pass(self):
        p = _BnSync.__new__(_BnSync)
        p.group, p.by_ptr, p.counts, p.arenas = self.group, self.by_ptr, {}, []
        return p

    def view(self, ptr, numel):
        ptr = int(ptr)
        for a in self.arenas:
            base = a.data_ptr()
            if base <= ptr < base + a.numel():
                return a[ptr - base:ptr - base + 4 * numel].view(torch.float32)
        raise _n.WsisError("synced BatchNorm: pointer outside the pass's arenas")


def _bn_fwd_synced(lib, op, sy, dev, st, slot):
    import torch.distributed as dist
    M, C, flags = int(op["M_in"]), int(op["Cin"]), int(op["flags"])
    inp, out = [int(v) for v in op["inp"]], [int(v) for v in op["out"]]
    mom, eps = float(op["momentum"]), float(op["eps"])
    mean, var = sy.view(out[1], C), sy.view(out[2], C)
    if M > 0 and (flags & F_STATS):
        n_part = (M + 31) // 32
        C0 = int(op["K"]) if inp[6] else C
        wsb = lib.wsis_bn_stats_finalize_workspace_bytes(n_part, C)
        ws = torch.empty(wsb, dtype=torch.uint8, device=dev)
        _n.check(lib.wsis_bn_stats_finalize(inp[5], n_part, M, C0, out[1], out[2], None, None, mom, _n.ptr(ws), wsb, slot, st),
                 "bn_stats_finalize")
        if inp[6]:
            _n.check(lib.wsis_bn_stats_finalize(inp[6], n_part, M, C - C0, out[1] + 4 * C0, out[2] + 4 * C0, None, None, mom,
                                                _n.ptr(ws), wsb, slot, st), "bn_stats_finalize")
    elif M > 0:
        wsb = lib.wsis_bn_workspace_bytes(M, C)
        ws = torch.empty(wsb, dtype=torch.uint8, device=dev)
        _n.check(lib.wsis_bn_stats(inp[0], M, C, out[1], out[2], None, None, mom, _n.ptr(ws), wsb, st), "bn_stats")
    else:
        mean.zero_()
        var.zero_()
    t = torch.cat((mean.double(), var.double(), torch.full((1,), float(M), dtype=torch.float64, device=dev)))
    parts = [torch.empty_like(t) for _ in range(dist.get_world_size(sy.group))]
    dist.all_gather(parts, t, group=sy.group)
    g = torch.stack(parts)
    n_i = g[:, 2 * C:2 * C + 1]
    N = n_i.sum()
    mean64 = (g[:, :C] * n_i).sum(0) / N
    dm = g[:, :C] - mean64
    var64 = ((g[:, C:2 * C] + dm * dm) * n_i).sum(0) / N
    mean.copy_(mean64.float())
    var.copy_(var64.float())
    if flags & F_UPDATE:
        rm, rv = sy.by_ptr[inp[3]], sy.by_ptr[inp[4]]
        unb = var64 * (N / (N - 1.0).clamp_min(1.0))
        rm.mul_(1.0 - mom).add_(mean, alpha=mom)
        rv.mul_(1.0 - mom).add_(unb.float(), alpha=mom)
    sy.counts[out[1]] = N
    if out[0] and M > 0:
        _n.check(lib.wsis_bn_apply(inp[0], out[1], out[2], inp[1] or None, inp[2] or None, eps, 1 if flags & F_RELU else 0,
                                   out[0], M, C, st), "bn_apply")


def _bn_bwd_synced(lib, op, sy, dev, st):
    import torch.distributed as dist
    M, C, flags = int(op["M_in"]), int(op["Cin"]), int(op["flags"])
    inp, out = [int(v) for v in op["inp"]], [int(v) for v in op["out"]]
    eps, relu = float(op["eps"]), 1 if flags & F_RELU else 0
    dg, db = sy.view(out[1], C), sy.view(out[2], C)
    if M > 0:
        wsb = lib.wsis_bn_workspace_bytes(M, C)
        ws = torch.empty(wsb, dtype=torch.uint8, device=dev)
        _n.check(lib.wsis_bn_bwd(inp[0], inp[1], inp[2], inp[3], inp[4] or None, inp[5] or None, eps, relu, 1, None, out[1],
                                 out[2], None, M, C, _n.ptr(ws), wsb, st), "bn_bwd")
    else:
        dg.zero_()
        db.zero_()
    g = torch.cat((dg, db)).double()
    dist.all_reduce(g, group=sy.group)
    N = sy.counts[inp[2]]
    if M > 0:
        sc = (g * (float(M) / N)).float()
        _n.check(lib.wsis_bn_bwd_apply(inp[0], inp[1], inp[2], inp[3], inp[4] or None, inp[5] or None, _n.ptr(sc[:C]),
                                       _n.ptr(sc[C:]), eps, relu, out[0], inp[6] or None, M, C, st), "bn_bwd_apply")


def _run_synced(lib, ops, device, sy):
    n = len(ops)
    base, item = ops.ctypes.data, ops.dtype.itemsize
    kinds = ops["kind"]
    bwd_pair = (kinds == OP_CONV_BWD) | (kinds == OP_BN_RELU_BWD)
    ops["flags"] = np.where(bwd_pair, ops["flags"] & ~F_STATS, ops["flags"])
    flags = ops["flags"]
    is_bn = ((kinds == OP_BN_RELU) | (kinds == OP_BN_RELU_BWD)) & ((flags & F_TRAINING) != 0)
    sync = _n.ptr(_n.sync_block(device))
    st = _n.stream_ptr()
    keep = []
    try:
        i = 0
        while i < n:
            j = i
            while j < n and not is_bn[j]:
                j += 1
            if j > i:
                p = base + i * item
                wsb = lib.wsis_run_ops_workspace_bytes(p, j - i)
                if wsb < 0:
                    raise _n.WsisError("run_ops workspace query failed")
                ws = torch.empty(wsb, dtype=torch.uint8, device=device)
                keep.append(ws)
                _n.check(lib.wsis_run_ops_part(p, j - i, _n.ptr(ws), wsb, sync, st, 0), "run_ops_part")
            if j < n:
                if int(kinds[j]) == OP_BN_RELU:
                    _bn_fwd_synced(lib, ops[j], sy, device, st, sync)
                else:
                    _bn_bwd_synced(lib, ops[j], sy, device, st)
                j += 1
            i = j
    finally:
        _n.check(lib.wsis_run_ops_part(None, 0, None, 0, sync, st, 1), "run_ops_part")
    return keep


def _run(lib, ops, device, mark_op=-1, waiter=None):
    n = len(ops)
    p = ops.ctypes.data
    ws_bytes = lib.wsis_run_ops_workspace_bytes(p, n)
    if ws_bytes < 0:
        raise _n.WsisError("run_ops workspace query failed")
    ws = torch.empty(ws_bytes, dtype=torch.uint8, device=device)
    sync = _n.ptr(_n.sync_block(device))
    if mark_op >= 0:
        _n.check(lib.wsis_run_ops_marked(p, n, _n.ptr(ws), ws_bytes, sync, _n.stream_ptr(), int(mark_op), waiter),
                 "run_ops")
    else:
        _n.check(lib.wsis_run_ops(p, n, _n.ptr(ws), ws_bytes, sync, _n.stream_ptr()), "run_ops")


_EXPERIMENTAL_SWITCHES = ("WSIS_DEEP", "WSIS_FWD2P", "WSIS_RING", "WSIS_GRAPH", "WSIS_BN_FUSED_APPLY", "WSIS_BN_FUSED_FWD", "WSIS_BN_FUSED_BWD")


TUNE_KNOBS = (
    "WSIS_BN_APPLY_PT", "WSIS_BN_FUSED_GRID", "WSIS_BN_TICKET", "WSIS_DW2", "WSIS_DW2_HI", "WSIS_DW2_LO",
    "WSIS_DW2_WAVES", "WSIS_DW2_XCD", "WSIS_DW2_XSH", "WSIS_DW2_DENSE_WG", "WSIS_DW2_RED", "WSIS_DW2_PFLOOR", "WSIS_DW_BAL", "WSIS_DW_H16", "WSIS_DW_DIV", "WSIS_DW_THREAD", "WSIS_FWD2P_MIN",
    "WSIS_FWD2_BD", "WSIS_FWD2_DA_NW4", "WSIS_FWD2_DEAL", "WSIS_FWD2_NOSLAB", "WSIS_FWD2_NW", "WSIS_FWD2_NW_MAX",
    "WSIS_FWD2_NW_MAX_NOSLAB", "WSIS_FWD2_RG", "WSIS_FWD2_RGH", "WSIS_FWD2_RGH_LATE", "WSIS_FWD2_SNAKE",
    "WSIS_FWD2_TR", "WSIS_FWD2_TR_DA", "WSIS_FWD2_WAVES", "WSIS_FWD2_XCD", "WSIS_FWD2_ZS", "WSIS_FWD_NB_SMALL",
    "WSIS_FWD_SMALL_TILES", "WSIS_KSPLIT_TARGET", "WSIS_SL_BLOCKS", "WSIS_TILE_BAND", "WSIS_TILE_SCHED",
    "WSIS_TILE_SCHED_MIN", "WSIS_XCD_AWARE")
_WARNED_KNOBS = set()
_KNOB_SCAN = [0]


def _check_experimental_switches():
    for k in _EXPERIMENTAL_SWITCHES:
        if os.environ.get(k, "0") not in ("", "0"):
            _n.require_experimental(k + "=" + os.environ[k])
    _KNOB_SCAN[0] += 1
    if _KNOB_SCAN[0] > 4 and _KNOB_SCAN[0] % 64:
        return
    ignored = [k for k in TUNE_KNOBS if k in os.environ and k not in _WARNED_KNOBS]
    if ignored and not _n.experimental():
        import warnings
        _WARNED_KNOBS.update(ignored)
        warnings.warn("tuning knob(s) %s are set but the DEFAULT libwsis_hip.so is loaded: they are live in the "
                      "EXPERIMENTAL build only (make -C 3d-wsis_amd/csrc EXPERIMENTAL=1) and have no effect here"
                      % ", ".join(ignored), RuntimeWarning, stacklevel=2)


def run_unet(net, input_tensor, sync_group=None):
    _check_experimental_switches()
    prog = getattr(net, "_native_prog", None)
    if prog is None:
        prog = UNetProgram(net)
        net._native_prog = prog
    if sync_group is None:
        prog.bn_sync = None
    elif prog.bn_sync is None or prog.bn_sync.group is not sync_group:
        prog.bn_sync = _BnSync(prog, sync_group)
    prog.bind(input_tensor)
    anchor = next((p for p in prog.params if p.requires_grad), None) if torch.is_grad_enabled() else None
    return UNetFunction.apply(input_tensor.features, prog, anchor)
```

Measured before the change: 134.2.

## Fuse U-block skip-gradient split into the first tail BatchNorm backward

In the U-block backward pass, the first tail BatchNorm backward can now write its dx directly into two separate buffers, the identity half and the upsample half, using a column cut. This removes the separate OP_SPLIT pass that read and rewrote the full gradient tensor. The apply kernels gain a SPLIT template variant that computes per-element destination addresses. The deep fused conv/BN paths are disabled for split ops, which could lose some fusion for those layers.

```diff
diff --git a/3d-wsis_amd/csrc/bn.hip b/3d-wsis_amd/csrc/bn.hip
--- a/3d-wsis_amd/csrc/bn.hip
+++ b/3d-wsis_amd/csrc/bn.hip
@@ -558,13 +558,14 @@
   }
 }
 
-template <bool COHERENT>
+template <bool COHERENT, bool SPLIT = false>
 __device__ __forceinline__ void bn_bwd_apply_body(const float* __restrict__ x, const float* __restrict__ dy,
                                                   const float* __restrict__ mean, const float* __restrict__ var,
                                                   const float* __restrict__ gamma, const float* __restrict__ beta,
                                                   const float* dgamma, const float* dbeta,
                                                   const float* __restrict__ addend, float eps, int relu, int training,
-                                                  float* __restrict__ dx, int64_t M, int C) {
+                                                  float* __restrict__ dx, int64_t M, int C,
+                                                  float* __restrict__ dx2 = nullptr, int cs = 0) {
   const int64_t total = M * C;
   const float inv_m = 1.0f / (float)M;
   const bool vec = (C & 3) == 0;
@@ -590,6 +591,16 @@
     }
   };
   if (t < totalw) coef((int)(t % Cw) * W);
+  auto split_dst = [&](int64_t r, int c) -> float* {
+    return c < cs ? dx + r * cs + c : dx2 + r * (C - cs) + (c - cs);
+  };
+  const int64_t rstep = SPLIT ? stride / Cw : 0;
+  int64_t srow = 0;
+  int scol = 0;
+  if (SPLIT && t < totalw) {
+    srow = t / Cw;
+    scol = (int)(t - srow * Cw) * W;
+  }
   auto one = [&](const float (&xv)[4], const float (&dv)[4], const float (&av)[4], float (&ov)[4]) {
 #pragma unroll
     for (int e = 0; e < 4; ++e) {
@@ -619,12 +630,22 @@
       float o0[4], o1[4];
       one(tx0.v, td0.v, ta0.v, o0);
       one(tx1.v, td1.v, ta1.v, o1);
-      reinterpret_cast<float4*>(dx)[t] = make_float4(o0[0], o0[1], o0[2], o0[3]);
-      reinterpret_cast<float4*>(dx)[u] = make_float4(o1[0], o1[1], o1[2], o1[3]);
+      if (SPLIT) {
+        *reinterpret_cast<float4*>(split_dst(srow, scol)) = make_float4(o0[0], o0[1], o0[2], o0[3]);
+        *reinterpret_cast<float4*>(split_dst(srow + rstep, scol)) = make_float4(o1[0], o1[1], o1[2], o1[3]);
+        srow += 2 * rstep;
+      } else {
+        reinterpret_cast<float4*>(dx)[t] = make_float4(o0[0], o0[1], o0[2], o0[3]);
+        reinterpret_cast<float4*>(dx)[u] = make_float4(o1[0], o1[1], o1[2], o1[3]);
+      }
     }
   }
   for (; t < totalw; t += stride) {
     if (!fixed_c) coef((int)(t % Cw) * W);
+    if (SPLIT && !fixed_c) {
+      srow = t / Cw;
+      scol = (int)(t - srow * Cw) * W;
+    }
     float xv[4], dv[4], av[4] = {0.f, 0.f, 0.f, 0.f}, ov[4];
     if (vec) {
       const f4 tx = ld4(x + t * 4, true), td = ld4(dy + t * 4, true);
@@ -644,27 +665,35 @@
       if (addend) av[0] = addend[t];
     }
     one(xv, dv, av, ov);
-    if (vec)
+    if (SPLIT) {
+      *reinterpret_cast<float4*>(split_dst(srow, scol)) = make_float4(ov[0], ov[1], ov[2], ov[3]);
+      srow += rstep;
+    } else if (vec) {
       reinterpret_cast<float4*>(dx)[t] = make_float4(ov[0], ov[1], ov[2], ov[3]);
-    else
+    } else {
       dx[t] = ov[0];
-  }
-}
-
+    }
+  }
+}
+
+template <bool SPLIT>
 __global__ void bn_bwd_apply_kernel(const float* __restrict__ x, const float* __restrict__ dy,
                                     const float* __restrict__ mean, const float* __restrict__ var,
                                     const float* __restrict__ gamma, const float* __restrict__ beta,
                                     const float* __restrict__ dgamma, const float* __restrict__ dbeta,
                                     const float* __restrict__ addend, float eps, int relu, int training,
-                                    float* __restrict__ dx, int64_t M, int C) {
-  bn_bwd_apply_body<false>(x, dy, mean, var, gamma, beta, dgamma, dbeta, addend, eps, relu, training, dx, M, C);
-}
-
+                                    float* __restrict__ dx, int64_t M, int C, float* __restrict__ dx2, int cs) {
+  bn_bwd_apply_body<false, SPLIT>(x, dy, mean, var, gamma, beta, dgamma, dbeta, addend, eps, relu, training, dx, M, C,
+                                  dx2, cs);
+}
+
+template <bool SPLIT>
 __global__ __launch_bounds__(256) void bn_bwd_finish_apply_kernel(
     const float* __restrict__ partial, int nblk, int C, double* __restrict__ chunk, int G, float* dbeta, float* dgamma,
     SyncSlot* __restrict__ sync, const float* __restrict__ x, const float* __restrict__ dy, const float* __restrict__ mean,
     const float* __restrict__ var, const float* __restrict__ gamma, const float* __restrict__ beta,
-    const float* __restrict__ addend, float eps, int relu, float* __restrict__ dx, int64_t M) {
+    const float* __restrict__ addend, float eps, int relu, float* __restrict__ dx, int64_t M, float* __restrict__ dx2,
+    int cs) {
   __shared__ double red[2][8][33];
   __shared__ int s_last;
   const int CG = (C + 31) / 32;
@@ -678,7 +707,7 @@
     }
   }
   bn_wait_published(sync);
-  bn_bwd_apply_body<true>(x, dy, mean, var, gamma, beta, dgamma, dbeta, addend, eps, relu, 1, dx, M, C);
+  bn_bwd_apply_body<true, SPLIT>(x, dy, mean, var, gamma, beta, dgamma, dbeta, addend, eps, relu, 1, dx, M, C, dx2, cs);
 }
 
 constexpr int BN_SF_ROWS = 256;
@@ -778,11 +807,12 @@
   }
 }
 
+template <bool SPLIT>
 __global__ __launch_bounds__(256) void bn_small_bwd_finish_apply_kernel(
     const float* __restrict__ partial, int nblk, int C, int64_t M, const float* __restrict__ x,
     const float* __restrict__ dy, const float* __restrict__ mean, const float* __restrict__ var,
     const float* __restrict__ gamma, const float* __restrict__ beta, const float* __restrict__ addend, float eps, int relu,
-    float* __restrict__ dx, float* __restrict__ dgamma, float* __restrict__ dbeta, int G) {
+    float* __restrict__ dx, float* __restrict__ dgamma, float* __restrict__ dbeta, int G, float* __restrict__ dx2, int cs) {
   __shared__ double red[2][8][33];
   __shared__ float s_k1[32], s_k2[32];
   const int cgi = blockIdx.y;
@@ -864,7 +894,8 @@
         ov[e] = gm[e] * rstd[e] * rr;
         if (addend) ov[e] += av[e];
       }
-      *reinterpret_cast<float4*>(dx + r * C + c4) = make_float4(ov[0], ov[1], ov[2], ov[3]);
+      float* const o = !SPLIT ? dx + r * C + c4 : c4 < cs ? dx + r * cs + c4 : dx2 + r * (C - cs) + (c4 - cs);
+      *reinterpret_cast<float4*>(o) = make_float4(ov[0], ov[1], ov[2], ov[3]);
     }
   }
 }
@@ -1280,8 +1311,94 @@
                               float eps, int32_t relu, float* d_dx, float* d_dgamma, float* d_dbeta,
                               const float* d_addend, int64_t M, int32_t C, void* d_ws, int64_t ws_bytes, void* d_sync,
                               void* stream) {
+  return wsis::bn_bwd_from_partials_split(d_partials, n_part, d_x, d_dy, d_mean, d_var, d_gamma, d_beta, eps, relu, d_dx,
+                                          nullptr, 0, d_dgamma, d_dbeta, d_addend, M, C, d_ws, ws_bytes, d_sync, stream);
+}
+
+int wsis_bn_bwd_apply(const float* d_x, const float* d_dy, const float* d_mean, const float* d_var,
+                      const float* d_gamma, const float* d_beta, const float* d_sum_dz_xhat, const float* d_sum_dz,
+                      float eps, int32_t relu, float* d_dx, const float* d_addend, int64_t M, int32_t C, void* stream) {
+  WSIS_REQUIRE(M >= 1 && C >= 1 && d_x && d_dy && d_mean && d_var && d_sum_dz_xhat && d_sum_dz && d_dx, "bad args");
+  const int64_t work = (C & 3) == 0 ? (M * C) >> 2 : M * C;
+  const int cw = (C & 3) == 0 ? C >> 2 : C;
+  const int grid = bn_apply_grid(work, cw, 2);
+  hipLaunchKernelGGL(bn_bwd_apply_kernel<false>, dim3(grid), dim3(256), 0, as_stream(stream), d_x, d_dy, d_mean, d_var,
+                     d_gamma, d_beta, d_sum_dz_xhat, d_sum_dz, d_addend, eps, relu, 1, d_dx, M, C, nullptr, 0);
+  WSIS_LAUNCH_CHECK();
+  return WSIS_OK;
+}
+
+int wsis_bn_bwd(const float* d_x, const float* d_dy, const float* d_mean, const float* d_var,
+                const float* d_gamma, const float* d_beta, float eps, int32_t relu, int32_t training,
+                float* d_dx, float* d_dgamma, float* d_dbeta, const float* d_addend, int64_t M, int32_t C, void* d_ws,
+                int64_t ws_bytes, void* stream) {
+  return wsis::bn_bwd_split(d_x, d_dy, d_mean, d_var, d_gamma, d_beta, eps, relu, training, d_dx, nullptr, 0, d_dgamma,
+                            d_dbeta, d_addend, M, C, d_ws, ws_bytes, stream);
+}
+
+int64_t wsis_sync_bytes(void) { return (int64_t)kSyncSlotsTotal * (int64_t)sizeof(SyncSlot); }
+
+int64_t wsis_colsum_workspace_bytes(int64_t M, int32_t C) {
+  if (M < 0 || C < 4) return -1;
+  int64_t per = (M + 127) / 128;
+  if (per < 256) per = 256;
+  const int64_t G = (M + per - 1) / per;
+  return (G > 1 ? G : 1) * (int64_t)C * (int64_t)sizeof(float) + 256;
+}
+
+int wsis_colsum(const float* d_x, int64_t M, int32_t C, float* d_out, void* d_ws, int64_t ws_bytes, void* d_sync,
+                void* stream) {
+  WSIS_REQUIRE(M >= 0 && C >= 4 && C % 4 == 0 && C <= 1024 && d_out, "colsum: C must be a multiple of 4, <= 1024");
+  hipStream_t st = as_stream(stream);
+  if (M == 0) {
+    WSIS_HIP_CHECK(hipMemsetAsync(d_out, 0, sizeof(float) * (size_t)C, st));
+    return WSIS_OK;
+  }
+  WSIS_REQUIRE(d_x && (reinterpret_cast<uintptr_t>(d_x) & 15) == 0 && (reinterpret_cast<uintptr_t>(d_out) & 15) == 0,
+               "colsum: 16-byte alignment");
+  int64_t per = (M + 127) / 128;
+  if (per < 256) per = 256;
+  const int64_t G = (M + per - 1) / per;
+  float* chunk = nullptr;
+  unsigned* ticket = nullptr;
+  if (G > 1) {
+    WSIS_REQUIRE(d_ws && ws_bytes >= wsis_colsum_workspace_bytes(M, C), "workspace too small");
+    chunk = reinterpret_cast<float*>((reinterpret_cast<uintptr_t>(d_ws) + 255) & ~(uintptr_t)255);
+    WSIS_REQUIRE(d_sync, "colsum over more than one chunk needs a sync slot");
+    ticket = static_cast<SyncSlot*>(d_sync)->ticket;
+  }
+  hipLaunchKernelGGL(colsum_kernel, dim3((unsigned)G), dim3(256), 0, st, d_x, M, (int)C, per, chunk, d_out, ticket);
+  WSIS_LAUNCH_CHECK();
+  return WSIS_OK;
+}
+
+}
+
+namespace wsis {
+
+static int check_split(const float* d_dx, const float* d_dx2, int c_split, int C) {
+  if (!d_dx2) {
+    WSIS_REQUIRE(c_split == 0, "BatchNorm backward: a column cut without a second dx");
+    return WSIS_OK;
+  }
+  WSIS_REQUIRE(d_dx && c_split > 0 && c_split < C && (c_split & 3) == 0 && (C & 3) == 0 &&
+                   (reinterpret_cast<uintptr_t>(d_dx) & 15) == 0 && (reinterpret_cast<uintptr_t>(d_dx2) & 15) == 0,
+               "BatchNorm backward: split dx needs C and the cut multiples of 4 and 16-byte aligned halves");
+  return WSIS_OK;
+}
+
+int bn_bwd_from_partials_split(const float* d_partials, int64_t n_part, const float* d_x, const float* d_dy,
+                               const float* d_mean, const float* d_var, const float* d_gamma, const float* d_beta, float eps,
+                               int32_t relu, float* d_dx, float* d_dx2, int32_t c_split, float* d_dgamma, float* d_dbeta,
+                               const float* d_addend, int64_t M, int32_t C, void* d_ws, int64_t ws_bytes, void* d_sync,
+                               void* stream) {
   WSIS_REQUIRE(M >= 1 && C >= 1 && d_partials && d_x && d_dy && d_mean && d_var && d_dgamma && d_dbeta, "bad args");
   WSIS_REQUIRE(n_part == (M + 31) / 32 && n_part < ((int64_t)1 << 31), "one partial per 32-row slice");
+  {
+    const int rc = check_split(d_dx, d_dx2, c_split, C);
+    if (rc != WSIS_OK) return rc;
+  }
+  const bool split = d_dx2 != nullptr;
   const int G = bn_fin_chunks(n_part);
   WSIS_REQUIRE(G == 1 || (d_ws && ws_bytes >= wsis_bn_stats_finalize_workspace_bytes(n_part, C)), "workspace too small");
   double* chunk = reinterpret_cast<double*>((reinterpret_cast<uintptr_t>(d_ws) + 255) & ~(uintptr_t)255);
@@ -1292,9 +1409,15 @@
       (reinterpret_cast<uintptr_t>(d_x) & 15) == 0 &&
       (reinterpret_cast<uintptr_t>(d_dy) & 15) == 0 && (reinterpret_cast<uintptr_t>(d_dx) & 15) == 0 &&
       (reinterpret_cast<uintptr_t>(d_addend) & 15) == 0) {
-    hipLaunchKernelGGL(bn_small_bwd_finish_apply_kernel, dim3((unsigned)ceil_div(M, BN_SF_ROWS), (unsigned)((C + 31) / 32)),
-                       dim3(256), 0, st, d_partials, (int)n_part, (int)C, M, d_x, d_dy, d_mean, d_var, d_gamma, d_beta,
-                       d_addend, eps, (int)relu, d_dx, d_dgamma, d_dbeta, G);
+    const dim3 grid((unsigned)ceil_div(M, BN_SF_ROWS), (unsigned)((C + 31) / 32));
+    if (split)
+      hipLaunchKernelGGL(bn_small_bwd_finish_apply_kernel<true>, grid, dim3(256), 0, st, d_partials, (int)n_part, (int)C, M,
+                         d_x, d_dy, d_mean, d_var, d_gamma, d_beta, d_addend, eps, (int)relu, d_dx, d_dgamma, d_dbeta, G,
+                         d_dx2, (int)c_split);
+    else
+      hipLaunchKernelGGL(bn_small_bwd_finish_apply_kernel<false>, grid, dim3(256), 0, st, d_partials, (int)n_part, (int)C,
+                         M, d_x, d_dy, d_mean, d_var, d_gamma, d_beta, d_addend, eps, (int)relu, d_dx, d_dgamma, d_dbeta, G,
+                         nullptr, 0);
     WSIS_LAUNCH_CHECK();
     return WSIS_OK;
   }
@@ -1302,9 +1425,14 @@
     const int CG = (C + 31) / 32;
     const int fgrid = tickets ? bn_fused_grid(M, C, G * CG, 1) : 0;
     if (fgrid > 0) {
-      hipLaunchKernelGGL(bn_bwd_finish_apply_kernel, dim3(fgrid), dim3(256), 0, st, d_partials, (int)n_part, (int)C, chunk, G,
-                         d_dbeta, d_dgamma, static_cast<SyncSlot*>(d_sync), d_x, d_dy, d_mean,
-                         d_var, d_gamma, d_beta, d_addend, eps, (int)relu, d_dx, M);
+      if (split)
+        hipLaunchKernelGGL(bn_bwd_finish_apply_kernel<true>, dim3(fgrid), dim3(256), 0, st, d_partials, (int)n_part, (int)C,
+                           chunk, G, d_dbeta, d_dgamma, static_cast<SyncSlot*>(d_sync), d_x, d_dy, d_mean, d_var, d_gamma,
+                           d_beta, d_addend, eps, (int)relu, d_dx, M, d_dx2, (int)c_split);
+      else
+        hipLaunchKernelGGL(bn_bwd_finish_apply_kernel<false>, dim3(fgrid), dim3(256), 0, st, d_partials, (int)n_part, (int)C,
+                           chunk, G, d_dbeta, d_dgamma, static_cast<SyncSlot*>(d_sync), d_x, d_dy, d_mean, d_var, d_gamma,
+                           d_beta, d_addend, eps, (int)relu, d_dx, M, nullptr, 0);
       WSIS_LAUNCH_CHECK();
       return WSIS_OK;
     }
@@ -1320,32 +1448,27 @@
     const int64_t work = (C & 3) == 0 ? (M * C) >> 2 : M * C;
     const int cw = (C & 3) == 0 ? C >> 2 : C;
     const int grid = bn_apply_grid(work, cw, 2);
-    hipLaunchKernelGGL(bn_bwd_apply_kernel, dim3(grid), dim3(256), 0, st, d_x, d_dy, d_mean, d_var, d_gamma, d_beta,
-                       d_dgamma, d_dbeta, d_addend, eps, relu, 1, d_dx, M, C);
+    if (split)
+      hipLaunchKernelGGL(bn_bwd_apply_kernel<true>, dim3(grid), dim3(256), 0, st, d_x, d_dy, d_mean, d_var, d_gamma, d_beta,
+                         d_dgamma, d_dbeta, d_addend, eps, relu, 1, d_dx, M, C, d_dx2, (int)c_split);
+    else
+      hipLaunchKernelGGL(bn_bwd_apply_kernel<false>, dim3(grid), dim3(256), 0, st, d_x, d_dy, d_mean, d_var, d_gamma,
+                         d_beta, d_dgamma, d_dbeta, d_addend, eps, relu, 1, d_dx, M, C, nullptr, 0);
     WSIS_LAUNCH_CHECK();
   }
   return WSIS_OK;
 }
 
-int wsis_bn_bwd_apply(const float* d_x, const float* d_dy, const float* d_mean, const float* d_var,
-                      const float* d_gamma, const float* d_beta, const float* d_sum_dz_xhat, const float* d_sum_dz,
-                      float eps, int32_t relu, float* d_dx, const float* d_addend, int64_t M, int32_t C, void* stream) {
-  WSIS_REQUIRE(M >= 1 && C >= 1 && d_x && d_dy && d_mean && d_var && d_sum_dz_xhat && d_sum_dz && d_dx, "bad args");
-  const int64_t work = (C & 3) == 0 ? (M * C) >> 2 : M * C;
-  const int cw = (C & 3) == 0 ? C >> 2 : C;
-  const int grid = bn_apply_grid(work, cw, 2);
-  hipLaunchKernelGGL(bn_bwd_apply_kernel, dim3(grid), dim3(256), 0, as_stream(stream), d_x, d_dy, d_mean, d_var, d_gamma,
-                     d_beta, d_sum_dz_xhat, d_sum_dz, d_addend, eps, relu, 1, d_dx, M, C);
-  WSIS_LAUNCH_CHECK();
-  return WSIS_OK;
-}
-
-int wsis_bn_bwd(const float* d_x, const float* d_dy, const float* d_mean, const float* d_var,
-                const float* d_gamma, const float* d_beta, float eps, int32_t relu, int32_t training,
-                float* d_dx, float* d_dgamma, float* d_dbeta, const float* d_addend, int64_t M, int32_t C, void* d_ws,
-                int64_t ws_bytes, void* stream) {
+int bn_bwd_split(const float* d_x, const float* d_dy, const float* d_mean, const float* d_var, const float* d_gamma,
+                 const float* d_beta, float eps, int32_t relu, int32_t training, float* d_dx, float* d_dx2, int32_t c_split,
+                 float* d_dgamma, float* d_dbeta, const float* d_addend, int64_t M, int32_t C, void* d_ws, int64_t ws_bytes,
+                 void* stream) {
   WSIS_REQUIRE(M >= 1 && C >= 1 && d_x && d_dy && d_mean && d_var && d_dgamma && d_dbeta && d_ws, "bad args");
   WSIS_REQUIRE(ws_bytes >= wsis_bn_workspace_bytes(M, C), "workspace too small");
+  {
+    const int rc = check_split(d_dx, d_dx2, c_split, C);
+    if (rc != WSIS_OK) return rc;
+  }
   const int Cp = (C + 3) / 4 * 4;
   const int nblk = bn_nblk(M, Cp);
   float* partial = static_cast<float*>(d_ws);
@@ -1366,47 +1489,15 @@
     const int64_t work = (C & 3) == 0 ? (M * C) >> 2 : M * C;
     const int cw = (C & 3) == 0 ? C >> 2 : C;
     const int grid = bn_apply_grid(work, cw, 2);
-    hipLaunchKernelGGL(bn_bwd_apply_kernel, dim3(grid), dim3(256), 0, st, d_x, d_dy, d_mean, d_var, d_gamma, d_beta,
-                       d_dgamma, d_dbeta, d_addend, eps, relu, training, d_dx, M, C);
+    if (d_dx2)
+      hipLaunchKernelGGL(bn_bwd_apply_kernel<true>, dim3(grid), dim3(256), 0, st, d_x, d_dy, d_mean, d_var, d_gamma, d_beta,
+                         d_dgamma, d_dbeta, d_addend, eps, relu, training, d_dx, M, C, d_dx2, (int)c_split);
+    else
+      hipLaunchKernelGGL(bn_bwd_apply_kernel<false>, dim3(grid), dim3(256), 0, st, d_x, d_dy, d_mean, d_var, d_gamma,
+                         d_beta, d_dgamma, d_dbeta, d_addend, eps, relu, training, d_dx, M, C, nullptr, 0);
     WSIS_LAUNCH_CHECK();
   }
   return WSIS_OK;
 }
 
-int64_t wsis_sync_bytes(void) { return (int64_t)kSyncSlotsTotal * (int64_t)sizeof(SyncSlot); }
-
-int64_t wsis_colsum_workspace_bytes(int64_t M, int32_t C) {
-  if (M < 0 || C < 4) return -1;
-  int64_t per = (M + 127) / 128;
-  if (per < 256) per = 256;
-  const int64_t G = (M + per - 1) / per;
-  return (G > 1 ? G : 1) * (int64_t)C * (int64_t)sizeof(float) + 256;
-}
-
-int wsis_colsum(const float* d_x, int64_t M, int32_t C, float* d_out, void* d_ws, int64_t ws_bytes, void* d_sync,
-                void* stream) {
-  WSIS_REQUIRE(M >= 0 && C >= 4 && C % 4 == 0 && C <= 1024 && d_out, "colsum: C must be a multiple of 4, <= 1024");
-  hipStream_t st = as_stream(stream);
-  if (M == 0) {
-    WSIS_HIP_CHECK(hipMemsetAsync(d_out, 0, sizeof(float) * (size_t)C, st));
-    return WSIS_OK;
-  }
-  WSIS_REQUIRE(d_x && (reinterpret_cast<uintptr_t>(d_x) & 15) == 0 && (reinterpret_cast<uintptr_t>(d_out) & 15) == 0,
-               "colsum: 16-byte alignment");
-  int64_t per = (M + 127) / 128;
-  if (per < 256) per = 256;
-  const int64_t G = (M + per - 1) / per;
-  float* chunk = nullptr;
-  unsigned* ticket = nullptr;
-  if (G > 1) {
-    WSIS_REQUIRE(d_ws && ws_bytes >= wsis_colsum_workspace_bytes(M, C), "workspace too small");
-    chunk = reinterpret_cast<float*>((reinterpret_cast<uintptr_t>(d_ws) + 255) & ~(uintptr_t)255);
-    WSIS_REQUIRE(d_sync, "colsum over more than one chunk needs a sync slot");
-    ticket = static_cast<SyncSlot*>(d_sync)->ticket;
-  }
-  hipLaunchKernelGGL(colsum_kernel, dim3((unsigned)G), dim3(256), 0, st, d_x, M, (int)C, per, chunk, d_out, ticket);
-  WSIS_LAUNCH_CHECK();
-  return WSIS_OK;
-}
-
-}
+}
diff --git a/3d-wsis_amd/csrc/common.h b/3d-wsis_amd/csrc/common.h
--- a/3d-wsis_amd/csrc/common.h
+++ b/3d-wsis_amd/csrc/common.h
@@ -168,6 +168,15 @@
                        unsigned* d_err, int64_t M_in, int64_t M_out, int K, int Cin, int Cout, hipEvent_t ka, hipEvent_t kb, hipStream_t st,
                        unsigned long long* d_dbg = nullptr);
 
+int bn_bwd_from_partials_split(const float* d_partials, int64_t n_part, const float* d_x, const float* d_dy,
+                               const float* d_mean, const float* d_var, const float* d_gamma, const float* d_beta, float eps,
+                               int32_t relu, float* d_dx, float* d_dx2, int32_t c_split, float* d_dgamma, float* d_dbeta,
+                               const float* d_addend, int64_t M, int32_t C, void* d_ws, int64_t ws_bytes, void* d_sync,
+                               void* stream);
+int bn_bwd_split(const float* d_x, const float* d_dy, const float* d_mean, const float* d_var, const float* d_gamma,
+                 const float* d_beta, float eps, int32_t relu, int32_t training, float* d_dx, float* d_dx2, int32_t c_split,
+                 float* d_dgamma, float* d_dbeta, const float* d_addend, int64_t M, int32_t C, void* d_ws, int64_t ws_bytes,
+                 void* stream);
 bool dw2_supported(int K, int Cin, int Cout);
 bool dw2_fits(int64_t M_in, int64_t M_out, int K, int Cin, int Cout);
 int64_t dw2_workspace_bytes(int64_t M_out, int K, int Cin, int Cout);
diff --git a/3d-wsis_amd/csrc/executor.hip b/3d-wsis_amd/csrc/executor.hip
--- a/3d-wsis_amd/csrc/executor.hip
+++ b/3d-wsis_amd/csrc/executor.hip
@@ -365,7 +365,7 @@
       if (!deep_conv_plan(op.M_in, op.K, op.Cout, op.Cin, &nw, &zs)) return false;
       if (op.flags & WSIS_OPF_STATS) {
         const int j = paired_bn(ops, n, i);
-        if (j < 0 || !ops[j].in[7] || ops[j].M_in != op.M_in || ops[j].Cin != op.Cin) return false;
+        if (j < 0 || !ops[j].in[7] || ops[j].M_in != op.M_in || ops[j].Cin != op.Cin || ops[j].out[3]) return false;
       }
       return aligned16(op.in[2]) && aligned16(op.out[0]);
     }
@@ -379,6 +379,7 @@
       }
       return aligned16(op.in[0]) && (!op.out[0] || aligned16(op.out[0]));
     case WSIS_OP_BN_RELU_BWD:
+      if (op.out[3]) return false;
       if (op.M_in < 1 || op.M_in > R || op.Cin % 32 || !deep_bn_rows_ok(op.M_in)) return false;
       if (!(op.flags & WSIS_OPF_TRAINING) || !(op.flags & WSIS_OPF_STATS) || !op.in[7]) return false;
       return aligned16(op.in[0]) && aligned16(op.in[1]) && aligned16(op.out[0]) && (!op.in[6] || aligned16(op.in[6]));
@@ -1156,18 +1157,20 @@
             rc = fail(WSIS_ERR_ARG, "op %d: BatchNorm backward from partials needs in[7] and training mode", i);
             break;
           }
-          rc = wsis_bn_bwd_from_partials((const float*)op.in[7], (op.M_in + 31) / 32, (const float*)op.in[0],
-                                         (const float*)op.in[1], (const float*)op.in[2], (const float*)op.in[3],
-                                         (const float*)op.in[4], (const float*)op.in[5], op.eps,
-                                         (op.flags & WSIS_OPF_RELU) ? 1 : 0, (float*)op.out[0], (float*)op.out[1],
-                                         (float*)op.out[2], (const float*)op.in[6], op.M_in, op.Cin, ws, ws_bytes,
-                                         sync_slot(d_sync, i), stream);
+          rc = bn_bwd_from_partials_split((const float*)op.in[7], (op.M_in + 31) / 32, (const float*)op.in[0],
+                                          (const float*)op.in[1], (const float*)op.in[2], (const float*)op.in[3],
+                                          (const float*)op.in[4], (const float*)op.in[5], op.eps,
+                                          (op.flags & WSIS_OPF_RELU) ? 1 : 0, (float*)op.out[0], (float*)op.out[3],
+                                          op.out[3] ? op.K : 0, (float*)op.out[1], (float*)op.out[2],
+                                          (const float*)op.in[6], op.M_in, op.Cin, ws, ws_bytes, sync_slot(d_sync, i),
+                                          stream);
           break;
         }
-        rc = wsis_bn_bwd((const float*)op.in[0], (const float*)op.in[1], (const float*)op.in[2], (const float*)op.in[3],
-                         (const float*)op.in[4], (const float*)op.in[5], op.eps, (op.flags & WSIS_OPF_RELU) ? 1 : 0,
-                         (op.flags & WSIS_OPF_TRAINING) ? 1 : 0, (float*)op.out[0], (float*)op.out[1], (float*)op.out[2],
-                         (const float*)op.in[6], op.M_in, op.Cin, ws, ws_bytes, stream);
+        rc = bn_bwd_split((const float*)op.in[0], (const float*)op.in[1], (const float*)op.in[2], (const float*)op.in[3],
+                          (const float*)op.in[4], (const float*)op.in[5], op.eps, (op.flags & WSIS_OPF_RELU) ? 1 : 0,
+                          (op.flags & WSIS_OPF_TRAINING) ? 1 : 0, (float*)op.out[0], (float*)op.out[3],
+                          op.out[3] ? op.K : 0, (float*)op.out[1], (float*)op.out[2], (const float*)op.in[6], op.M_in,
+                          op.Cin, ws, ws_bytes, stream);
         break;
       default:
         rc = fail(WSIS_ERR_ARG, "wsis_run_ops: unknown op kind");
diff --git a/3d-wsis_amd/model/unet_native.py b/3d-wsis_amd/model/unet_native.py
--- a/3d-wsis_amd/model/unet_native.py
+++ b/3d-wsis_amd/model/unet_native.py
@@ -54,6 +54,10 @@
 
 def _fuse_stats_enabled():
     return os.environ.get("WSIS_FUSE_BN_STATS", "1") != "0"
+
+
+def _skip_fuse_enabled():
+    return os.environ.get("WSIS_SKIP_FUSE", "1") != "0"
 
 
 def _lvl(level):
@@ -263,14 +267,15 @@
                    inp=(x, _ptr(bn.weight), _ptr(bn.bias), mean, var), out=(y,))
             self._acc_f.append(("bn_op", 0, lvl, C, 2))
 
-        def bwd(recb, dy, addend=0):
-            dx = recb.alloc(lvl, C)
+        def bwd(recb, dy, addend=0, split=0):
+            dx = recb.alloc(lvl, split if split else C)
+            dx2 = recb.alloc(lvl, C - split) if split else 0
             dg = self._grad_handle(bn.weight) if bn.weight is not None else recb.alloc(-1, C)
             db = self._grad_handle(bn.bias) if bn.bias is not None else recb.alloc(-1, C)
-            recb.op(OP_BN_RELU_BWD, flags & ~F_STATS, _lvl(lvl), _lvl(lvl), 0, C, C, bn.eps, 0.0,
-                    inp=(x, dy, mean, var, _ptr(bn.weight), _ptr(bn.bias), addend), out=(dx, dg, db))
+            recb.op(OP_BN_RELU_BWD, flags & ~F_STATS, _lvl(lvl), _lvl(lvl), split, C, C, bn.eps, 0.0,
+                    inp=(x, dy, mean, var, _ptr(bn.weight), _ptr(bn.bias), addend), out=(dx, dg, db, dx2))
             self._acc_b.append(("bn_op", 0, lvl, C, 3 + (1 if addend else 0)))
-            return dx
+            return (dx, dx2) if split else dx
         return y, bwd
 
     def _fuse_bn_bwd(self, recb):
@@ -307,12 +312,12 @@
             res, b_i = self._conv(rec, x, first, None, lvl, lvl, stats=False)
         out, b_c2 = self._conv(rec, a2, conv2, table, lvl, lvl, residual=res)
 
-        def bwd(recb, d_out):
+        def bwd(recb, d_out, split=0):
             d_a2 = b_c2(recb, d_out)
             d_z1 = b_bn2(recb, d_a2)
             d_a1 = b_c1(recb, d_z1)
             d_skip = d_out if b_i is None else b_i(recb, d_out)
-            return b_bn1(recb, d_a1, addend=d_skip)
+            return b_bn1(recb, d_a1, addend=d_skip, split=split)
         return out, bwd
 
     def _ublock(self, rec, x, ub, lvl):
@@ -343,12 +348,21 @@
             x, b = self._residual_block(rec, x, blk, lvl)
             tails.append(b)
 
+        first_bn = ub.blocks_tail[0].conv_branch[0] if len(ub.blocks_tail) else None
+        split_in_bn = (self._skip_fuse and self.bn_sync is None and first_bn is not None and
+                       first_bn.num_features == 2 * C0 and C0 % 4 == 0)
+
         def bwd(recb, dcur):
-            for b in reversed(tails):
-                dcur = b(recb, dcur)
-            d_id = recb.alloc(lvl, C0)
-            d_up = recb.alloc(lvl, C0)
-            recb.op(OP_SPLIT, 0, _lvl(lvl), _lvl(lvl), 0, C0, C0, inp=(dcur,), out=(d_id, d_up))
+            if split_in_bn:
+                for b in reversed(tails[1:]):
+                    dcur = b(recb, dcur)
+                d_id, d_up = tails[0](recb, dcur, split=C0)
+            else:
+                for b in reversed(tails):
+                    dcur = b(recb, dcur)
+                d_id = recb.alloc(lvl, C0)
+                d_up = recb.alloc(lvl, C0)
+                recb.op(OP_SPLIT, 0, _lvl(lvl), _lvl(lvl), 0, C0, C0, inp=(dcur,), out=(d_id, d_up))
             d_a2 = b_up(recb, d_up)
             d_u = b_bn2(recb, d_a2)
             d_d = b_u(recb, d_u)
@@ -368,7 +382,7 @@
 
     def _mode_key(self, need_dx):
         return (need_dx, self.bn_sync is not None, _fuse_stats_enabled(), _fuse_fin_enabled(), _fuse_apply_level(),
-                os.environ.get("WSIS_FUSE_BN_FIN_LVL", "0"),
+                os.environ.get("WSIS_FUSE_BN_FIN_LVL", "0"), _skip_fuse_enabled(),
                 os.environ.get("WSIS_FWD2", "1"), tuple(bn.training for bn in self.bns), tuple(p.data_ptr() for p in self.params),
                 tuple(bn.running_mean.data_ptr() if bn.running_mean is not None else 0 for bn in self.bns))
 
@@ -388,6 +402,7 @@
         self._virt, self._fuse_apply_lvl = {}, _fuse_apply_level()
         self._fuse_fin = _fuse_fin_enabled() and self._fuse_stats
         self._fuse_fin_lvl = int(os.environ.get("WSIS_FUSE_BN_FIN_LVL", "0"))
+        self._skip_fuse = _skip_fuse_enabled()
         if self.bn_sync is not None:
             self._fuse_fin, self._fuse_apply_lvl = False, 99
         y, b_in = self._conv(rec, _EXT | 0, net.input_conv[0], _subm(0), 0, 0)
@@ -656,6 +671,8 @@
     import torch.distributed as dist
     M, C, flags = int(op["M_in"]), int(op["Cin"]), int(op["flags"])
     inp, out = [int(v) for v in op["inp"]], [int(v) for v in op["out"]]
+    if out[3]:
+        raise _n.WsisError("synced BatchNorm: a split dx is not supported (the program is recorded with SPLIT ops)")
     eps, relu = float(op["eps"]), 1 if flags & F_RELU else 0
     dg, db = sy.view(out[1], C), sy.view(out[2], C)
     if M > 0:
```

Result: no change. 134.8, median of 6 (+0.5%).
